# afcarl/BayesBridge

Hardware: AMD Instinct MI355X
Metric: Gibbs sweeps/sec at n=2000,p=50000,alpha=0.5 (higher is better)
Workload: dtype f64; 1 GPU; C3 Gaussian bridge n=2000 p=50000 alpha=0.5; n=2000, p=50000, mode=single, parallelism=one GPU, beta_step=woodbury (exact, p > n), gram=ozaki-II int8 (fp64-accurate)

## Files before the change

### bayesbridge_amd/__init__.py

```python
from __future__ import annotations

import ctypes
import os
from dataclasses import dataclass
from typing import Optional

import numpy as np

from . import _build

__all__ = ["bridge_reg_stb", "bridge_reg", "retstable_ld", "set_seed", "get_rng_state",
           "set_rng_state", "Engine", "EngineConfig", "library", "device_count",
           "sample_lambda", "retstable_batch", "gram", "chol_solve", "bridge_reg_stb_chains",
           "bridge_reg_tri_chains", "ChainBatch", "compute_units",
           "bridge_reg_stb_chains_summary", "bridge_reg_tri_chains_summary", "trace_summary",
           "bridge_reg_logit_chains", "bridge_reg_logit_chains_summary"]

_lib: Optional[ctypes.CDLL] = None
_dp = ctypes.POINTER(ctypes.c_double)
_ip = ctypes.POINTER(ctypes.c_int)


class bb_config(ctypes.Structure):
    _fields_ = [("n", ctypes.c_int), ("p", ctypes.c_int), ("p_local", ctypes.c_int),
                ("j0", ctypes.c_int), ("rank", ctypes.c_int), ("world", ctypes.c_int),
                ("sig2_shape", ctypes.c_double), ("sig2_scale", ctypes.c_double),
                ("nu_shape", ctypes.c_double), ("nu_rate", ctypes.c_double),
                ("alpha_a", ctypes.c_double), ("alpha_b", ctypes.c_double),
                ("true_sig2", ctypes.c_double), ("true_tau", ctypes.c_double),
                ("true_alpha", ctypes.c_double), ("ortho", ctypes.c_int),
                ("method", ctypes.c_int), ("trace_capacity", ctypes.c_int),
                ("seed", ctypes.c_uint64), ("stream", ctypes.c_uint64), ("device", ctypes.c_int),
                ("gram_mode", ctypes.c_int), ("betaburn", ctypes.c_int)]

GRAM_FP64, GRAM_OZAKI = 0, 1


EXPORTED_SYMBOLS = [
    "bridge_reg_stable", "retstable_LD", "bb_version", "bb_last_error", "bb_device_count",
    "bb_set_seed", "bb_get_rng_state", "bb_set_rng_state", "bb_use_r_rng", "bb_set_device",
    "bb_set_verbose", "bb_config_default", "bb_engine_create", "bb_engine_destroy",
    "bb_comm_id_size", "bb_comm_unique_id", "bb_engine_comm_init", "bb_engine_init_state",
    "bb_engine_run", "bb_engine_sync", "bb_engine_get_trace", "bb_engine_get_state",
    "bb_engine_set_state", "bb_engine_method", "bb_engine_enable_timing",
    "bb_engine_kernel_times", "bb_engine_reset_timing", "bb_engine_error_flags",
    "bb_retstable_batch", "bb_sample_lambda", "bb_gram", "bb_chol_solve",
    "bb_engine_phase_times", "bb_phase_count", "bb_phase_name", "bb_bench_lambda",
    "bb_group_create", "bb_group_destroy", "bb_group_init_state", "bb_group_run",
    "bb_bench_chol", "bb_gram_ozaki", "bb_engine_gram_mode", "bb_bench_ozaki",
    "bridge_EM", "bb_bridge_em", "bb_bridge_em_batch", "bridge_regression",
    "bb_engine_get_tri_trace", "bb_engine_get_tri_basis", "bb_engine_set_tri_state",
    "rtnorm_left", "rtnorm_both", "rtnorm", "rtexpon_rate_left", "rtexpon_rate_both",
    "rtexpon_rate", "mytest", "bb_trunc_batch", "rrtgamma_rate", "bb_rrtgamma_batch",
    "bridge_reg_stable_csc", "bb_engine_create_csc", "bb_engine_sparse_pairs", "bb_sparse_gram",
    "bb_bench_sparse_gram", "bb_engine_sparse_info", "bridge_reg_logit", "bb_engine_get_omega",
    "bb_pg_batch", "bb_group_create_rccl", "bb_group_sync", "bb_set_device_count",
    "bb_set_trace_budget", "bb_debug_interrupt_after", "bb_last_call_info",
    "bb_engine_set_timed_phase", "bb_engine_set_timing_stride", "bb_set_chol_version",
    "bb_set_tuning", "bridge_reg_stable_chains", "bb_chains_create", "bb_chains_destroy",
    "bb_chains_count", "bb_chains_resident_per_cu", "bb_chains_init_state", "bb_chains_run",
    "bb_chains_sync", "bb_chains_get_trace", "bb_chains_get_state", "bb_chains_set_state",
    "bb_chains_error_flags", "bridge_regression_chains", "bb_chains_get_tri_trace",
    "bb_chains_set_tri_state", "bb_chains_get_tri_basis", "bb_chains_threads",
    "bb_chains_set_threads", "bb_compute_units", "bridge_reg_stable_chains_summary",
    "bridge_regression_chains_summary", "bb_chains_summary_reset", "bb_chains_summary_add",
    "bb_chains_summary_get", "bb_trace_summary", "bridge_reg_logit_chains",
    "bridge_reg_logit_chains_summary", "bb_chains_get_omega", "bb_set_em_scratch_budget",
]


def library(build: bool = True) -> ctypes.CDLL:
    global _lib
    if _lib is not None:
        return _lib
    path = _build.SO_PATH
    if build:
        try:
            path = _build.build()
        except Exception:
            if not os.path.exists(_build.SO_PATH):
                raise
    if not os.path.exists(path):
        raise RuntimeError(f"BayesBridge.so not found at {path}; run bayesbridge_amd._build")
    L = ctypes.CDLL(path)
    c = ctypes
    L.bb_version.restype = c.c_char_p
    L.bb_last_error.restype = c.c_char_p
    L.bb_device_count.restype = c.c_int
    L.bb_set_seed.argtypes = [c.c_uint64]
    L.bb_get_rng_state.argtypes = [c.POINTER(c.c_uint64), c.POINTER(c.c_uint64)]
    L.bb_set_rng_state.argtypes = [c.c_uint64, c.c_uint64]
    L.bb_use_r_rng.argtypes = [c.c_int]
    L.bb_set_device.argtypes = [c.c_int]
    L.bb_set_verbose.argtypes = [c.c_int]
    L.bb_config_default.argtypes = [c.POINTER(bb_config)]
    L.bb_engine_create.argtypes = [c.POINTER(bb_config), _dp, _dp, c.POINTER(c.c_void_p)]
    L.bb_engine_destroy.argtypes = [c.c_void_p]
    L.bb_comm_id_size.restype = c.c_int
    L.bb_comm_unique_id.argtypes = [c.c_void_p]
    L.bb_engine_comm_init.argtypes = [c.c_void_p, c.c_void_p]
    L.bb_engine_init_state.argtypes = [c.c_void_p]
    L.bb_engine_run.argtypes = [c.c_void_p, c.c_uint64, c.c_int, c.c_int, c.c_int, c.c_int]
    L.bb_engine_sync.argtypes = [c.c_void_p]
    L.bb_engine_get_trace.argtypes = [c.c_void_p, c.c_int, c.c_int, _dp, _dp, _dp, _dp, _dp]
    L.bb_engine_get_state.argtypes = [c.c_void_p, _dp, _dp, _dp, _dp, _dp]
    L.bb_engine_set_state.argtypes = [c.c_void_p, _dp, c.c_double, c.c_double, c.c_double]
    L.bb_engine_method.argtypes = [c.c_void_p]
    L.bb_engine_gram_mode.argtypes = [c.c_void_p]
    L.bb_engine_enable_timing.argtypes = [c.c_void_p, c.c_int]
    L.bb_engine_reset_timing.argtypes = [c.c_void_p]
    L.bb_engine_set_timed_phase.argtypes = [c.c_void_p, c.c_int]
    L.bb_engine_set_timing_stride.argtypes = [c.c_void_p, c.c_int]
    L.bb_engine_kernel_times.argtypes = [c.c_void_p, _dp, _dp, _ip]
    L.bb_engine_error_flags.argtypes = [c.c_void_p, c.POINTER(c.c_uint32)]
    L.bb_retstable_batch.argtypes = [_dp, _dp, _dp, _dp, c.c_int, c.c_uint64, c.c_uint64,
                                     c.c_uint64, c.c_int]
    L.bb_sample_lambda.argtypes = [_dp, _dp, c.c_int, c.c_double, c.c_double, c.c_uint64,
                                   c.c_uint64, c.c_uint64, c.c_uint64, c.c_int]
    L.bb_gram.argtypes = [_dp, _dp, _dp, c.c_int, c.c_int]
    L.bb_gram_ozaki.argtypes = [_dp, _dp, _dp, c.c_int, c.c_int]
    L.bb_bench_ozaki.argtypes = [c.c_int, c.c_int, c.c_int, c.c_int, c.c_int, _dp]
    L.bb_chol_solve.argtypes = [_dp, _dp, _dp, c.c_int, c.c_int]
    L.bb_group_create.argtypes = [c.POINTER(c.c_void_p), c.c_int, c.POINTER(c.c_void_p)]
    L.bb_group_create_rccl.argtypes = [c.POINTER(c.c_void_p), c.c_int, c.POINTER(c.c_void_p)]
    L.bb_group_sync.argtypes = [c.c_void_p]
    L.bb_set_device_count.argtypes = [c.c_int]
    L.bb_set_chol_version.argtypes = [c.c_int]
    L.bb_set_tuning.argtypes = [c.c_int, c.c_int]
    L.bb_set_trace_budget.argtypes = [c.c_longlong]
    L.bb_set_em_scratch_budget.argtypes = [c.c_longlong]
    L.bb_debug_interrupt_after.argtypes = [c.c_int]
    L.bb_last_call_info.argtypes = [_ip, _ip, _ip]
    L.bb_debug_fail_member.argtypes = [c.c_int, c.c_int]
    u64p = c.POINTER(c.c_ulonglong)
    L.bb_engine_nid_stats.argtypes = [c.c_void_p, u64p, u64p, u64p, _dp, _ip]
    L.bb_engine_timed_brackets.argtypes = [c.c_void_p, _ip]
    L.bb_engine_nid_bound.argtypes = [c.c_void_p, _dp, _ip]
    L.bb_engine_launch_counts.argtypes = [c.c_void_p, u64p, u64p]
    L.bb_kernel_instance.argtypes = [c.c_char_p, c.c_char_p, c.c_int]
    L.bb_engine_nid_mixed.argtypes = [c.c_void_p, u64p, u64p, _dp, _ip, _ip]
    L.bb_engine_nid_beta32.argtypes = [c.c_void_p, u64p, _ip]
    L.bb_group_destroy.argtypes = [c.c_void_p]
    L.bb_group_init_state.argtypes = [c.c_void_p]
    L.bb_group_run.argtypes = [c.c_void_p, c.c_uint64, c.c_int, c.c_int, c.c_int, c.c_int]
    L.bb_bench_chol.argtypes = [c.c_int, c.c_int, _dp, _dp, c.c_void_p]
    L.bb_bench_lambda.argtypes = [_dp, c.c_int, c.c_double, c.c_double, c.c_int, c.c_int,
                                  c.c_int, _dp, _dp]
    L.bb_engine_phase_times.argtypes = [c.c_void_p, _dp, c.c_int, _ip]
    L.bb_phase_count.restype = c.c_int
    L.bb_phase_name.argtypes = [c.c_int]
    L.bb_phase_name.restype = c.c_char_p
    L.retstable_LD.argtypes = [_dp, _dp, _dp, _dp, _ip]
    L.bridge_reg_stable.argtypes = [_dp] * 7 + [_dp] * 9 + [_ip] * 4 + [_dp, _ip]
    L.bridge_reg_stable_chains.argtypes = [_dp] * 7 + [_dp] * 9 + [_ip] * 4 + [_dp, _ip, _ip]
    L.bb_chains_create.argtypes = [c.POINTER(bb_config), c.c_int, _dp, _dp,
                                   c.POINTER(c.c_void_p)]
    L.bb_chains_destroy.argtypes = [c.c_void_p]
    L.bb_chains_count.argtypes = [c.c_void_p]
    L.bb_chains_resident_per_cu.argtypes = [c.c_void_p]
    L.bb_chains_init_state.argtypes = [c.c_void_p]
    L.bb_chains_run.argtypes = [c.c_void_p, c.c_uint64, c.c_int, c.c_int, c.c_int, c.c_int]
    L.bb_chains_sync.argtypes = [c.c_void_p]
    L.bb_chains_get_trace.argtypes = [c.c_void_p, c.c_int, c.c_int, c.c_int, _dp, _dp, _dp, _dp,
                                      _dp]
    L.bb_chains_get_state.argtypes = [c.c_void_p, c.c_int, _dp, _dp, _dp, _dp, _dp]
    L.bb_chains_set_state.argtypes = [c.c_void_p, c.c_int, _dp, c.c_double, c.c_double,
                                      c.c_double]
    L.bb_chains_error_flags.argtypes = [c.c_void_p, c.c_int]
    L.bb_chains_error_flags.restype = c.c_uint
    L.bridge_reg_stable_csc.argtypes = ([_dp] * 6 + [_ip, _ip, _dp] + [_dp] * 9 + [_ip] * 4 +
                                        [_dp, _ip])
    L.bb_engine_create_csc.argtypes = [c.POINTER(bb_config), _ip, _ip, _dp, _dp,
                                       c.POINTER(c.c_void_p)]
    L.bb_engine_sparse_pairs.argtypes = [c.c_void_p]
    L.bb_engine_sparse_pairs.restype = c.c_longlong
    L.bridge_reg_logit.argtypes = [_dp] * 6 + [_dp] * 6 + [_ip] * 4 + [_dp]
    L.bb_engine_get_omega.argtypes = [c.c_void_p, _dp]
    L.bridge_reg_logit_chains.argtypes = [_dp] * 6 + [_dp] * 6 + [_ip] * 4 + [_dp, _ip]
    L.bridge_reg_logit_chains_summary.argtypes = ([_dp] * 5 + [_ip, _ip] + [_dp] * 2 + [_dp] * 6 +
                                                  [_ip] * 4 + [_dp, _ip])
    L.bb_chains_get_omega.argtypes = [c.c_void_p, c.c_int, _dp]
    L.bb_pg_batch.argtypes = [_dp, _dp, c.c_int, c.c_uint64, c.c_uint64, c.c_uint64]
    L.bb_engine_sparse_info.argtypes = [c.c_void_p, c.POINTER(c.c_longlong),
                                        c.POINTER(c.c_longlong), _ip, _ip]
    L.bb_sparse_gram.argtypes = [_dp, _dp, _ip, _ip, _dp, _dp, _dp, c.c_int, c.c_int]
    L.bb_bench_sparse_gram.argtypes = [_ip, _ip, _dp, _dp, c.c_int, c.c_int, c.c_int, _dp, _dp,
                                       c.POINTER(c.c_longlong)]
    L.bridge_regression.argtypes = [_dp] * 9 + [_dp] * 9 + [_ip] * 4 + [_dp] + [_ip] * 3
    for name, npar in (("rtnorm_left", 3), ("rtnorm_both", 4), ("rtnorm", 4),
                       ("rtexpon_rate_left", 2), ("rtexpon_rate_both", 3), ("rtexpon_rate", 3)):
        getattr(L, name).argtypes = [_dp] * (1 + npar) + [_ip]
    L.mytest.argtypes = [_ip, _dp]
    L.rrtgamma_rate.argtypes = [_dp] * 4 + [_ip]
    L.bb_rrtgamma_batch.argtypes = [c.c_int, _dp, _dp, _dp, _dp, c.c_uint64, c.c_uint64]
    L.bb_trunc_batch.argtypes = [c.c_int, c.c_int, _dp, _dp, _dp, _dp, _dp, c.c_uint64,
                                 c.c_uint64]
    L.bridge_regression_chains.argtypes = ([_dp] * 9 + [_dp] * 9 + [_ip] * 4 + [_dp] +
                                           [_ip] * 4)
    L.bb_chains_get_tri_trace.argtypes = [c.c_void_p, c.c_int, c.c_int, c.c_int, _dp, _dp]
    L.bridge_reg_stable_chains_summary.argtypes = ([_dp] * 5 + [_ip, _ip] + [_dp] * 2 +
                                                   [_dp] * 9 + [_ip] * 4 + [_dp, _ip, _ip])
    L.bridge_regression_chains_summary.argtypes = ([_dp] * 5 + [_ip, _ip] + [_dp] * 2 +
                                                   [_dp] * 9 + [_ip] * 4 + [_dp] + [_ip] * 4)
    L.bb_chains_summary_reset.argtypes = [c.c_void_p, c.c_int, c.c_int]
    L.bb_chains_summary_add.argtypes = [c.c_void_p, c.c_int, c.c_int, c.c_int]
    L.bb_chains_summary_get.argtypes = [c.c_void_p, _dp, _dp, _dp, _dp, _dp, _ip]
    L.bb_trace_summary.argtypes = [_dp, c.c_int, c.c_int, c.c_int, c.c_int, c.c_int, _dp, _dp,
                                   _dp, _dp, _dp]
    L.bb_chains_set_tri_state.argtypes = [c.c_void_p, c.c_int, _dp]
    L.bb_chains_get_tri_basis.argtypes = [c.c_void_p, _dp, _dp, _dp]
    L.bb_chains_threads.argtypes = [c.c_void_p]
    L.bb_compute_units.argtypes = [c.c_int]
    L.bb_chains_set_threads.argtypes = [c.c_void_p, c.c_int]
    L.bb_engine_get_tri_trace.argtypes = [c.c_void_p, c.c_int, c.c_int, _dp, _dp]
    L.bb_engine_get_tri_basis.argtypes = [c.c_void_p, _dp, _dp, _dp]
    L.bb_engine_set_tri_state.argtypes = [c.c_void_p, _dp]
    L.bridge_EM.argtypes = [_dp, _dp, _dp, _dp, _dp, _ip, _ip, _dp, _dp, _ip, _ip]
    L.bb_bridge_em.argtypes = [_dp, _dp, _dp, c.c_int, c.c_int, c.c_double, c.c_double,
                               c.c_double, c.c_double, c.c_int, c.c_int]
    L.bb_bridge_em_batch.argtypes = [_dp, _ip, _dp, _dp, c.c_int, c.c_int, _dp, _dp, c.c_int,
                                     c.c_double, c.c_double, c.c_int]
    _lib = L
    return L


def device_count() -> int:
    return int(library().bb_device_count())


def compute_units(device: int = 0) -> int:
    _require_gpu()
    n = int(library().bb_compute_units(int(device)))
    if n < 1:
        raise RuntimeError(f"bayesbridge_amd: cannot query device {device}")
    return n


def _require_gpu():
    if device_count() < 1:
        raise RuntimeError("bayesbridge_amd: no HIP device visible (the sampler has no CPU path)")


def kernel_instance(phase: str):
    buf = ctypes.create_string_buffer(512)
    if library().bb_kernel_instance(phase.encode(), buf, 512) != 0:
        return None
    return buf.value.decode()


def _err() -> str:
    return library().bb_last_error().decode()


def _check(rc: int, what: str):
    if rc != 0:
        raise RuntimeError(f"{what} failed ({rc}): {_err()}")


def _p(a: np.ndarray):
    return a.ctypes.data_as(_dp)


def set_seed(seed: int) -> None:
    library().bb_set_seed(int(seed) & 0xFFFFFFFFFFFFFFFF)


def get_rng_state():
    s, t = ctypes.c_uint64(), ctypes.c_uint64()
    library().bb_get_rng_state(ctypes.byref(s), ctypes.byref(t))
    return int(s.value), int(t.value)


def set_rng_state(seed: int, stream: int) -> None:
    library().bb_set_rng_state(int(seed), int(stream))


def set_verbose(v: int) -> None:
    library().bb_set_verbose(int(v))


def set_device_count(k: int) -> None:
    library().bb_set_device_count(int(k))


def set_chol_version(version: int) -> None:
    _check(library().bb_set_chol_version(int(version)), "bb_set_chol_version")


def set_tuning(key: int, value: int) -> int:
    return int(library().bb_set_tuning(int(key), int(value)))


def set_wide_chains(on: bool) -> bool:
    return bool(library().bb_set_tuning(25, 1 if on else 0))
# ... 829 lines not shown

    def __init__(self, cfg: EngineConfig, X_local, y):
        L = library()
        _require_gpu()
        self.cfg = cfg
        self._c = cfg.to_c()
        y = np.ascontiguousarray(y, dtype=np.float64)
        self.p_local = self._c.p_local
        h = ctypes.c_void_p()
        if _is_sparse(X_local):
            colptr, rowidx, val, shape = csc_arrays(X_local)
            assert shape == (cfg.n, self._c.p_local), shape
            _check(L.bb_engine_create_csc(ctypes.byref(self._c), colptr.ctypes.data_as(_ip),
                                          rowidx.ctypes.data_as(_ip), _p(val), _p(y),
                                          ctypes.byref(h)), "bb_engine_create_csc")
        else:
            X_local = np.asfortranarray(X_local, dtype=np.float64)
            assert X_local.shape == (cfg.n, self._c.p_local), X_local.shape
            _check(L.bb_engine_create(ctypes.byref(self._c), _p(X_local), _p(y),
                                      ctypes.byref(h)), "bb_engine_create")
        self._h = h

    def sparse_pairs(self) -> int:
        return int(library().bb_engine_sparse_pairs(self._h))

    def sparse_info(self):
        pr, nz, mr, cm = ctypes.c_longlong(), ctypes.c_longlong(), ctypes.c_int(), ctypes.c_int()
        _check(library().bb_engine_sparse_info(self._h, ctypes.byref(pr), ctypes.byref(nz),
                                               ctypes.byref(mr), ctypes.byref(cm)),
               "bb_engine_sparse_info")
        return dict(pairs=pr.value, nnz=nz.value, max_row=mr.value, col_mode=bool(cm.value))

    def comm_init(self, id_bytes: bytes):
        _check(library().bb_engine_comm_init(self._h, ctypes.c_char_p(id_bytes)),
               "bb_engine_comm_init")

    @staticmethod
    def comm_unique_id() -> bytes:
        L = library()
        buf = ctypes.create_string_buffer(L.bb_comm_id_size())
        _check(L.bb_comm_unique_id(buf), "bb_comm_unique_id")
        return buf.raw

    def init_state(self):
        _check(library().bb_engine_init_state(self._h), "bb_engine_init_state")

    def run(self, t0: int, count: int, first_slot: int = -1, slot_step: int = 1,
            mcmc_phase: int = 1):
        _check(library().bb_engine_run(self._h, int(t0), int(count), int(first_slot),
                                       int(slot_step), int(mcmc_phase)), "bb_engine_run")

    def sync(self):
        _check(library().bb_engine_sync(self._h), "bb_engine_sync")

    def method(self) -> int:
        return int(library().bb_engine_method(self._h))

    def gram_mode(self) -> int:
        return int(library().bb_engine_gram_mode(self._h))

    def trace(self, slot0: int, count: int):
        pl = self.p_local
        beta = np.zeros((pl, count), order="F")
        lam = np.zeros((pl, count), order="F")
        sig2, tau, alpha = np.zeros(count), np.zeros(count), np.zeros(count)
        _check(library().bb_engine_get_trace(self._h, slot0, count, _p(beta), _p(lam), _p(sig2),
                                             _p(tau), _p(alpha)), "bb_engine_get_trace")
        return dict(beta=beta, **{"lambda": lam}, sig2=sig2, tau=tau, alpha=alpha)

    def omega(self):
        om = np.zeros(self.cfg.n)
        _check(library().bb_engine_get_omega(self._h, _p(om)), "bb_engine_get_omega")
        return om

    def tri_trace(self, slot0: int, count: int):
        pl = self.p_local
        u = np.zeros((pl, count), order="F")
        shape = np.zeros((pl, count), order="F")
        _check(library().bb_engine_get_tri_trace(self._h, slot0, count, _p(u), _p(shape)),
               "bb_engine_get_tri_trace")
        return dict(u=u, shape=shape)

    def set_tri_state(self, u):
        u = np.ascontiguousarray(u, dtype=np.float64)
        _check(library().bb_engine_set_tri_state(self._h, _p(u)), "bb_engine_set_tri_state")

    def tri_basis(self):
        p = self.p_local
        tV = np.zeros((p, p), order="F")
        a, d = np.zeros(p), np.zeros(p)
        _check(library().bb_engine_get_tri_basis(self._h, _p(tV), _p(a), _p(d)),
               "bb_engine_get_tri_basis")
        return tV, a, d

    def state(self):
        pl = self.p_local
        beta, lam = np.zeros(pl), np.zeros(pl)
        tau, sig2, alpha = ctypes.c_double(), ctypes.c_double(), ctypes.c_double()
        _check(library().bb_engine_get_state(self._h, _p(beta), _p(lam), ctypes.byref(tau),
                                             ctypes.byref(sig2), ctypes.byref(alpha)),
               "bb_engine_get_state")
        return dict(beta=beta, **{"lambda": lam}, tau=tau.value, sig2=sig2.value,
                    alpha=alpha.value)

    def set_state(self, beta, tau, sig2, alpha):
        beta = np.ascontiguousarray(beta, dtype=np.float64)
        _check(library().bb_engine_set_state(self._h, _p(beta), tau, sig2, alpha),
               "bb_engine_set_state")

    def enable_timing(self, on: bool = True, phases: bool = True, timed_phase: str = "gram",
                      stride: int = 1):
        L = library()
        names = [L.bb_phase_name(i).decode() for i in range(L.bb_phase_count())]
        _check(L.bb_engine_set_timed_phase(self._h, names.index(timed_phase)),
               "bb_engine_set_timed_phase")
        _check(L.bb_engine_set_timing_stride(self._h, int(stride)),
               "bb_engine_set_timing_stride")
        L.bb_engine_enable_timing(self._h, (2 if phases else 1) if on else 0)

    def reset_timing(self):
        library().bb_engine_reset_timing(self._h)

    def kernel_times(self):
        g, s, n = ctypes.c_double(), ctypes.c_double(), ctypes.c_int()
        _check(library().bb_engine_kernel_times(self._h, ctypes.byref(g), ctypes.byref(s),
                                                ctypes.byref(n)), "bb_engine_kernel_times")
        return g.value, s.value, n.value

    def phase_times(self):
        L = library()
        k = L.bb_phase_count()
        ms = np.zeros(k)
        n = ctypes.c_int()
        _check(L.bb_engine_phase_times(self._h, _p(ms), k, ctypes.byref(n)),
               "bb_engine_phase_times")
        return {L.bb_phase_name(i).decode(): float(ms[i]) for i in range(k) if ms[i] > 0}

    def timed_brackets(self) -> int:
        k = ctypes.c_int()
        _check(library().bb_engine_timed_brackets(self._h, ctypes.byref(k)),
               "bb_engine_timed_brackets")
        return int(k.value)

    def nid_stats(self):
        a, b, c = ctypes.c_ulonglong(), ctypes.c_ulonglong(), ctypes.c_ulonglong()
        eps, mode = ctypes.c_double(), ctypes.c_int()
        _check(library().bb_engine_nid_stats(self._h, ctypes.byref(a), ctypes.byref(b),
                                             ctypes.byref(c), ctypes.byref(eps),
                                             ctypes.byref(mode)), "bb_engine_nid_stats")
        lam, kmax = ctypes.c_double(), ctypes.c_int()
        library().bb_engine_nid_bound(self._h, ctypes.byref(lam), ctypes.byref(kmax))
        return dict(cheb_sweeps=a.value, products=b.value, chol_sweeps=c.value, eps=eps.value,
                    mode=mode.value, lambda_x=lam.value, kmax=kmax.value,
                    beta32_sweeps=self._beta32()[0])

    def _beta32(self):
        a, f = ctypes.c_ulonglong(), ctypes.c_int()
        _check(library().bb_engine_nid_beta32(self._h, ctypes.byref(a), ctypes.byref(f)),
               "bb_engine_nid_beta32")
        return a.value, bool(f.value)

    def nid_mixed(self):
        a, b = ctypes.c_ulonglong(), ctypes.c_ulonglong()
        eta, k2, hx = ctypes.c_double(), ctypes.c_int(), ctypes.c_int()
        _check(library().bb_engine_nid_mixed(self._h, ctypes.byref(a), ctypes.byref(b),
                                             ctypes.byref(eta), ctypes.byref(k2),
                                             ctypes.byref(hx)), "bb_engine_nid_mixed")
        n32, last32 = self._beta32()
        return dict(mixed_sweeps=a.value, products32=b.value, eta=eta.value, k2=k2.value,
                    holds_x32=bool(hx.value), beta32_sweeps=n32, beta32=last32)

    def launch_counts(self):
        a, b = ctypes.c_ulonglong(), ctypes.c_ulonglong()
        library().bb_engine_launch_counts(self._h, ctypes.byref(a), ctypes.byref(b))
        return dict(lambda_xu=a.value, lambda_alone=b.value)

    def error_flags(self) -> int:
        f = ctypes.c_uint32()
        _check(library().bb_engine_error_flags(self._h, ctypes.byref(f)), "bb_engine_error_flags")
        return int(f.value)

    def close(self):
        if getattr(self, "_h", None):
            library().bb_engine_destroy(self._h)
            self._h = None

    def __del__(self):
        try:
            self.close()
        except Exception:
            pass


class ChainBatch:

    def __init__(self, cfg: EngineConfig, nchains: int, X, y):
        L = library()
        _require_gpu()
        self.cfg = cfg
        self._c = cfg.to_c()
        self.p = self._c.p
        X = np.asfortranarray(X, dtype=np.float64)
        y = np.ascontiguousarray(y, dtype=np.float64)
        assert X.shape == (cfg.n, cfg.p), X.shape
        h = ctypes.c_void_p()
        _check(L.bb_chains_create(ctypes.byref(self._c), int(nchains), _p(X), _p(y),
                                  ctypes.byref(h)), "bb_chains_create")
        self._h = h
        self.nchains = int(L.bb_chains_count(h))

    def resident_per_cu(self) -> int:
        return int(library().bb_chains_resident_per_cu(self._h))

    def init_state(self):
        _check(library().bb_chains_init_state(self._h), "bb_chains_init_state")

    def run(self, t0: int, count: int, first_slot: int = -1, slot_step: int = 1,
            mcmc_phase: int = 1):
        _check(library().bb_chains_run(self._h, int(t0), int(count), int(first_slot),
                                       int(slot_step), int(mcmc_phase)), "bb_chains_run")

    def sync(self):
        _check(library().bb_chains_sync(self._h), "bb_chains_sync")

    def trace(self, chain: int, slot0: int, count: int):
        p = self.p
        beta = np.zeros((p, count), order="F")
        lam = np.zeros((p, count), order="F")
        sig2, tau, alpha = np.zeros(count), np.zeros(count), np.zeros(count)
        _check(library().bb_chains_get_trace(self._h, int(chain), slot0, count, _p(beta),
                                             _p(lam), _p(sig2), _p(tau), _p(alpha)),
               "bb_chains_get_trace")
        return dict(beta=beta, **{"lambda": lam}, sig2=sig2, tau=tau, alpha=alpha)

    def state(self, chain: int):
        beta, lam = np.zeros(self.p), np.zeros(self.p)
        tau, sig2, alpha = ctypes.c_double(), ctypes.c_double(), ctypes.c_double()
        _check(library().bb_chains_get_state(self._h, int(chain), _p(beta), _p(lam),
                                             ctypes.byref(tau), ctypes.byref(sig2),
                                             ctypes.byref(alpha)), "bb_chains_get_state")
        return dict(beta=beta, **{"lambda": lam}, tau=tau.value, sig2=sig2.value,
                    alpha=alpha.value)

    def set_state(self, chain: int, beta, tau, sig2, alpha):
        beta = np.ascontiguousarray(beta, dtype=np.float64)
        _check(library().bb_chains_set_state(self._h, int(chain), _p(beta), tau, sig2, alpha),
               "bb_chains_set_state")

    def omega(self, chain: int):
        om = np.zeros(self._c.n)
        _check(library().bb_chains_get_omega(self._h, int(chain), _p(om)), "bb_chains_get_omega")
        return om

    def tri_trace(self, chain: int, slot0: int, count: int):
        u = np.zeros((self.p, count), order="F")
        shape = np.zeros((self.p, count), order="F")
        _check(library().bb_chains_get_tri_trace(self._h, int(chain), slot0, count, _p(u),
                                                 _p(shape)), "bb_chains_get_tri_trace")
        return dict(u=u, shape=shape)

    def set_tri_state(self, chain: int, u):
        u = np.ascontiguousarray(u, dtype=np.float64)
        _check(library().bb_chains_set_tri_state(self._h, int(chain), _p(u)),
               "bb_chains_set_tri_state")

    def tri_basis(self):
        p = self.p
        tV = np.zeros((p, p), order="F")
        a, d = np.zeros(p), np.zeros(p)
        _check(library().bb_chains_get_tri_basis(self._h, _p(tV), _p(a), _p(d)),
               "bb_chains_get_tri_basis")
        return tV, a, d

    def summary_reset(self, nsamp: int, maxlag=None):
        self._sum = (int(nsamp), _summary_maxlag(nsamp, maxlag))
        _check(library().bb_chains_summary_reset(self._h, *self._sum), "bb_chains_summary_reset")

    def summary_add(self, slot0: int, count: int, s0: int):
        _check(library().bb_chains_summary_add(self._h, int(slot0), int(count), int(s0)),
               "bb_chains_summary_add")

    def summary(self):
        nsamp, lag = getattr(self, "_sum", (0, 0))
        raw = _summary_buffers(self.nchains, self.p + 3, lag)
        _check(library().bb_chains_summary_get(
            self._h, _p(raw["mean"]), _p(raw["var"]), _p(raw["acov"]), _p(raw["hmean"]),
            _p(raw["hvar"]), raw["flags"].ctypes.data_as(_ip)), "bb_chains_summary_get")
        raw["flags"] = raw["flags"].astype(np.uint32)
        raw.update(nsamp=nsamp, maxlag=lag, p=self.p)
        return raw

    def threads(self) -> int:
        return int(library().bb_chains_threads(self._h))

    def set_threads(self, threads: int):
        _check(library().bb_chains_set_threads(self._h, int(threads)), "bb_chains_set_threads")

    def error_flags(self, chain: int) -> int:
        f = int(library().bb_chains_error_flags(self._h, int(chain)))
        if f == 0xFFFFFFFF and _err():
            raise RuntimeError(f"bb_chains_error_flags failed: {_err()}")
        return f

    def close(self):
        if getattr(self, "_h", None):
            library().bb_chains_destroy(self._h)
            self._h = None

    def __del__(self):
        try:
            self.close()
        except Exception:
            pass


class ShardGroup:

    def __init__(self, engines, rccl=False):
        L = library()
        self.engines = list(engines)
        arr = (ctypes.c_void_p * len(self.engines))(*[e._h.value for e in self.engines])
        h = ctypes.c_void_p()
        fn = L.bb_group_create_rccl if rccl else L.bb_group_create
# ... 24 lines not shown
```

### bayesbridge_amd/csrc/bb_engine.cpp

```cpp
#include <dlfcn.h>

#include <chrono>
#include <cxxabi.h>
#include <cmath>
#include <cstring>
#include <atomic>
#include <initializer_list>
#include <memory>
#include <mutex>
#include <thread>

#include "../../include/bayesbridge.h"
#include "bb_host.h"
#include "bb_ozaki.h"

using namespace bb;

namespace bb {

thread_local std::string g_last_error;
int g_device = 0;
int g_verbose = 1;

}

namespace {

std::mutex g_mu;
uint64_t g_seed = 0xB4E5B41D6EULL;
uint64_t g_stream = 0;
int g_use_r_rng = 1;
std::atomic<int> g_debug_fail_member{-1}, g_debug_fail_sweep{-1};

struct RRng {
    void (*get)(void) = nullptr;
    void (*put)(void) = nullptr;
    double (*unif)(void) = nullptr;
    bool tried = false;
    bool ok() {
        if (!tried) {
            tried = true;
            get = (void (*)(void))dlsym(RTLD_DEFAULT, "GetRNGstate");
            put = (void (*)(void))dlsym(RTLD_DEFAULT, "PutRNGstate");
            unif = (double (*)(void))dlsym(RTLD_DEFAULT, "unif_rand");
        }
        return get && put && unif;
    }
} g_rrng;

}

void bb::next_call_key(uint64_t *k0, uint64_t *k1, int count) {
    std::lock_guard<std::mutex> lk(g_mu);
    if (g_use_r_rng && g_rrng.ok()) {
        g_rrng.get();
        uint64_t a = (uint64_t)(g_rrng.unif() * 4294967296.0);
        uint64_t b = (uint64_t)(g_rrng.unif() * 4294967296.0);
        uint64_t c = (uint64_t)(g_rrng.unif() * 4294967296.0);
        g_rrng.put();
        *k0 = (a << 32) ^ b;
        *k1 = c;
        return;
    }
    *k0 = g_seed;
    *k1 = g_stream;
    g_stream += (uint64_t)count;
}

enum Phase {
    PH_PRE, PH_SCALARS, PH_LAMBDA, PH_PG, PH_OZPREP, PH_GRAM, PH_XU, PH_REDUCE, PH_FORM, PH_CHOL,
    PH_SOLVE, PH_BETA, PH_XB, PH_ALPHA, PH_NID, PH_EAPPLY, PH_END, PH_COUNT
};

int g_nid_kmax = 16;
int g_nid_sync = 1;
int g_shard_proto = 0;
int g_nid_mixed = 1;
int g_nid_poll = 1;
int g_nid_fold = 1;
int g_nid_b32 = 1;
int g_chains_packed = 0;
int g_chains_wide = 0;
int g_fused_alpha = 0;
int g_fused_tri_alpha = 0;
static const char *kPhaseNames[PH_COUNT] = {"pre", "scalars", "lambda", "pg", "ozprep", "gram",
                                            "xu", "reduce", "form", "chol", "solve", "beta",
                                            "xb", "alpha", "nid", "eapply", "end"};

enum Method { AUTO = 0, CHOL = 1, WOODBURY = 2, ORTHO = 3, TRI = 4, SPARSE = 5, LOGIT = 6 };

struct bb_engine {
    bb_config cfg{};
    int n = 0, p = 0, p_loc = 0, n_pad = 0, p_pad = 0;
    int chol_m = 0;
    Method method = AUTO;
    int group = 1;
    bool fused = false;
    bool wide = false;
    SparseDesign spd;
    Hyper hy{};
    hipStream_t stream = nullptr;
    std::vector<void *> owned;

    double *X = nullptr, *y = nullptr;
    double *beta = nullptr, *lam = nullptr, *D = nullptr, *u = nullptr;
    DevScalars *sc = nullptr;
    uint32_t *err = nullptr;
    double *xb_part = nullptr, *red1 = nullptr;
    double *red3 = nullptr;
    int nparts = 0, nbS = 0;
    bool xb_stale = false;
    double *slabs = nullptr, *xu_part = nullptr, *red2 = nullptr, *M = nullptr, *w = nullptr,
           *Wd = nullptr;
    unsigned int *flags = nullptr;
    int S = 1;
    size_t slab_stride = 0;
    int n_oz = 0, oz_b = 0, oz_S = 1;
    double *oz_xmax = nullptr, *oz_rscale = nullptr;
    double *oz_rowmax = nullptr;
    int *oz_escale = nullptr;
    int8_t *oz_R = nullptr, *oz_P = nullptr;
    double *Xt = nullptr, *omega = nullptr, *kappa = nullptr, *Gw = nullptr;
    double *G = nullptr, *cvec = nullptr, *A = nullptr, *Y2 = nullptr, *W2 = nullptr,
           *gdiag = nullptr;
    double *tVc = nullptr, *tVr = nullptr, *tri_a = nullptr, *tri_d = nullptr,
           *tri_G = nullptr;
    double *tr_u = nullptr, *tr_shape = nullptr;
    std::vector<double> h_tV, h_a, h_d;
    double *tr_beta = nullptr, *tr_lam = nullptr, *tr_sig2 = nullptr, *tr_tau = nullptr,
           *tr_alpha = nullptr;
    int cap = 1;
    double *cn = nullptr;
    NidState *nid = nullptr;
    double *ch_r = nullptr, *ch_d = nullptr, *ea_part = nullptr, *sp_s = nullptr,
           *nid_xu = nullptr;
    double *eps_host = nullptr;
    float *X32 = nullptr;
    double *ch_b = nullptr;
    int nid_k2 = 0;
    double *gb = nullptr, *ch_c = nullptr, *ch_xu = nullptr;
    bool nid_b32 = false;
    double nid_cost[3] = {0.0, 0.0, 0.0};
    int ea_parts = 1;
    int nid_kmax = 0;
    double lambda_x = 0.0;
    hipEvent_t nid_ev[8] = {};
    long nid_seq = 0;
    double *nid_red = nullptr, *nid_sum = nullptr, *nid_wg = nullptr;
    hipEvent_t nid_sev = nullptr;
    bool nid_only = false;
    bool group_member = false;
    int nid_last = -1;
    ncclComm_t comm = nullptr;
    bool own_comm = true;
    bool timing = false;
    int timing_level = 2;
    int timed_phase = PH_GRAM;
    int timing_stride = 1;
    std::vector<hipEvent_t> ev_pool;
    std::vector<std::vector<std::pair<int, int>>> sweep_marks;
    size_t ev_next = 0;

    void mark(int phase) {
        if (!timing) return;
        if (timing_level == 1) {
            if ((sweep_marks.size() - 1) % (size_t)timing_stride != 0) return;
            const bool open = !sweep_marks.back().empty() &&
                              sweep_marks.back().back().first == timed_phase;
            if (phase != timed_phase && !open) return;
        }
        int e0 = ev();
        HIPCHECK(hipEventRecord(ev_pool[e0], stream));
        sweep_marks.back().push_back({phase, e0});
    }

    ~bb_engine() {
        if (stream) (void)hipStreamSynchronize(stream);
        if (comm && own_comm) ncclCommDestroy(comm);
        for (auto e : ev_pool) (void)hipEventDestroy(e);
        for (auto e : nid_ev)
            if (e) (void)hipEventDestroy(e);
        if (nid_sev) (void)hipEventDestroy(nid_sev);
        if (eps_host) (void)hipHostFree(eps_host);
        for (void *q : owned) (void)hipFree(q);
        if (stream) (void)hipStreamDestroy(stream);
    }

    int ev() {
        if (ev_next == ev_pool.size()) {
            hipEvent_t e;
            HIPCHECK(hipEventCreate(&e));
            ev_pool.push_back(e);
        }
        return (int)ev_next++;
    }

    void allreduce(double *buf, size_t count) {
        if (cfg.world <= 1 && !comm) return;
        if (!comm) throw HipError("world > 1 but no communicator (call bb_engine_comm_init)");
        NCCLCHECK(ncclAllReduce(buf, buf, count, ncclFloat64, ncclSum, comm, stream));
    }

    double *slot_ptr(double *base, int slot, int stride) {
        if (slot < 0 || base == nullptr) return nullptr;
        return base + (size_t)(slot % cap) * stride;
    }

    bool woodbury() const { return method == WOODBURY || method == SPARSE; }
    bool dense() const { return method == WOODBURY; }
    bool sparse() const { return method == SPARSE; }
    bool ortho() const { return method == ORTHO; }
    bool tri() const { return method == TRI; }
    bool logit() const { return method == LOGIT; }
    bool pxp() const { return method == CHOL || method == LOGIT; }

    bool nid_enabled() const {
        return nid != nullptr && (cfg.world == 1 || comm != nullptr || group_member) &&
               std::min(g_nid_kmax, nid_kmax) > 0;
    }
    bool sharded() const {
        return cfg.world > 1 || (g_shard_proto && (comm != nullptr || group_member));
    }
    bool nid_sync() const { return (sharded() || g_nid_sync) && nid_enabled(); }
    bool mixed_ok() const {
        return X32 != nullptr && g_nid_mixed && !sharded() && !group_member && dense();
    }
    bool b32_ok() const { return gb != nullptr && g_nid_b32 && mixed_ok() && nid_sync(); }
    int allow_mask() const {
        return (mixed_ok() ? kAllowMixed : 0) |
               (b32_ok() ? kAllowBeta32 | (g_nid_b32 == 2 ? kBeta32AnyCost : 0) : 0);
    }
    double *bank() const { return b32_ok() ? gb : nullptr; }
    Beta32Vecs b32_vecs() const {
        return b32_ok() ? Beta32Vecs{ch_c, ch_b, ch_xu, xb_part} : Beta32Vecs{};
    }
    bool nid_vec() const { return sharded() || sparse(); }

    int nid_kmax_model() const {
        double t_pass, t_chol;
        const double steps = n_pad / 64.0;
        if (sparse()) {
            t_pass = 24.0 * (double)spd.nnz / 3.0e12 + 10e-6;
            t_chol = 10.0 * (double)spd.pairs / 4.0e12 + steps * 21e-6 + 60e-6;
        } else {
            t_pass = 8.0 * n_pad * (double)p_loc / 6.0e12 + 10e-6;
            const double gram = cfg.gram_mode == 1
                ? 16.0 * (double)n_pad * n_pad * p_pad / 2.6e15 + 24.0 * (double)n_pad * p_pad / 5.0e12
                : 2.0 * (double)n_pad * n_pad * p_pad / 33e12;
            t_chol = gram + steps * 19e-6 + 40e-6;
        }
        if (cfg.world > 1) {
            t_pass += 25e-6;
            t_chol += 8.0 * (double)red2_count() / 100e9 + 25e-6;
        }
        return (int)std::min(64.0, std::floor(t_chol / t_pass));
    }

    static constexpr int kNidRing = 8, kNidLag = 3;
    int nid_launch_count() {
        const int kmax = std::min(g_nid_kmax, nid_kmax);
        if (nid_seq < kNidLag) return kmax;
        const long q = nid_seq - kNidLag;
        wait_event(nid_ev[q % kNidRing]);
        const double h = ((volatile double *)eps_host)[q % kNidRing];
        if (!(h >= 0.0)) return kmax;
        return cheb_iterations(8.0 * h, kmax, kNidTol);
    }

    int nid_begin(int kl) {
        if (!nid_enabled()) return 0;
        mark(PH_NID);
        const long q = nid_seq++;
        launch_nid_sums(stream, D, cn, p_loc, sc, nid, kl, kl > 0, 1, nid_wg, nid_red,
                        eps_dev + q % kNidRing);
        hipEvent_t &ev = nid_ev[q % kNidRing];
        if (!ev) HIPCHECK(hipEventCreateWithFlags(&ev, hipEventDisableTiming));
        HIPCHECK(hipEventRecord(ev, stream));
        return kl;
    }
    double *eps_dev = nullptr;

    void nid_solve(uint64_t t, int kl) {
        mark(PH_NID);
        if (sparse())
            launch_cheb_init(stream, nid_xu, 1, n, n_pad, y, sc, cfg.seed, cfg.stream, t, nid, w,
                             ch_r, ch_d);
        else
            launch_cheb_init(stream, nid_xu, xu_fused ? xu_fused : ea_parts, n, n_pad, y, sc,
                             cfg.seed, cfg.stream, t, nid, w, ch_r, ch_d);
        for (int j = 1; j < kl; ++j) {
            mark(PH_EAPPLY);
            if (sparse())
                launch_sp_eapply(stream, spd.colptr, spd.rowidx, spd.cval, spd.rowptr, spd.colidx,
                                 spd.rval, p_loc, n_pad, D, ch_d, nid, j, sp_s, ea_part);
            else
                launch_eapply(stream, X, n_pad, n_pad, p_loc, D, ch_d, nid, j, ea_part);
            mark(PH_NID);
            launch_cheb_step(stream, ea_part, sparse() ? 1 : ea_parts, n_pad, sc, nid, j, w,
                             ch_r, ch_d);
        }
    }

    static constexpr int kNidRed = kNidTS + 2;
    void nidx_partials(int folded = 0, int nstream = 0) {
        mark(PH_NID);
        if (folded == 2) return;
        if (folded == 1 && sharded())
            launch_nid_reduce(stream, nid_wg, nstream, sc, nid, nid_red);
        else if (folded == 1)
            launch_nid_reduce(stream, nid_wg, nstream, sc, nid, nid_red,
                              std::min(g_nid_kmax, nid_kmax), eps_dev + kNidRing,
                              allow_mask(), ++nid_dseq);
        else if (sharded())
            launch_nid_sums(stream, D, cn, p_loc, sc, nid, 0, 0, 0, nid_wg, nid_red, nullptr);
        else
            launch_nid_sums_decide(stream, D, cn, p_loc, sc, nid, std::min(g_nid_kmax, nid_kmax),
                                   nid_wg, nid_red, eps_dev + kNidRing, allow_mask(),
                                   ++nid_dseq);
    }
    void nidx_decide_launch() {
        if (sharded())
            launch_nid_decide_from(stream, nid_red, sc, std::min(g_nid_kmax, nid_kmax), nid,
                                   eps_dev + kNidRing, ++nid_dseq);
        if (g_nid_poll) return;
        if (!nid_sev) HIPCHECK(hipEventCreateWithFlags(&nid_sev, hipEventDisableTiming));
        HIPCHECK(hipEventRecord(nid_sev, stream));
    }
    int nidx_decide_read() {
        int mode, k2;
        if (g_nid_poll) {
            const unsigned long long tag = wait_tag(nid_dseq);
            mode = (int)((tag >> 8) & 0xff);
            k2 = (int)(tag & 0xff);
        } else {
            wait_event(nid_sev);
            mode = (int)((volatile double *)eps_host)[kNidRing + 1];
            k2 = (int)((volatile double *)eps_host)[kNidRing + 2];
        }
        nid_b32 = b32_ok() && (k2 & 128) != 0;
        k2 &= 127;
        nid_k2 = mixed_ok() ? k2 : 0;
        nid_only = mode > 0;
        nid_last = mode;
        return mode;
    }
    unsigned long long wait_tag(unsigned long long seq) {
        const unsigned long long *tp = (const unsigned long long *)(eps_host + kNidRing + 3);
        const unsigned long long want = seq & 0xffffffffffffull;
        for (long spin = 0;; ++spin) {
            const unsigned long long v = __atomic_load_n(tp, __ATOMIC_ACQUIRE);
            if ((v >> 16) == want) return v;
            if ((spin & 1023) != 1023) {
                __builtin_ia32_pause();
                continue;
            }
            if (stop && stop->load(std::memory_order_relaxed))
                throw HipError("stopped: another member of the shard group failed");
            const hipError_t q = hipStreamQuery(stream);
            if (q == hipSuccess) {
                const unsigned long long w = __atomic_load_n(tp, __ATOMIC_ACQUIRE);
                if ((w >> 16) == want) return w;
                throw HipError("near-identity decision tag not written by the drained stream");
            }
            if (q != hipErrorNotReady) HIPCHECK(q);
            if (spin > 65536) std::this_thread::yield();
        }
    }
    unsigned long long nid_dseq = 0;
    void wait_event(hipEvent_t ev) {
        if (!stop) {
            HIPCHECK(hipEventSynchronize(ev));
            return;
        }
        for (long spin = 0;; ++spin) {
            const hipError_t q = hipEventQuery(ev);
            if (q == hipSuccess) return;
            if (q != hipErrorNotReady) HIPCHECK(q);
            if (stop->load(std::memory_order_relaxed))
                throw HipError("stopped: another member of the shard group failed");
            if (spin > 64) std::this_thread::yield();
        }
    }
    void nidx_xu() {
        mark(PH_NID);
        if (sparse()) {
            launch_sp_nid_xu(stream, spd.rowptr, spd.colidx, spd.rval, n_pad, u, nid, nid_sum);
        } else {
            if (!xu_fused) launch_nid_xu(stream, X, n_pad, u, p_loc, n_pad, nid, nid_xu);
            if (nid_vec())
                launch_part_sum(stream, nid_xu, xu_fused ? xu_fused : ea_parts, n_pad, nid_sum);
        }
    }
    void nidx_init(uint64_t t) {
        if (nid_vec())
            launch_cheb_init(stream, nid_sum, 1, n, n_pad, y, sc, cfg.seed, cfg.stream, t, nid,
                             w, ch_r, ch_d);
        else
            launch_cheb_init(stream, nid_xu, xu_fused ? xu_fused : ea_parts, n, n_pad, y, sc,
                             cfg.seed, cfg.stream, t, nid, w, ch_r, ch_d,
                             mixed_ok() ? ch_b : nullptr, b32_ok() ? ch_xu : nullptr);
    }
    void nidx_mixed_tail(int k2) {
        const Beta32Vecs bv = b32_vecs();
        mark(PH_EAPPLY);
        launch_eapply(stream, X, n_pad, n_pad, p_loc, D, w, nid, 0, ea_part, X32, 2, bank());
        mark(PH_NID);
        launch_cheb_restart(stream, ea_part, ea_parts, n_pad, sc, nid, ch_b, w, ch_r, ch_d, &bv);
        for (int j = 1; j < k2; ++j) {
            mark(PH_EAPPLY);
            launch_eapply(stream, X, n_pad, n_pad, p_loc, D, ch_d, nid, j, ea_part, X32, 3);
            mark(PH_NID);
            launch_cheb_step(stream, ea_part, ea_parts, n_pad, sc, nid, j, w, ch_r, ch_d, 2,
                             &bv);
        }
    }
    void nidx_eapply(int j) {
        mark(PH_EAPPLY);
        if (sparse()) {
            launch_sp_eapply(stream, spd.colptr, spd.rowidx, spd.cval, spd.rowptr, spd.colidx,
                             spd.rval, p_loc, n_pad, D, ch_d, nid, j, sp_s, nid_sum);
        } else {
            launch_eapply(stream, X, n_pad, n_pad, p_loc, D, ch_d, nid, j, ea_part,
                          mixed_ok() ? X32 : nullptr, 0, bank());
            if (nid_vec()) launch_part_sum(stream, ea_part, ea_parts, n_pad, nid_sum);
        }
    }
    void nidx_step(int j) {
        mark(PH_NID);
        if (nid_vec())
            launch_cheb_step(stream, nid_sum, 1, n_pad, sc, nid, j, w, ch_r, ch_d);
        else {
            const Beta32Vecs bv = b32_vecs();
            launch_cheb_step(stream, ea_part, ea_parts, n_pad, sc, nid, j, w, ch_r, ch_d, 1, &bv);
        }
    }
    void xbeta() {
        xb_stale = false;
        if (sparse()) {
            launch_sp_rows(stream, spd.rowptr, spd.colidx, spd.rval, n_pad, beta, nullptr,
                           xb_part, nullptr);
            nparts = 1;
        } else {
            launch_xv(stream, X, n_pad, beta, p_loc, n_pad, xb_part);
            nparts = xv_chunks(p_loc, n_pad);
        }
    }

    void pre() {
        if (xb_stale) xbeta();
        launch_pre(stream, xb_part, nparts, n_pad, beta, p_loc, sc, red1, nbS);
    }
    void scalars(uint64_t t, int slot, int tau_only) {
        launch_scalars(stream, red1, nbS, y, n, p, sc, hy, cfg.seed, cfg.stream, t,
                       slot_ptr(tr_tau, slot, 1), slot_ptr(tr_sig2, slot, 1),
                       slot_ptr(tr_alpha, slot, 1), tau_only, err);
    }

    void phase_a(uint64_t t) {
        (void)t;
        if (timing) sweep_marks.emplace_back();
        mark(PH_PRE);
        pre();
    }

    void wb_gram(const int *gate) {
        if (sparse()) {
            mark(PH_GRAM);
            spd.gram(stream, D, u, red2, red2 + tri_count(n_pad), gate);
            return;
        }
        if (cfg.gram_mode == 1) {
            mark(PH_OZPREP);
            launch_oz_scale(stream, D, p_pad, oz_xmax, n_oz, oz_b, oz_rowmax, oz_rscale,
                            oz_escale, gate);
            launch_oz_residues(stream, X, n_pad, n_pad, n_oz, p_pad, D, oz_rscale, oz_R, u,
                               xu_part, gate);
            mark(PH_GRAM);
            launch_oz_gemm(stream, oz_R, n_oz, p_pad, oz_S, oz_P, 0, kOzLeadDefault, -1, gate);
        } else {
            mark(PH_GRAM);
            launch_gram(stream, X, n_pad, D, n_pad, p_pad, S, slabs, n_pad, slab_stride, gate);
            mark(PH_XU);
            launch_xv(stream, X, n_pad, u, p_pad, n_pad, xu_part, gate);
        }
        mark(PH_REDUCE);
        if (cfg.gram_mode == 1)
            launch_oz_crt(stream, oz_P, oz_S, n_oz, n_pad, oz_escale, xu_part,
                          oz_xu_parts(p_pad, n_oz), red2, gate);
        else
            launch_slab_sum(stream, slabs, S, slab_stride, n_pad, xu_part, xv_chunks(p_pad, n_pad),
                            red2, 1, gate);
    }

    void phase_b(uint64_t t, int slot) {
        mark(PH_SCALARS);
        scalars(t, slot, 0);
        double *trl = slot_ptr(tr_lam, slot, p_loc);
        mark(PH_LAMBDA);
        if (woodbury()) {
            const bool sync = nid_sync();
            const int kl = (!sync && nid_enabled()) ? nid_launch_count() : 0;
            xu_fused = 0;
            int folded = 0;
            if (dense() && (sync ? nid_last != 0 : kl > 0)) {
                NidFold fold;
                if (sync && g_nid_fold) {
                    fold.cn = cn;
                    fold.wg_part = nid_wg;
                    fold.cnt = lam_sync + lambda_xs_sync_words(p_pad);
                    fold.decide = (!sharded() && g_nid_fold == 2) ? 1 : 0;
                    fold.k_launched = std::min(g_nid_kmax, nid_kmax);
                    fold.allow_mixed = allow_mask();
                    fold.nid = nid;
                    fold.red = nid_red;
                    fold.host2 = eps_dev + kNidRing;
                    fold.tag_seq = nid_dseq + 1;
                }
                xu_fused = launch_lambda_xu(stream, beta, p_loc, p_pad, (uint64_t)cfg.j0, sc,
                                            cfg.seed, cfg.stream, t, lam, D, u, trl, err, X,
                                            n_pad, n_pad, nid_xu, lam_sync, ++lam_ep, &fold,
                                            &folded);
                if (folded == 2) ++nid_dseq;
            }
            if (!xu_fused)
                launch_lambda(stream, beta, p_loc, p_pad, (uint64_t)cfg.j0, sc, cfg.seed,
                              cfg.stream, t, LAMBDA_WOODBURY, group, lam, D, u, trl, err);
            ++(xu_fused ? n_lambda_xu : n_lambda_alone);
            nid_only = false;
            nid_b32 = false;
            if (sync) {
                nid_kl = 0;
                nidx_partials(folded, xu_fused);
                return;
            }
            nid_kl = nid_begin(kl);
            wb_gram(nid_kl ? &nid->mode : nullptr);
            if (nid_kl && !xu_fused) {
                mark(PH_NID);
                if (sparse())
                    launch_sp_nid_xu(stream, spd.rowptr, spd.colidx, spd.rval, n_pad, u, nid,
                                     nid_xu);
                else
                    launch_nid_xu(stream, X, n_pad, u, p_loc, n_pad, nid, nid_xu);
            }
        } else if (logit()) {
            if (!launch_lambda_pg(stream, beta, p_loc, p_pad, 0, sc, cfg.seed, cfg.stream, t,
                                  group, lam, trl, red1 + nbS, n, n_pad, omega, err))
                throw HipError("logistic sweep: p beyond the fused lambda / Polya-Gamma launch");
            if (cfg.gram_mode == 1) {
                mark(PH_OZPREP);
                launch_oz_scale(stream, omega, n_pad, oz_xmax, n_oz, oz_b, oz_rowmax, oz_rscale,
                                oz_escale);
                launch_oz_residues(stream, Xt, p_pad, p_pad, n_oz, n_pad, omega, oz_rscale, oz_R,
                                   nullptr, nullptr);
                mark(PH_GRAM);
                launch_oz_gemm(stream, oz_R, n_oz, n_pad, oz_S, oz_P);
                mark(PH_REDUCE);
                launch_oz_crt(stream, oz_P, oz_S, n_oz, p_pad, oz_escale, nullptr, 0, Gw);
            } else {
                mark(PH_GRAM);
                launch_gram(stream, Xt, p_pad, omega, p_pad, n_pad, S, slabs, p_pad, slab_stride);
                mark(PH_REDUCE);
                launch_slab_sum(stream, slabs, S, slab_stride, p_pad, nullptr, 0, Gw, 0);
            }
        } else if (tri()) {
            mark(PH_BETA);
            launch_tri_update(stream, beta, u, lam, D, p, tVc, tVr, tri_a, tri_d, tri_G, cvec,
// ... 273 lines not shown
                if (c == 0.0 || fabs(c) <= 1e-15 * sqrt(a * b)) continue;
                ++rotated;
                const double zeta = (b - a) / (2.0 * c);
                const double t = (zeta >= 0 ? 1.0 : -1.0) / (fabs(zeta) + sqrt(1.0 + zeta * zeta));
                const double cs = 1.0 / sqrt(1.0 + t * t), sn = cs * t;
                nrm2[i] = a - t * c;
                nrm2[j] = b + t * c;
                for (int k = 0; k < p; ++k) {
                    const double x = wi[k], y = wj[k];
                    wi[k] = cs * x - sn * y;
                    wj[k] = sn * x + cs * y;
                    const double u = vi[k], w = vj[k];
                    vi[k] = cs * u - sn * w;
                    vj[k] = sn * u + cs * w;
                }
            }
        }
        if (rotated == 0) break;
    }
    d.resize(p);
    for (int j = 0; j < p; ++j) {
        double s2 = 0.0;
        for (int k = 0; k < p; ++k) s2 += W[(size_t)j * p + k] * W[(size_t)j * p + k];
        d[j] = sqrt(s2);
    }
}

void tri_setup(bb_engine *e, const double *Xh) {
    const int p = e->p, pp = e->p_pad;
    std::vector<double> Gp((size_t)pp * pp), c(pp);
    HIPCHECK(hipStreamSynchronize(e->stream));
    HIPCHECK(hipMemcpy(Gp.data(), e->G, Gp.size() * sizeof(double), hipMemcpyDeviceToHost));
    HIPCHECK(hipMemcpy(c.data(), e->cvec, (size_t)pp * sizeof(double), hipMemcpyDeviceToHost));
    std::vector<double> G((size_t)p * p);
    for (int j = 0; j < p; ++j)
        for (int i = 0; i < p; ++i) {
            const int r = i < j ? i : j, q = i < j ? j : i;
            G[(size_t)j * p + i] = Gp[(size_t)q * pp + r];
        }
    std::vector<double> V, sv;
    svd_right(Xh, e->n, p, V, sv);
    std::vector<int> ord(p);
    for (int i = 0; i < p; ++i) ord[i] = i;
    std::stable_sort(ord.begin(), ord.end(), [&](int x, int y) { return sv[x] > sv[y]; });
    e->h_tV.assign((size_t)p * p, 0.0);
    e->h_a.assign(p, 0.0);
    e->h_d.assign(p, 0.0);
    std::vector<double> tVr((size_t)p * p);
    for (int i = 0; i < p; ++i) {
        const double *v = &V[(size_t)ord[i] * p];
        int jm = 0;
        for (int j = 1; j < p; ++j)
            if (fabs(v[j]) > fabs(v[jm])) jm = j;
        const double sg = v[jm] < 0 ? -1.0 : 1.0;
        double a = 0.0;
        for (int j = 0; j < p; ++j) {
            const double x = sg * v[j];
            e->h_tV[i + (size_t)j * p] = x;
            tVr[(size_t)i * p + j] = x;
            a += x * c[j];
        }
        e->h_a[i] = a;
        e->h_d[i] = sv[ord[i]];
    }
    auto &o = e->owned;
    e->tVc = dalloc<double>((size_t)p * p, o);
    e->tVr = dalloc<double>((size_t)p * p, o);
    e->tri_a = dalloc<double>(p, o);
    e->tri_d = dalloc<double>(p, o);
    HIPCHECK(hipMemcpy(e->tVc, e->h_tV.data(), (size_t)p * p * sizeof(double),
                       hipMemcpyHostToDevice));
    HIPCHECK(hipMemcpy(e->tVr, tVr.data(), (size_t)p * p * sizeof(double), hipMemcpyHostToDevice));
    HIPCHECK(hipMemcpy(e->tri_a, e->h_a.data(), (size_t)p * sizeof(double), hipMemcpyHostToDevice));
    HIPCHECK(hipMemcpy(e->tri_d, e->h_d.data(), (size_t)p * sizeof(double), hipMemcpyHostToDevice));
    e->tri_G = dalloc<double>((size_t)p * p, o);
    HIPCHECK(hipMemcpy(e->tri_G, G.data(), (size_t)p * p * sizeof(double), hipMemcpyHostToDevice));
    e->tr_u = dalloc<double>((size_t)p * e->cap, o);
    e->tr_shape = dalloc<double>((size_t)p * e->cap, o);
}

struct SparseIn {
    const int *colptr, *rowidx;
    const double *val;
};

void nid_certify_lambda(bb_engine *e) {
    const int n_pad = e->n_pad, p_pad = e->p_pad;
    hipStream_t s = e->stream;
    double *ones = nullptr;
    NidState *gate = nullptr;
    HIPCHECK(hipMalloc(&ones, (size_t)p_pad * sizeof(double)));
    HIPCHECK(hipMalloc(&gate, sizeof(NidState)));
    std::vector<double> h1(p_pad, 0.0);
    for (int j = 0; j < e->p_loc; ++j) h1[j] = 1.0;
    HIPCHECK(hipMemcpyAsync(ones, h1.data(), h1.size() * sizeof(double), hipMemcpyHostToDevice, s));
    NidState g{};
    g.mode = 64;
    HIPCHECK(hipMemcpyAsync(gate, &g, sizeof(g), hipMemcpyHostToDevice, s));
    std::vector<double> v(n_pad, 0.0), w(n_pad);
    double nv = 0.0;
    for (int i = 0; i < e->n; ++i) {
        v[i] = std::cos(0.7 * i + 0.3) + 0.5 * std::sin(1.3 * i * i + 0.1);
        nv += v[i] * v[i];
    }
    for (auto &x : v) x /= std::sqrt(nv);
    double rho = 0.0;
    for (int it = 0; it < 40; ++it) {
        HIPCHECK(hipMemcpyAsync(e->ch_d, v.data(), n_pad * sizeof(double), hipMemcpyHostToDevice, s));
        if (e->sparse())
            launch_sp_eapply(s, e->spd.colptr, e->spd.rowidx, e->spd.cval, e->spd.rowptr,
                             e->spd.colidx, e->spd.rval, e->p_loc, n_pad, ones, e->ch_d, gate, 0,
                             e->sp_s, e->ea_part);
        else
            launch_eapply(s, e->X, n_pad, n_pad, e->p_loc, ones, e->ch_d, gate, 0, e->ea_part);
        launch_part_sum(s, e->ea_part, e->sparse() ? 1 : e->ea_parts, n_pad, e->ch_r);
        HIPCHECK(hipMemcpyAsync(w.data(), e->ch_r, n_pad * sizeof(double), hipMemcpyDeviceToHost, s));
        HIPCHECK(hipStreamSynchronize(s));
        double vw = 0.0, ww = 0.0;
        for (int i = 0; i < n_pad; ++i) {
            vw += v[i] * w[i];
            ww += w[i] * w[i];
        }
        rho = vw;
        if (!(ww > 0.0)) break;
        for (int i = 0; i < n_pad; ++i) v[i] = w[i] / std::sqrt(ww);
    }
    double lam = 0.0;
    if (rho > 0.0 && std::isfinite(rho)) {
        if (e->sparse()) {
            e->spd.gram(s, ones, ones, e->red2, e->red2 + tri_count(n_pad));
        } else if (e->cfg.gram_mode == 1) {
            launch_oz_scale(s, ones, p_pad, e->oz_xmax, e->n_oz, e->oz_b, e->oz_rowmax,
                            e->oz_rscale, e->oz_escale);
            launch_oz_residues(s, e->X, n_pad, n_pad, e->n_oz, p_pad, ones, e->oz_rscale, e->oz_R);
            launch_oz_gemm(s, e->oz_R, e->n_oz, p_pad, e->oz_S, e->oz_P);
            launch_oz_crt(s, e->oz_P, e->oz_S, e->n_oz, n_pad, e->oz_escale, nullptr, 0, e->red2);
        } else {
            launch_gram(s, e->X, n_pad, ones, n_pad, p_pad, e->S, e->slabs, n_pad, e->slab_stride);
            launch_slab_sum(s, e->slabs, e->S, e->slab_stride, n_pad, nullptr, 0, e->red2, 1);
        }
        double U = 1.02 * rho;
        for (int attempt = 0; attempt < 7 && lam == 0.0; ++attempt, U *= 1.25) {
            e->clear_err();
            launch_shift_gram(s, e->red2, n_pad, U, e->M, n_pad);
            chol_factor(s, e->M, n_pad, n_pad, 1, e->err, e->Wd, e->flags);
            if ((e->read_err() & (8u | 16u)) == 0) lam = U * (1.0 + 1e-9);
        }
        e->clear_err();
    }
    HIPCHECK(hipMemsetAsync(e->nid, 0, sizeof(NidState), s));
    HIPCHECK(hipMemcpyAsync(&e->nid->lambda_x, &lam, sizeof(double), hipMemcpyHostToDevice, s));
    HIPCHECK(hipMemcpyAsync(&e->nid->c64, e->nid_cost, sizeof(e->nid_cost), hipMemcpyHostToDevice,
                            s));
    HIPCHECK(hipStreamSynchronize(s));
    e->lambda_x = lam;
    (void)hipFree(ones);
    (void)hipFree(gate);
}

void engine_setup(bb_engine *e, const double *Xh, const double *yh, const SparseIn *spin) {
    const bb_config &c = e->cfg;
    e->n = c.n;
    e->p = c.p;
    e->p_loc = c.p_local;
    e->n_pad = round_up(c.n, kGramTile);
    e->p_pad = round_up(c.p_local, 256);
    e->chol_m = round_up(c.p_local, kNB);
    e->cap = c.trace_capacity < 1 ? 1 : c.trace_capacity;
    e->hy = Hyper{c.sig2_shape, c.sig2_scale, c.nu_shape, c.nu_rate, c.alpha_a, c.alpha_b,
                  c.true_tau > 0, c.true_sig2 > 0, c.true_alpha > 0};
    if (spin) {
        if (c.ortho || c.method == CHOL || c.method == ORTHO || c.method == TRI ||
            c.method == LOGIT)
            throw HipError("a CSC design runs the Woodbury (p > n) draw only");
        e->method = SPARSE;
    } else if (c.method == LOGIT) {
        e->method = LOGIT;
        e->hy.know_sig2 = 1;
        e->n_pad = round_up(c.n, 512);
        if (c.world > 1) throw HipError("the logistic path runs on one device (world == 1)");
        if (c.ortho) throw HipError("the logistic path has no orthogonal-design variant");
        if (c.p > 16384) throw HipError("logistic path limited to p <= 16384");
    } else if (c.method == TRI) e->method = TRI;
    else if (c.ortho) e->method = ORTHO;
    else if (c.method == CHOL || (c.method == AUTO && c.p <= c.n)) e->method = CHOL;
    else e->method = WOODBURY;
    if (c.world > 1 && !e->woodbury() && !(e->ortho() && c.p > c.n))
        throw HipError("column sharding (world > 1) is implemented for the p > n paths only "
                       "(Woodbury, sparse Woodbury, orthogonal design)");
    if (e->tri() && (c.p > c.n || c.p > kTriMaxP))
        throw HipError("triangle sampler needs p <= n and p <= 2048");
    if (e->method == CHOL && c.p > 16384)
        throw HipError("p x p Cholesky path limited to p <= 16384");
    if (e->woodbury() && e->n_pad > 8192)
        throw HipError("Woodbury path limited to n <= 8192 in this build");

    HIPCHECK(hipSetDevice(c.device));
    HIPCHECK(hipStreamCreateWithFlags(&e->stream, hipStreamNonBlocking));
    auto &o = e->owned;
    const int n_pad = e->n_pad, p_pad = e->p_pad;
    if (spin) {
        e->spd.build(e->stream, c.n, n_pad, c.p_local, spin->colptr, spin->rowidx, spin->val, o);
    } else {
        e->X = dalloc<double>((size_t)n_pad * p_pad, o);
        HIPCHECK(hipMemcpy2D(e->X, (size_t)n_pad * sizeof(double), Xh,
                             (size_t)c.n * sizeof(double), (size_t)c.n * sizeof(double),
                             (size_t)c.p_local, hipMemcpyHostToDevice));
    }
    e->y = dalloc<double>(n_pad, o);
    HIPCHECK(hipMemcpy(e->y, yh, (size_t)c.n * sizeof(double), hipMemcpyHostToDevice));
    e->beta = dalloc<double>(p_pad, o);
    e->lam = dalloc<double>(p_pad, o);
    e->D = dalloc<double>(p_pad, o);
    e->u = dalloc<double>(p_pad, o);
    e->sc = dalloc<DevScalars>(1, o);
    e->err = dalloc<uint32_t>(4, o);
    e->nparts = xv_chunks(p_pad, n_pad);
    e->xb_part = dalloc<double>(
        (size_t)std::max(e->sparse() ? 1 : xv_chunks_max(p_pad), beta_xb_parts(c.p_local)) *
            n_pad,
        o);
    e->nbS = pre_blocks_s(c.p_local);
    e->red1 = dalloc<double>((size_t)e->nbS + n_pad, o);
    e->red3 = dalloc<double>(2, o);
    e->group = stable_group_for(c.p_local);
    e->tr_beta = dalloc<double>((size_t)c.p_local * e->cap, o);
    e->tr_lam = dalloc<double>((size_t)c.p_local * e->cap, o);
    e->tr_sig2 = dalloc<double>(e->cap, o);
    e->tr_tau = dalloc<double>(e->cap, o);
    e->tr_alpha = dalloc<double>(e->cap, o);

    if (e->dense()) {
        if (c.gram_mode == 1) {
            e->n_oz = oz_rows(n_pad);
            const int nkc = p_pad / kOzKC;
            e->oz_b = oz_bits_for(p_pad);
            e->oz_S = oz_splits_for(e->n_oz, nkc);
            e->oz_xmax = dalloc<double>((size_t)nkc * e->n_oz, o);
            e->oz_rowmax = dalloc<double>((size_t)oz_bound_groups(p_pad) * e->n_oz, o);
            e->oz_rscale = dalloc<double>(e->n_oz, o);
            e->oz_escale = dalloc<int>(e->n_oz, o);
            e->oz_R = dalloc<int8_t>(oz_residue_bytes(e->n_oz, p_pad), o);
            e->oz_P = dalloc<int8_t>(oz_partial_bytes(e->n_oz, e->oz_S), o);
            launch_oz_xmax(e->stream, e->X, n_pad, n_pad, e->n_oz, p_pad, e->oz_xmax);
        } else {
            e->S = gram_splits_for(n_pad, p_pad);
            e->slab_stride = (size_t)n_pad * n_pad;
            e->slabs = dalloc<double>(e->slab_stride * e->S, o);
        }
        e->xu_part = dalloc<double>((size_t)xv_chunks_max(p_pad) * n_pad, o);
    }
    if (e->woodbury()) {
        e->red2 = dalloc<double>(tri_count(n_pad) + n_pad, o);
        e->M = dalloc<double>((size_t)n_pad * (n_pad + kNB), o);
        e->w = dalloc<double>(n_pad, o);
        if (e->sparse() || eapply_supported(n_pad)) {
            e->cn = dalloc<double>(p_pad, o);
            if (e->sparse()) {
                std::vector<double> h(c.p_local, 0.0);
                for (int j = 0; j < c.p_local; ++j)
                    for (int q = spin->colptr[j]; q < spin->colptr[j + 1]; ++q)
                        h[j] += spin->val[q] * spin->val[q];
                HIPCHECK(hipMemcpy(e->cn, h.data(), h.size() * sizeof(double),
                                   hipMemcpyHostToDevice));
                e->sp_s = dalloc<double>(p_pad, o);
                e->ea_parts = 1;
                e->ea_part = dalloc<double>(n_pad, o);
                e->nid_xu = dalloc<double>(n_pad, o);
            } else {
                launch_colnorm2(e->stream, e->X, n_pad, n_pad, c.p_local, e->cn);
                e->ea_parts = eapply_parts(c.p_local, n_pad);
                e->ea_part = dalloc<double>((size_t)e->ea_parts * n_pad, o);
                const int xp = std::max(e->ea_parts, lambda_xu_parts(c.p_local, p_pad, n_pad));
                e->nid_xu = dalloc<double>((size_t)xp * n_pad, o);
                const int sw = lambda_xs_sync_words(p_pad) + 1;
                e->lam_sync = dalloc<unsigned int>(sw, o);
                HIPCHECK(hipMemsetAsync(e->lam_sync, 0, sizeof(unsigned int) * sw, e->stream));
            }
            e->nid = dalloc<NidState>(1, o);
            {
                const double bytes = (double)n_pad * (double)c.p_local;
                e->nid_cost[0] = 8.0 * bytes / 6.2e12 + 4e-6;
                e->nid_cost[1] = 4.0 * bytes / 6.2e12 + 4e-6;
                e->nid_cost[2] = 6e-6;
            }
            e->ch_r = dalloc<double>(n_pad, o);
            e->ch_d = dalloc<double>(n_pad, o);
            e->nid_red = dalloc<double>(bb_engine::kNidRed, o);
            e->nid_wg = dalloc<double>(
                (size_t)std::max(nid_sum_groups(c.p_local), 1024) * (kNidTS + 1), o);
            e->nid_sum = dalloc<double>(n_pad, o);
            const int nh = bb_engine::kNidRing + 4;
            HIPCHECK(hipHostMalloc((void **)&e->eps_host, nh * sizeof(double),
                                   hipHostMallocMapped | hipHostMallocCoherent));
            for (int q = 0; q < nh; ++q) e->eps_host[q] = -1.0;
            *(unsigned long long *)(e->eps_host + bb_engine::kNidRing + 3) = 0ull;
            HIPCHECK(hipHostGetDevicePointer((void **)&e->eps_dev, e->eps_host, 0));
            e->nid_kmax = e->nid_kmax_model();
            if (e->dense() && c.world == 1 && g_nid_mixed && e->nid_kmax > 0) {
                void *x32 = nullptr;
                if (hipMalloc(&x32, (size_t)n_pad * p_pad * sizeof(float)) != hipSuccess) {
                    (void)hipGetLastError();
                    x32 = nullptr;
                }
                if (x32) {
                    e->ch_b = dalloc<double>(n_pad, o);
                    int *bad = dalloc<int>(1, o);
                    HIPCHECK(hipMemsetAsync(bad, 0, sizeof(int), e->stream));
                    launch_cast_f32(e->stream, e->X, n_pad, n_pad, c.p_local, (float *)x32, bad);
                    int hb = 0;
                    HIPCHECK(hipMemcpyAsync(&hb, bad, sizeof(int), hipMemcpyDeviceToHost, e->stream));
                    HIPCHECK(hipStreamSynchronize(e->stream));
                    if (hb) {
                        (void)hipFree(x32);
                    } else {
                        o.push_back(x32);
                        e->X32 = (float *)x32;
                        if (beta_xb_supported(n_pad)) {
                            e->gb = dalloc<double>(p_pad, o);
                            e->ch_c = dalloc<double>(n_pad, o);
                            e->ch_xu = dalloc<double>(n_pad, o);
                            HIPCHECK(hipMemsetAsync(e->gb, 0, sizeof(double) * p_pad, e->stream));
                            HIPCHECK(hipMemsetAsync(e->ch_c, 0, sizeof(double) * n_pad, e->stream));
                            HIPCHECK(hipMemsetAsync(e->ch_xu, 0, sizeof(double) * n_pad, e->stream));
                        }
                    }
                }
            }
        }
    }
    const bool small = c.p <= c.n && c.world == 1 && !e->sparse() && !e->logit();
    const int m_sys = (e->woodbury() && !small) ? n_pad : (n_pad > p_pad ? n_pad : p_pad);
    e->Wd = dalloc<double>(chol_wd_words(m_sys), o);
    e->flags = dalloc<unsigned int>(chol_flag_words(m_sys, 1), o);
    if (e->logit()) {
        e->Xt = dalloc<double>((size_t)p_pad * n_pad, o);
        launch_transpose(e->stream, e->X, n_pad, n_pad, p_pad, e->Xt, p_pad);
        if (c.gram_mode == 1) {
            e->n_oz = oz_rows(p_pad);
            const int nkc = n_pad / kOzKC;
            e->oz_b = oz_bits_for(n_pad);
            e->oz_S = oz_splits_for(e->n_oz, nkc);
            e->oz_xmax = dalloc<double>((size_t)nkc * e->n_oz, o);
            e->oz_rowmax = dalloc<double>((size_t)oz_bound_groups(n_pad) * e->n_oz, o);
            e->oz_rscale = dalloc<double>(e->n_oz, o);
            e->oz_escale = dalloc<int>(e->n_oz, o);
            e->oz_R = dalloc<int8_t>(oz_residue_bytes(e->n_oz, n_pad), o);
            e->oz_P = dalloc<int8_t>(oz_partial_bytes(e->n_oz, e->oz_S), o);
            launch_oz_xmax(e->stream, e->Xt, p_pad, p_pad, e->n_oz, n_pad, e->oz_xmax);
        } else {
            e->S = gram_splits_for(p_pad, n_pad);
            e->slab_stride = (size_t)p_pad * p_pad;
            e->slabs = dalloc<double>(e->slab_stride * e->S, o);
        }
        e->Gw = dalloc<double>(std::max((size_t)p_pad * p_pad, tri_count(p_pad)) + p_pad, o);
        e->omega = dalloc<double>(n_pad, o);
        e->kappa = dalloc<double>(n_pad, o);
        launch_kappa(e->stream, e->y, c.n, n_pad, e->kappa);
        e->cvec = dalloc<double>(p_pad, o);
        launch_coldot(e->stream, e->X, n_pad, n_pad, e->kappa, c.p_local, e->cvec);
        e->A = dalloc<double>((size_t)p_pad * (p_pad + kNB), o);
        e->Y2 = dalloc<double>((size_t)2 * p_pad, o);
        e->W2 = dalloc<double>((size_t)2 * p_pad, o);
    } else if (!e->woodbury() || small) {
        e->cvec = dalloc<double>(p_pad, o);
        launch_coldot(e->stream, e->X, n_pad, n_pad, e->y, c.p_local, e->cvec);
        e->gdiag = dalloc<double>(p_pad, o);
        if (small) {
            double *Xt = nullptr;
            HIPCHECK(hipMalloc(&Xt, (size_t)p_pad * n_pad * sizeof(double)));
            launch_transpose(e->stream, e->X, n_pad, n_pad, p_pad, Xt, p_pad);
            double *ones = nullptr;
            HIPCHECK(hipMalloc(&ones, (size_t)n_pad * sizeof(double)));
            std::vector<double> h1(n_pad, 1.0);
            HIPCHECK(hipMemcpyAsync(ones, h1.data(), n_pad * sizeof(double),
                                    hipMemcpyHostToDevice, e->stream));
            const int Sg = gram_splits_for(p_pad, n_pad);
            double *sl = nullptr;
            HIPCHECK(hipMalloc(&sl, (size_t)Sg * p_pad * p_pad * sizeof(double)));
            launch_gram(e->stream, Xt, p_pad, ones, p_pad, n_pad, Sg, sl, p_pad,
                        (size_t)p_pad * p_pad);
            double *red = nullptr;
            HIPCHECK(hipMalloc(&red, ((size_t)p_pad * p_pad + p_pad) * sizeof(double)));
            launch_slab_sum(e->stream, sl, Sg, (size_t)p_pad * p_pad, p_pad, nullptr, 0, red, 0);
            e->G = dalloc<double>((size_t)p_pad * p_pad, o);
            HIPCHECK(hipMemcpyAsync(e->G, red, (size_t)p_pad * p_pad * sizeof(double),
                                    hipMemcpyDeviceToDevice, e->stream));
            HIPCHECK(hipStreamSynchronize(e->stream));
            (void)hipFree(Xt);
            (void)hipFree(ones);
            (void)hipFree(sl);
            (void)hipFree(red);
            launch_gdiag(e->stream, e->G, p_pad, c.p_local, e->gdiag);
            e->A = dalloc<double>((size_t)p_pad * (p_pad + kNB), o);
            e->Y2 = dalloc<double>((size_t)2 * p_pad, o);
            e->W2 = dalloc<double>((size_t)2 * p_pad, o);
        } else {
            launch_colnorm2(e->stream, e->X, n_pad, n_pad, c.p_local, e->gdiag);
        }
    }
    if (e->tri()) tri_setup(e, Xh);
    e->fused = (e->method == CHOL || e->ortho()) && c.p <= kSmallChainMaxP && c.world == 1 &&
               (e->hy.know_alpha || g_fused_alpha) && e->cvec && e->gdiag &&
               (e->ortho() || e->G);
    e->wide = g_chains_wide && (e->method == CHOL || e->ortho()) && c.p > kSmallChainMaxP &&
              c.p <= kWideChainMaxP && (c.p <= c.n || e->ortho()) && c.world == 1 &&
              e->hy.know_alpha && e->cvec && e->gdiag && (e->ortho() || e->G);
    if (e->wide) e->fused = true;
    if (e->tri())
        e->fused = c.p <= kTriChainMaxP && c.world == 1 &&
                   (e->hy.know_alpha || (g_fused_tri_alpha && c.p <= c.n)) &&
                   (!c.ortho || (e->tri_G && e->cvec));
    if (e->nid) nid_certify_lambda(e);
    HIPCHECK(hipStreamSynchronize(e->stream));
}

void engine_init_state_local(bb_engine *e) {
    const bb_config &c = e->cfg;
    e->nid_seq = 0;
    e->nid_last = -1;
    bool ls_ok = false;
    if (e->G != nullptr) {
        e->clear_err();
        const int m = e->chol_m ? e->chol_m : e->p_pad;
        launch_form_a(e->stream, e->G, e->p_pad, nullptr, e->sc, e->cvec, e->p, m, e->A,
                      e->p_pad, m);
        chol_factor(e->stream, e->A, e->p_pad, m, 1, e->err, e->Wd, e->flags);
        HIPCHECK(hipMemcpyAsync(e->Y2, e->A + (size_t)m * e->p_pad, m * sizeof(double),
                                hipMemcpyDeviceToDevice, e->stream));
        chol_bsolve(e->stream, e->A, e->p_pad, m, e->Wd, e->Y2, e->W2, 1, e->flags, e->err);
        uint32_t f = e->read_err();
        ls_ok = (f & 8u) == 0;
        if (ls_ok) {
            HIPCHECK(hipMemcpyAsync(e->beta, e->W2, (size_t)e->p * sizeof(double),
                                    hipMemcpyDeviceToDevice, e->stream));
        }
        e->clear_err();
    }
    if (!ls_ok) {
        HIPCHECK(hipMemsetAsync(e->beta, 0, (size_t)e->p_pad * sizeof(double), e->stream));
        if (g_verbose && c.rank == 0 && !e->logit()) {
            printf("Warning: cannot calculate least squares estimate; X'X is singular.\n");
            printf("Warning: setting least squares estimate to 0.0.\n");
        }
    }
    DevScalars s{};
    s.alpha = c.true_alpha > 0 ? c.true_alpha : 0.5;
    s.sig2 = e->logit() ? 1.0 : (c.true_sig2 > 0 ? c.true_sig2 : 0.0);
    s.tau = c.true_tau > 0 ? c.true_tau : 0.0;
    HIPCHECK(hipMemcpyAsync(e->sc, &s, sizeof(s), hipMemcpyHostToDevice, e->stream));
    if (e->tri()) {
        std::vector<double> h(e->p_pad, 0.5);
        HIPCHECK(hipMemcpyAsync(e->u, h.data(), h.size() * sizeof(double), hipMemcpyHostToDevice,
                                e->stream));
        std::vector<double> h1(e->p_pad, 1.0);
        HIPCHECK(hipMemcpyAsync(e->lam, h1.data(), h1.size() * sizeof(double),
                                hipMemcpyHostToDevice, e->stream));
        HIPCHECK(hipMemcpyAsync(e->tr_u, h.data(), (size_t)e->p_loc * sizeof(double),
                                hipMemcpyHostToDevice, e->stream));
        HIPCHECK(hipMemcpyAsync(e->tr_lam, h1.data(), (size_t)e->p_loc * sizeof(double),
                                hipMemcpyHostToDevice, e->stream));
        HIPCHECK(hipStreamSynchronize(e->stream));
    }
    HIPCHECK(hipMemcpyAsync(e->tr_beta, e->beta, (size_t)e->p_loc * sizeof(double),
                            hipMemcpyDeviceToDevice, e->stream));
    e->xbeta();
    launch_record_scalars(e->stream, e->sc, e->tr_tau, e->tr_sig2, e->tr_alpha);
}

void engine_preburn_draw(bb_engine *e) {
// ... 455 lines not shown
    return guarded([&] {
        if (!e->logit()) throw HipError("not a logistic engine");
        HIPCHECK(hipStreamSynchronize(e->stream));
        HIPCHECK(hipMemcpy(omega, e->omega, (size_t)e->n * sizeof(double), hipMemcpyDeviceToHost));
    });
}

int bb_engine_get_tri_trace(bb_engine *e, int slot0, int count, double *u, double *shape) {
    return guarded([&] {
        if (!e->tri()) throw HipError("not a triangle-method engine");
        HIPCHECK(hipStreamSynchronize(e->stream));
        const size_t pl = (size_t)e->p_loc;
        ring_fetch(slot0, count, e->cap, {{u, e->tr_u, pl}, {shape, e->tr_shape, pl}});
    });
}

int bb_engine_set_tri_state(bb_engine *e, const double *u) {
    return guarded([&] {
        if (!e->tri()) throw HipError("not a triangle-method engine");
        HIPCHECK(hipStreamSynchronize(e->stream));
        HIPCHECK(hipMemcpy(e->u, u, (size_t)e->p_loc * sizeof(double), hipMemcpyHostToDevice));
    });
}

int bb_engine_get_tri_basis(bb_engine *e, double *tV, double *a, double *d) {
    if (!e->tri()) {
        set_error("not a triangle-method engine");
        return -1;
    }
    if (tV) memcpy(tV, e->h_tV.data(), e->h_tV.size() * sizeof(double));
    if (a) memcpy(a, e->h_a.data(), e->h_a.size() * sizeof(double));
    if (d) memcpy(d, e->h_d.data(), e->h_d.size() * sizeof(double));
    return 0;
}
int bb_engine_gram_mode(const bb_engine *e) { return e->cfg.gram_mode; }

int bb_engine_enable_timing(bb_engine *e, int enable) {
    e->timing = enable != 0;
    e->timing_level = enable == 1 ? 1 : 2;
    return 0;
}

int bb_engine_set_timed_phase(bb_engine *e, int phase) {
    if (phase < 0 || phase >= PH_END) {
        set_error("bb_engine_set_timed_phase: phase %d out of range", phase);
        return -1;
    }
    e->timed_phase = phase;
    return 0;
}

int bb_engine_set_timing_stride(bb_engine *e, int stride) {
    if (stride < 1) {
        set_error("bb_engine_set_timing_stride: stride %d < 1", stride);
        return -1;
    }
    e->timing_stride = stride;
    return 0;
}

int bb_engine_reset_timing(bb_engine *e) {
    (void)hipStreamSynchronize(e->stream);
    e->sweep_marks.clear();
    e->ev_next = 0;
    return 0;
}

int bb_engine_phase_times(bb_engine *e, double *ms, int cap, int *samples) {
    return guarded([&] {
        HIPCHECK(hipStreamSynchronize(e->stream));
        std::vector<double> acc(PH_COUNT, 0.0);
        for (auto &marks : e->sweep_marks)
            for (size_t i = 0; i + 1 < marks.size(); ++i) {
                float v = 0;
                HIPCHECK(hipEventElapsedTime(&v, e->ev_pool[marks[i].second],
                                             e->ev_pool[marks[i + 1].second]));
                acc[marks[i].first] += v;
            }
        const double ns = e->sweep_marks.empty() ? 1.0 : (double)e->sweep_marks.size();
        for (int i = 0; i < cap && i < PH_COUNT; ++i) ms[i] = acc[i] / ns;
        if (samples) *samples = (int)e->sweep_marks.size();
    });
}

const char *bb_phase_name(int i) { return (i >= 0 && i < PH_COUNT) ? kPhaseNames[i] : ""; }
int bb_phase_count(void) { return PH_COUNT; }

int bb_engine_kernel_times(bb_engine *e, double *gram_ms_avg, double *sweep_ms_avg,
                           int *samples) {
    return guarded([&] {
        HIPCHECK(hipStreamSynchronize(e->stream));
        double g = 0, s = 0;
        int ng = 0, ns = 0;
        for (auto &marks : e->sweep_marks) {
            for (size_t i = 0; i + 1 < marks.size(); ++i)
                if (marks[i].first == e->timed_phase) {
                    float v = 0;
                    HIPCHECK(hipEventElapsedTime(&v, e->ev_pool[marks[i].second],
                                                 e->ev_pool[marks[i + 1].second]));
                    g += v;
                    ++ng;
                }
            if (marks.size() >= 2) {
                float v = 0;
                HIPCHECK(hipEventElapsedTime(&v, e->ev_pool[marks.front().second],
                                             e->ev_pool[marks.back().second]));
                s += v;
                ++ns;
            }
        }
        if (gram_ms_avg) *gram_ms_avg = ng ? g / ng : 0.0;
        if (sweep_ms_avg) *sweep_ms_avg = ns ? s / ns : 0.0;
        if (samples) *samples = ns;
    });
}

int bb_engine_timed_brackets(bb_engine *e, int *count) {
    int ng = 0;
    for (auto &marks : e->sweep_marks)
        for (size_t i = 0; i + 1 < marks.size(); ++i)
            if (marks[i].first == e->timed_phase) ++ng;
    *count = ng;
    return 0;
}

int bb_engine_nid_mixed(bb_engine *e, unsigned long long *mixed_sweeps,
                        unsigned long long *products32, double *eta, int *k2, int *holds_x32) {
    return guarded([&] {
        NidState h{};
        if (e->nid) {
            HIPCHECK(hipMemcpyAsync(&h, e->nid, sizeof(h), hipMemcpyDeviceToHost, e->stream));
            HIPCHECK(hipStreamSynchronize(e->stream));
        }
        if (mixed_sweeps) *mixed_sweeps = h.n_mixed;
        if (products32) *products32 = h.n_products32;
        if (eta) *eta = h.eta;
        if (k2) *k2 = h.k2;
        if (holds_x32) *holds_x32 = e->X32 != nullptr;
    });
}

int bb_engine_nid_beta32(bb_engine *e, unsigned long long *beta32_sweeps, int *b32) {
    return guarded([&] {
        NidState h{};
        if (e->nid) {
            HIPCHECK(hipMemcpyAsync(&h, e->nid, sizeof(h), hipMemcpyDeviceToHost, e->stream));
            HIPCHECK(hipStreamSynchronize(e->stream));
        }
        if (beta32_sweeps) *beta32_sweeps = h.n_beta32;
        if (b32) *b32 = h.b32;
    });
}

int bb_engine_nid_bound(bb_engine *e, double *lambda_x, int *kmax) {
    if (lambda_x) *lambda_x = e->lambda_x;
    if (kmax) *kmax = e->nid ? std::min(g_nid_kmax, e->nid_kmax) : -1;
    return 0;
}

int bb_engine_nid_stats(bb_engine *e, unsigned long long *cheb_sweeps,
                        unsigned long long *products, unsigned long long *chol_sweeps,
                        double *eps, int *mode) {
    return guarded([&] {
        NidState h{};
        if (e->nid) {
            HIPCHECK(hipMemcpyAsync(&h, e->nid, sizeof(h), hipMemcpyDeviceToHost, e->stream));
            HIPCHECK(hipStreamSynchronize(e->stream));
        }
        if (cheb_sweeps) *cheb_sweeps = h.n_cheb;
        if (products) *products = h.n_products;
        if (chol_sweeps) *chol_sweeps = h.n_chol;
        if (eps) *eps = e->nid ? h.eps : -1.0;
        if (mode) *mode = e->nid ? h.mode : -1;
    });
}

int bb_kernel_instance(const char *phase, char *buf, int len) {
    static const char *kFam[KF_COUNT] = {"lambda", "gram", "reduce", "chol", "solve", "beta",
                                         "eapply"};
    if (!phase || !buf || len <= 0) return -1;
    buf[0] = 0;
    int f = -1;
    for (int i = 0; i < KF_COUNT; ++i)
        if (!strcmp(phase, kFam[i])) f = i;
    const void *k = launched_instance(f);
    if (!k) return -1;
    const char *mangled = hipKernelNameRefByPtr(k, nullptr);
    if (!mangled) return -1;
    int st = 0;
    char *dem = abi::__cxa_demangle(mangled, nullptr, nullptr, &st);
    std::string name = (st == 0 && dem) ? dem : mangled;
    free(dem);
    if (name.rfind("void ", 0) == 0) name = name.substr(5);
    int depth = 0;
    for (size_t i = 0; i < name.size(); ++i) {
        if (name[i] == '<') ++depth;
        if (name[i] == '>') --depth;
        if (name[i] == '(' && depth == 0) {
            name.resize(i);
            break;
        }
    }
    snprintf(buf, (size_t)len, "%s", name.c_str());
    return 0;
}

int bb_engine_launch_counts(bb_engine *e, unsigned long long *lambda_xu,
                            unsigned long long *lambda_alone) {
    if (lambda_xu) *lambda_xu = e->n_lambda_xu;
    if (lambda_alone) *lambda_alone = e->n_lambda_alone;
    return 0;
}

int bb_engine_error_flags(bb_engine *e, uint32_t *flags) {
    return guarded([&] { *flags = e->read_err(); });
}

int bb_chains_create(const bb_config *cfg, int nchains, const double *X, const double *y,
                     bb_chains **out) {
    *out = nullptr;
    if (nchains < 1) {
        set_error("bb_chains_create: nchains must be at least 1 (got %d)", nchains);
        return -1;
    }
    if (const char *why = chains_refusal(*cfg)) {
        set_error("bb_chains_create: %s", why);
        return -1;
    }
    bb_chains *b = new bb_chains();
    try {
        bb_config c = *cfg;
        b->K = nchains;
        b->p = c.p;
        b->cap = c.trace_capacity < 1 ? 1 : c.trace_capacity;
        b->base_stream = c.stream;
        c.p_local = c.p;
        c.trace_capacity = 1;
        if (bb_engine_create(&c, X, y, &b->proto) != 0) throw HipError(g_last_error);
        if (b->proto->logit() != (c.method == LOGIT) ||
            (!b->proto->logit() && (!b->proto->fused || b->proto->tri() != (c.method == TRI))))
            throw HipError("this design does not run as a fused small chain");
        int cus = 0;
        HIPCHECK(hipDeviceGetAttribute(&cus, hipDeviceAttributeMultiprocessorCount, c.device));
        b->wide = b->proto->wide;
        b->packed = !b->tri() && !b->wide && g_chains_packed && nchains >= 2 * cus &&
                    b->proto->hy.know_alpha;
        if (b->tri())
            b->threads = tri_chains_threads(c.n, c.p, nchains, cus, !b->proto->hy.know_alpha);
        auto &o = b->owned;
        const size_t K = (size_t)nchains, p = (size_t)c.p, cap = (size_t)b->cap;
        b->beta = dalloc<double>(K * p, o);
        b->lam = dalloc<double>(K * p, o);
        b->sc = dalloc<DevScalars>(K, o);
        b->sc0 = dalloc<DevScalars>(1, o);
        b->err = dalloc<uint32_t>(K, o);
        b->tr_beta = dalloc<double>(K * cap * p, o);
        b->tr_lam = dalloc<double>(K * cap * p, o);
        b->tr_sig2 = dalloc<double>(K * cap, o);
        b->tr_tau = dalloc<double>(K * cap, o);
        b->tr_alpha = dalloc<double>(K * cap, o);
        if (b->tri()) {
            b->u = dalloc<double>(K * p, o);
            b->shape = dalloc<double>(K * p, o);
            b->tr_u = dalloc<double>(K * cap * p, o);
            b->tr_shape = dalloc<double>(K * cap * p, o);
        }
        if (b->logit()) {
            b->omega = dalloc<double>(K * (size_t)c.n, o);
            HIPCHECK(hipMemset(b->omega, 0, K * (size_t)c.n * sizeof(double)));
        }
    } catch (std::exception &ex) {
        const std::string msg = ex.what();
        delete b;
        set_error("bb_chains_create: %s", msg.c_str());
        return -1;
    }
    *out = b;
    return 0;
}

void bb_chains_destroy(bb_chains *b) { delete b; }
int bb_chains_count(const bb_chains *b) { return b->K; }

int bb_chains_resident_per_cu(const bb_chains *b) {
    if (hipSetDevice(b->proto->cfg.device) != hipSuccess) return -1;
    if (b->tri())
        return tri_chains_resident_per_cu(b->proto->n, b->p, b->threads,
                                          !b->proto->hy.know_alpha);
    if (b->logit())
        return logit_chains_resident_per_cu(b->proto->n, b->p, !b->proto->hy.know_alpha);
    if (b->wide) return wide_chains_resident_per_cu(b->p);
    return small_chains_resident_per_cu(b->proto->n, b->p, b->packed, !b->proto->hy.know_alpha);
}

int bb_chains_threads(const bb_chains *b) {
    if (b->wide) return wide_chains_threads(b->p);
    return b->tri() ? b->threads : b->packed ? 256 : 512;
}

int bb_chains_set_threads(bb_chains *b, int threads) {
    if (!b->tri() || hipSetDevice(b->proto->cfg.device) != hipSuccess ||
        tri_chains_resident_per_cu(b->proto->n, b->p, threads, !b->proto->hy.know_alpha) < 0) {
        set_error("bb_chains_set_threads: no triangle chain-batch instance of %d threads", threads);
        return -1;
    }
    b->threads = threads;
// ... 868 lines not shown
        print_abort("%s", ex.what());
        *runtime = 0.0;
        return OUT_ERROR;
    }
    std::vector<double> Xd((size_t)n * p, 0.0);
    for (int j = 0; j < p; ++j)
        for (int q = Xcolptr[j]; q < Xcolptr[j + 1]; ++q) Xd[(size_t)j * n + Xrowidx[q]] = Xval[q];
    return dense_call(stable_kind(b), c, yp, Xd.data(), b, out, runtime);
}

Outcome logit_call(bb_config c, const double *yp, const double *Xp, int b, Traces out,
                   double *runtime) {
    c.method = LOGIT;
    for (int i = 0; i < c.n; ++i)
        if (!(yp[i] == 0.0 || yp[i] == 1.0)) {
            print_abort("logistic bridge needs y in {0, 1} (y[%d] = %g)", i, yp[i]);
            *runtime = 0.0;
            return OUT_ERROR;
        }
    std::vector<double> sig2(c.trace_capacity);
    out.sig2 = sig2.data();
    return dense_call(
        stable_kind(b, "Bridge Regression (logistic, Polya-Gamma mix. of normals):"), c, yp, Xp,
        b, out, runtime);
}

CallKind logit_kind(int b) {
    return stable_kind(b, "Bridge Regression (logistic, Polya-Gamma mix. of normals):");
}

bool logit_y_ok(const char *entry, const double *yp, int n) {
    for (int i = 0; i < n; ++i)
        if (!(yp[i] == 0.0 || yp[i] == 1.0)) {
            set_error("%s: logistic bridge needs y in {0, 1} (y[%d] = %g)", entry, i, yp[i]);
            printf("Error: %s\n", g_last_error.c_str());
            fflush(stdout);
            return false;
        }
    return true;
}

bb_config logit_chains_config(const double *nu_shape, const double *nu_rate,
                              const double *alpha_a, const double *alpha_b,
                              const double *true_tau, const double *true_alpha, int p, int n,
                              int m, int nchains) {
    const double zero = 0.0, one = 1.0;
    const int no = 0;
    bb_config c = stable_call_config(&zero, &zero, nu_shape, nu_rate, alpha_a, alpha_b, &one,
                                     true_tau, true_alpha, p, n, m, &no, nchains);
    c.method = LOGIT;
    return c;
}

bool nchains_ok(const char *entry, int nchains) {
    if (nchains >= 1) return true;
    set_error("%s: nchains must be at least 1 (got %d)", entry, nchains);
    printf("Error: %s\n", g_last_error.c_str());
    fflush(stdout);
    return false;
}

bool summary_args_ok(const char *entry, int nsamp, int maxlag) {
    const char *why = TraceSummary::refusal(nsamp, maxlag);
    if (!why) return true;
    set_error("%s: %s (got maxlag %d, %d samples)", entry, why, maxlag, nsamp);
    printf("Error: %s\n", g_last_error.c_str());
    fflush(stdout);
    return false;
}

bb_config tri_call_config(const double *sig2_shape, const double *sig2_scale,
                          const double *nu_shape, const double *nu_rate, const double *alpha_a,
                          const double *alpha_b, const double *true_sig2, const double *true_tau,
                          const double *true_alpha, int p, int n, int m, const int *ortho,
                          const int *betaburn, int nchains = 1) {
    const int no = 0;
    bb_config c = stable_call_config(sig2_shape, sig2_scale, nu_shape, nu_rate, alpha_a, alpha_b,
                                     true_sig2, true_tau, true_alpha, p, n, m, &no, nchains);
    c.method = TRI;
    c.ortho = *ortho != 0;
    c.betaburn = *betaburn > 0 ? *betaburn : 0;
    return c;
}

}

extern "C" {

void bb_set_device_count(int count) { g_max_devices = count < 0 ? 0 : count; }

void bb_set_device_count_C(const int *count) { bb_set_device_count(*count); }
void bb_get_device_count_C(int *count) { *count = g_max_devices; }
void bb_plan_devices_C(const int *n, const int *p, const int *ortho, const int *nvisible,
                       int *devices) {
    bb_config c;
    bb_config_default(&c);
    c.n = *n;
    c.p = *p;
    c.ortho = *ortho != 0;
    *devices = chain_devices(c, *nvisible >= 0 ? *nvisible : -1);
}
void bb_set_device_C(const int *device, int *status) {
    const int rc = bb_set_device(*device);
    if (status) *status = rc;
}
void bb_set_verbose_C(const int *verbose) { bb_set_verbose(*verbose); }
void bb_use_r_rng_C(const int *enable) { bb_use_r_rng(*enable); }
static bool r_count_ok(const char *what, double v) {
    if (std::isfinite(v) && v >= 0.0 && v <= 9007199254740992.0 && v == std::floor(v)) return true;
    set_error("%s: %g is not an integer in [0, 2^53]; ignored", what, v);
    fprintf(stderr, "BayesBridge: %s: %g is not an integer in [0, 2^53]; ignored\n", what, v);
    return false;
}
void bb_set_seed_C(const double *seed) {
    if (r_count_ok("bb_set_seed_C seed", *seed)) bb_set_seed((uint64_t)*seed);
}
void bb_set_rng_state_C(const double *seed, const double *stream) {
    if (r_count_ok("bb_set_rng_state_C seed", *seed) &&
        r_count_ok("bb_set_rng_state_C stream", *stream))
        bb_set_rng_state((uint64_t)*seed, (uint64_t)*stream);
}
void bb_get_rng_state_C(double *seed, double *stream) {
    uint64_t s = 0, t = 0;
    bb_get_rng_state(&s, &t);
    *seed = (double)s;
    *stream = (double)t;
}
void bb_set_trace_budget_C(const double *bytes) {
    if (r_count_ok("bb_set_trace_budget_C bytes", *bytes)) bb_set_trace_budget((long long)*bytes);
}
void bb_last_call_info_C(int *devices, int *trace_capacity, int *interrupted) {
    (void)bb_last_call_info(devices, trace_capacity, interrupted);
}
void bb_debug_fail_member(int member, int sweep) {
    g_debug_fail_sweep = sweep;
    g_debug_fail_member = member;
}

int bb_set_chol_version(int version) {
    if (version == 0) return g_chol_version;
    if (version < 1 || version > 4) return -1;
    g_chol_version = version;
    return 0;
}
int bb_set_tuning(int key, int value) {
    static const struct {
        int key, *var, max;
    } kKeys[] = {{1, &g_oz_res_nt, 2},  {2, &g_bxb_nt, 1},     {3, &g_sp_nt, 3},
                 {6, &g_nid_kmax, 64},  {7, &g_lam_xu, 3},     {8, &g_nid_sync, 2},
                 {9, &g_shard_proto, 1}, {10, &g_nid_mixed, 1}, {11, &g_nid_poll, 1},
                 {12, &g_rs_xcd, 1},    {13, &g_lam_wave, 1},  {15, &g_lam_lend, 1},
                 {17, &g_nid_fold, 2},  {20, &g_bsolve_ll, 1}, {21, &g_chains_packed, 1},
                 {24, &g_nid_b32, 2},   {25, &g_chains_wide, 1}, {26, &g_fused_alpha, 1},
                 {27, &g_fused_tri_alpha, 1}};
    for (const auto &k : kKeys)
        if (k.key == key) {
            const int old = *k.var;
            if (value >= 0) *k.var = std::min(value, k.max);
            return old;
        }
    if (key == 4) {
        const int old = g_lam_occ;
        if (value >= 0) g_lam_occ = value & 15;
        return old;
    }
    if (key == 5) {
        const int old = g_lam_lanes;
        if (value == 0 || value == 4 || value == 8 || value == 16 || value == 32 || value == 64)
            g_lam_lanes = value;
        return old;
    }
    if (key == 16) {
        const int old = g_nid_force_k;
        if (value >= 0) nid_set_force_k(std::min(value, 64));
        return old;
    }
    return -1;
}
void bb_set_trace_budget(long long bytes) {
    g_trace_budget = bytes > 0 ? (size_t)bytes : (size_t(1) << 30);
}
void bb_debug_interrupt_after(int polls) { g_debug_interrupt = polls; }
int bb_last_call_info(int *devices, int *trace_capacity, int *interrupted) {
    if (devices) *devices = g_last_devices;
    if (trace_capacity) *trace_capacity = g_last_capacity;
    if (interrupted) *interrupted = g_last_interrupted;
    return 0;
}

void bridge_reg_stable(double *betap, double *lambdap, double *sig2p, double *taup,
                       double *alphap, const double *yp, const double *Xp,
                       const double *sig2_shape, const double *sig2_scale,
                       const double *nu_shape, const double *nu_rate, const double *alpha_a,
                       const double *alpha_b, const double *true_sig2, const double *true_tau,
                       const double *true_alpha, const int *P, const int *N, const int *M,
                       const int *burn, double *runtime, const int *ortho) {
    const bb_config c = stable_call_config(sig2_shape, sig2_scale, nu_shape, nu_rate, alpha_a,
                                           alpha_b, true_sig2, true_tau, true_alpha, *P, *N, *M,
                                           ortho);
    if (dense_call(stable_kind(*burn), c, yp, Xp, *burn, {betap, lambdap, sig2p, taup, alphap},
                   runtime) == OUT_INTERRUPTED)
        reraise_interrupt();
}

void bridge_reg_stable_chains(double *betap, double *lambdap, double *sig2p, double *taup,
                              double *alphap, const double *yp, const double *Xp,
                              const double *sig2_shape, const double *sig2_scale,
                              const double *nu_shape, const double *nu_rate,
                              const double *alpha_a, const double *alpha_b,
                              const double *true_sig2, const double *true_tau,
                              const double *true_alpha, const int *P, const int *N,
                              const int *M, const int *burn, double *runtime,
                              const int *ortho, const int *nchains) {
    if (!nchains_ok("bridge_reg_stable_chains", *nchains)) return;
    const bb_config c = stable_call_config(sig2_shape, sig2_scale, nu_shape, nu_rate, alpha_a,
                                           alpha_b, true_sig2, true_tau, true_alpha, *P, *N, *M,
                                           ortho, *nchains);
    if (chains_call(stable_kind(*burn), c, *nchains, yp, Xp, *burn,
                    {betap, lambdap, sig2p, taup, alphap}, runtime) == OUT_INTERRUPTED)
        reraise_interrupt();
}

void bridge_reg_stable_chains_summary(double *meanp, double *varp, double *acovp, double *hmeanp,
                                      double *hvarp, int *flagsp, const int *maxlag,
                                      const double *yp, const double *Xp,
                                      const double *sig2_shape, const double *sig2_scale,
                                      const double *nu_shape, const double *nu_rate,
                                      const double *alpha_a, const double *alpha_b,
                                      const double *true_sig2, const double *true_tau,
                                      const double *true_alpha, const int *P, const int *N,
                                      const int *M, const int *burn, double *runtime,
                                      const int *ortho, const int *nchains) {
    const char *entry = "bridge_reg_stable_chains_summary";
    if (!nchains_ok(entry, *nchains) || !summary_args_ok(entry, *M, *maxlag)) return;
    const bb_config c = stable_call_config(sig2_shape, sig2_scale, nu_shape, nu_rate, alpha_a,
                                           alpha_b, true_sig2, true_tau, true_alpha, *P, *N, *M,
                                           ortho, *nchains);
    if (chains_summary_call(entry, stable_kind(*burn), c, *nchains, yp, Xp, *burn,
                            {meanp, varp, acovp, hmeanp, hvarp, flagsp, *maxlag},
                            runtime) == OUT_INTERRUPTED)
        reraise_interrupt();
}

void bridge_reg_stable_csc(double *betap, double *lambdap, double *sig2p, double *taup,
                           double *alphap, const double *yp, const int *Xcolptr,
                           const int *Xrowidx, const double *Xval, const double *sig2_shape,
                           const double *sig2_scale, const double *nu_shape,
                           const double *nu_rate, const double *alpha_a, const double *alpha_b,
                           const double *true_sig2, const double *true_tau,
                           const double *true_alpha, const int *P, const int *N, const int *M,
                           const int *burn, double *runtime, const int *ortho) {
    const bb_config c = stable_call_config(sig2_shape, sig2_scale, nu_shape, nu_rate, alpha_a,
                                           alpha_b, true_sig2, true_tau, true_alpha, *P, *N, *M,
                                           ortho);
    if (stable_csc(c, yp, Xcolptr, Xrowidx, Xval, *burn, {betap, lambdap, sig2p, taup, alphap},
                   runtime) == OUT_INTERRUPTED)
        reraise_interrupt();
}

void bridge_reg_logit(double *betap, double *lambdap, double *taup, double *alphap,
                      const double *yp, const double *Xp, const double *nu_shape,
                      const double *nu_rate, const double *alpha_a, const double *alpha_b,
                      const double *true_tau, const double *true_alpha, const int *P,
                      const int *N, const int *M, const int *burn, double *runtime) {
    const double zero = 0.0, one = 1.0;
    const int no = 0;
    const bb_config c = stable_call_config(&zero, &zero, nu_shape, nu_rate, alpha_a, alpha_b,
                                           &one, true_tau, true_alpha, *P, *N, *M, &no);
    if (logit_call(c, yp, Xp, *burn, {betap, lambdap, nullptr, taup, alphap}, runtime) ==
        OUT_INTERRUPTED)
        reraise_interrupt();
}

void bridge_reg_logit_chains(double *betap, double *lambdap, double *taup, double *alphap,
                             const double *yp, const double *Xp, const double *nu_shape,
                             const double *nu_rate, const double *alpha_a,
                             const double *alpha_b, const double *true_tau,
                             const double *true_alpha, const int *P, const int *N, const int *M,
                             const int *burn, double *runtime, const int *nchains) {
    const char *entry = "bridge_reg_logit_chains";
    if (!nchains_ok(entry, *nchains) || !logit_y_ok(entry, yp, *N)) return;
    const bb_config c = logit_chains_config(nu_shape, nu_rate, alpha_a, alpha_b, true_tau,
                                            true_alpha, *P, *N, *M, *nchains);
    std::vector<double> sig2((size_t)c.trace_capacity * (size_t)*nchains);
    if (chains_call(logit_kind(*burn), c, *nchains, yp, Xp, *burn,
                    {betap, lambdap, sig2.data(), taup, alphap}, runtime) == OUT_INTERRUPTED)
        reraise_interrupt();
}

void bridge_reg_logit_chains_summary(double *meanp, double *varp, double *acovp, double *hmeanp,
                                     double *hvarp, int *flagsp, const int *maxlag,
                                     const double *yp, const double *Xp, const double *nu_shape,
                                     const double *nu_rate, const double *alpha_a,
                                     const double *alpha_b, const double *true_tau,
                                     const double *true_alpha, const int *P, const int *N,
                                     const int *M, const int *burn, double *runtime,
                                     const int *nchains) {
    const char *entry = "bridge_reg_logit_chains_summary";
    if (!nchains_ok(entry, *nchains) || !summary_args_ok(entry, *M, *maxlag) ||
        !logit_y_ok(entry, yp, *N))
        return;
    const bb_config c = logit_chains_config(nu_shape, nu_rate, alpha_a, alpha_b, true_tau,
                                            true_alpha, *P, *N, *M, *nchains);
    if (chains_summary_call(entry, logit_kind(*burn), c, *nchains, yp, Xp, *burn,
                            {meanp, varp, acovp, hmeanp, hvarp, flagsp, *maxlag},
                            runtime) == OUT_INTERRUPTED)
        reraise_interrupt();
// ... 64 lines not shown
```

### bayesbridge_amd/csrc/bb_kernels.h

```cpp
#pragma once
#include <hip/hip_runtime.h>
#include <stddef.h>
#include <stdint.h>

#include <cmath>

namespace bb {

struct Key;

struct DevScalars {
    double tau, sig2, alpha;
    double s_abs_pow;
    double rss;
    double pad[3];
};

struct Hyper {
    double sig2_shape, sig2_scale, nu_shape, nu_rate, alpha_a, alpha_b;
    int know_tau, know_sig2, know_alpha;
};

constexpr int kGramTile = 128;
constexpr int kGramBK = 16;
constexpr int kNB = 64;
constexpr int kXvCols = 256;
constexpr int kXvMinCols = 32;
constexpr int kXvRows = 512;
constexpr int kTriMaxP = 2048;

__host__ __device__ inline size_t tri_index(int r, int c) { return (size_t)c * (c + 1) / 2 + r; }
__host__ __device__ inline size_t tri_count(int n) { return (size_t)n * (n + 1) / 2; }

enum LambdaMode { LAMBDA_ONLY = 0, LAMBDA_WOODBURY = 1 };

struct NidState {
    double eps, theta, delta, sigma1;
    int mode, k2;
    unsigned long long n_cheb, n_products, n_chol;
    double lambda_x;
    double eta;
    unsigned long long n_mixed, n_products32;
    double c64, c32, cstep;
    int b32;
    unsigned long long n_beta32;
};
constexpr double kNidTol = 1.3877787807814457e-17;
constexpr double kBeta32Tol = 1.4901161193847656e-08;

struct ChebConst {
    double theta, delta, sigma1;
};
__host__ __device__ inline ChebConst cheb_const(double eps) {
    ChebConst c;
    c.theta = 1.0 + 0.5 * eps;
    c.delta = 0.5 * eps;
    c.sigma1 = c.delta > 0.0 ? c.theta / c.delta : 0.0;
    return c;
}
__host__ __device__ inline int cheb_iterations(double eps, int kmax, double tol) {
    if (!(eps >= 0.0) || !(eps < 1e300)) return 0;
    if (eps == 0.0) return kmax >= 1 ? 1 : 0;
    const ChebConst c = cheb_const(eps);
    const double lim = sqrt(1.0 + eps) / tol;
    double tm1 = 1.0, tk = c.sigma1;
    for (int k = 1; k <= kmax; ++k) {
        if (tk >= lim) return k;
        const double tn = 2.0 * c.sigma1 * tk - tm1;
        tm1 = tk;
        tk = tn;
    }
    return 0;
}

__host__ __device__ inline double cheb_bound_at(double eps, int k) {
    const ChebConst c = cheb_const(eps);
    double tm1 = 1.0, tk = c.sigma1;
    for (int i = 1; i < k; ++i) {
        const double tn = 2.0 * c.sigma1 * tk - tm1;
        tm1 = tk;
        tk = tn;
    }
    return sqrt(1.0 + eps) / tk;
}

__device__ __forceinline__ bool gated(const int *gate) { return gate && *gate != 0; }

enum KernelFamily { KF_LAMBDA, KF_GRAM, KF_REDUCE, KF_CHOL, KF_SOLVE, KF_BETA, KF_EAPPLY, KF_COUNT };
void note_launch(KernelFamily f, const void *kernel);
const void *launched_instance(int f);

int eapply_parts(int p_loc, int n_pad);
bool eapply_supported(int n_pad);
constexpr int kNidTS = 32;
constexpr int kAllowMixed = 1, kAllowBeta32 = 2, kBeta32AnyCost = 4;
int nid_sum_groups(int p_loc);
void launch_nid_sums(hipStream_t s, const double *D, const double *cn, int p_loc,
                     const DevScalars *sc, NidState *nid, int k_launched, int allow, int decide,
                     double *wg_part, double *red, double *eps_host);
void launch_nid_sums_decide(hipStream_t s, const double *D, const double *cn, int p_loc,
                            const DevScalars *sc, NidState *nid, int k_launched,
                            double *wg_part, double *red, double *host2, int allow_mixed = 0,
                            unsigned long long tag_seq = 0);
void launch_nid_reduce(hipStream_t s, const double *wg_part, int G, const DevScalars *sc,
                       NidState *nid, double *red, int k_launched = 0, double *host2 = nullptr,
                       int allow_mixed = 0, unsigned long long tag_seq = 0);
struct NidFold {
    const double *cn = nullptr;
    double *wg_part = nullptr;
    unsigned int *cnt = nullptr;
    int decide = 0, k_launched = 0, allow_mixed = 0;
    NidState *nid = nullptr;
    double *red = nullptr, *host2 = nullptr;
    unsigned long long tag_seq = 0;
};
void launch_nid_decide_from(hipStream_t s, const double *red, const DevScalars *sc,
                            int k_launched, NidState *nid, double *host2,
                            unsigned long long tag_seq = 0);
void launch_nid_xu(hipStream_t s, const double *X, int ldx, const double *u, int ncols,
                   int n_pad, const NidState *nid, double *part);
void launch_cheb_init(hipStream_t s, const double *xu_part, int nparts, int n, int n_pad,
                      const double *y, const DevScalars *sc, uint64_t k0, uint64_t k1,
                      uint64_t t, const NidState *nid, double *x, double *r, double *d,
                      double *b = nullptr, double *xu = nullptr);
struct Beta32Vecs {
    double *c = nullptr;
    const double *b = nullptr, *xu = nullptr;
    double *xb = nullptr;
};
void launch_cheb_step(hipStream_t s, const double *part, int nparts, int n_pad,
                      const DevScalars *sc, const NidState *nid, int j, double *x, double *r,
                      double *d, int phase = 1, const Beta32Vecs *bv = nullptr);
void launch_cheb_restart(hipStream_t s, const double *part, int nparts, int n_pad,
                         const DevScalars *sc, const NidState *nid, const double *b, double *x,
                         double *r, double *d, const Beta32Vecs *bv = nullptr);
void launch_eapply(hipStream_t s, const double *X, int ldx, int n_pad, int p_loc,
                   const double *D, const double *v, const NidState *nid, int j, double *part,
                   const float *X32 = nullptr, int kind = 0, double *gb = nullptr);
void launch_cast_f32(hipStream_t s, const double *X, int ldx, int n_pad, int ncols, float *X32,
                     int *bad);
constexpr double kU32 = 5.9604644775390625e-08;
void launch_sp_eapply(hipStream_t s, const int *colptr, const int *rowidx, const double *cval,
                      const int *rowptr, const int *colidx, const double *rval, int p_loc,
                      int n_pad, const double *D, const double *v, const NidState *nid, int j,
                      double *scratch_p, double *out);
void launch_part_sum(hipStream_t s, const double *part, int nparts, int n_pad, double *out);
void launch_shift_gram(hipStream_t s, const double *red2, int n_pad, double U, double *M,
                       int ldm);
void launch_sp_nid_xu(hipStream_t s, const int *rowptr, const int *colidx, const double *rval,
                      int n_pad, const double *u, const NidState *nid, double *out);

int stable_group_for(long count);
bool stable_noinline_for(long count);

void launch_retstable_batch(hipStream_t s, double *x, const double *alpha, const double *V0,
                            const double *h, int num, uint64_t k0, uint64_t k1, uint64_t t,
                            int group, uint32_t *err);

bool launch_lambda_pg(hipStream_t s, const double *beta, int p_loc, int p_pad, uint64_t j0,
                      const DevScalars *sc, uint64_t k0, uint64_t k1, uint64_t t, int group,
                      double *lam, double *lam_trace, const double *psi, int n, int n_pad,
                      double *omega, uint32_t *err);
void launch_lambda(hipStream_t s, const double *beta, int p_loc, int p_pad, uint64_t j0,
                   const DevScalars *sc, uint64_t k0, uint64_t k1, uint64_t t, int mode,
                   int group, double *lam, double *D, double *u, double *lam_trace,
                   uint32_t *err);

int lambda_xu_parts(int p_loc, int p_pad, int n_pad);
int launch_lambda_xu(hipStream_t s, const double *beta, int p_loc, int p_pad, uint64_t j0,
                     const DevScalars *sc, uint64_t k0, uint64_t k1, uint64_t t, double *lam,
                     double *D, double *u, double *lam_trace, uint32_t *err, const double *X,
                     int ldx, int n_pad, double *xu_part, unsigned int *sync = nullptr,
                     unsigned int ep = 0, const NidFold *fold = nullptr, int *folded = nullptr);
int launch_lambda_xs(hipStream_t s, const double *beta, int p_loc, int p_pad, uint64_t j0,
                     const DevScalars *sc, uint64_t k0, uint64_t k1, uint64_t t, double *lam,
                     double *D, double *u, double *lam_trace, uint32_t *err, const double *X,
                     int ldx, int n_pad, int nchunk, double *xu_part, unsigned int *sync,
                     unsigned int ep, int ndraw, int nstream, const NidFold *fold);
int lambda_xs_resident(int nr);
int lambda_xs_sync_words(int p_pad);
extern int g_lam_xu;
extern int g_lam_wave;
extern int g_lam_lend;

void launch_lambda_variant(hipStream_t s, const double *beta, int p, const DevScalars *sc,
                           uint64_t k0, uint64_t k1, uint64_t t, int group, int noinline,
                           double *lam, uint32_t *err);

int gram_splits_for(int n_pad, int K);
void launch_gram(hipStream_t s, const double *Y, int ldy, const double *w, int n_pad, int K,
                 int S, double *slabs, int ldo, size_t slab_stride, const int *gate = nullptr);

int xv_chunks(int ncols, int n_pad);
int xv_chunks_max(int ncols);
void launch_xv(hipStream_t s, const double *X, int ldx, const double *v, int ncols, int n_pad,
               double *part, const int *gate = nullptr);

int pre_blocks_s(int p_loc);
void launch_pre(hipStream_t s, const double *part, int nparts, int n_pad, const double *beta,
                int p_loc, const DevScalars *sc, double *red1, int nbS);

void launch_scalars(hipStream_t s, const double *red1, int nbS, const double *y, int n,
                    int p, DevScalars *sc, Hyper hy, uint64_t k0, uint64_t k1, uint64_t t,
                    double *tau_tr, double *sig2_tr, double *alpha_tr, int tau_only,
                    uint32_t *err);

void launch_slab_sum(hipStream_t s, const double *slabs, int S, size_t slab_stride, int n_pad,
                     const double *xu_part, int nxu, double *red2, int packed, const int *gate = nullptr);

void launch_form_m(hipStream_t s, const double *red2, int n, int n_pad, const double *y,
                   const DevScalars *sc, uint64_t k0, uint64_t k1, uint64_t t, double *M,
                   int ldm, int rhs_col, const int *gate = nullptr);

void launch_em_form(hipStream_t s, const double *G, int ldg, const double *dlam, const int *mask,
                    const double *b, int p, int p_pad, double *A, int lda, int rhs_col);
void launch_em_cg(hipStream_t s, const double *A, int lda, int n, const double *b, double *x,
                  double tol, int max_it, double *work, int *out_it);
void launch_em_batch(hipStream_t s, const double *G, int ldg, const double *b, int p,
                     const double *ratios, const double *lambda_max, int count, double alpha,
                     double tol, int max_iter, double *beta_out, int *solves_out);
void launch_em_batch_tiled(hipStream_t s, const double *G, int ldg, const double *b, int p,
                           int p_pad, const double *ratios, const double *lambda_max, int r0,
                           int count, double alpha, double tol, int max_iter, double *scratch,
                           double *vecs, int *masks, double *beta_out, int *solves_out);
int em_tile();
void launch_form_a(hipStream_t s, const double *G, int ldg, const double *lam,
                   const DevScalars *sc, const double *c, int p, int p_pad, double *A, int lda,
                   int rhs_col, int packed = 0);

size_t chol_flag_words(int m_pad, int nrhs_blocks);
extern int g_bsolve_ll;
size_t chol_wd_words(int m_pad);
extern int g_bxb_nt;
extern int g_rs_xcd;
extern int g_nid_force_k;
void nid_set_force_k(int k);
extern int g_lam_occ;
extern int g_lam_lanes;
extern int g_chol_version;
void chol_factor(hipStream_t s, double *A, int lda, int m_pad, int nrhs_blocks, uint32_t *err,
                 double *Wd, unsigned int *flags, unsigned long long *trace = nullptr, const int *gate = nullptr);


void chol_bsolve(hipStream_t s, const double *A, int lda, int m_pad, const double *Wd,
                 double *Y, double *W, int nrhs, unsigned int *flags = nullptr,
                 uint32_t *err = nullptr, const int *gate = nullptr);

void launch_beta_woodbury(hipStream_t s, const double *X, int ldx, int n_pad, const double *w,
                          const double *u, const double *D, const DevScalars *sc, int p_loc,
                          double *beta, double *beta_trace);

int beta_xb_parts(int p_loc);
bool beta_xb_supported(int n_pad);
void launch_beta_woodbury_xb(hipStream_t s, const double *X, int ldx, int n_pad, const double *w,
                             const double *u, const double *D, const DevScalars *sc, int p_loc,
                             double *beta, double *beta_trace, double *part);
void launch_beta_woodbury32(hipStream_t s, const float *X32, int ldx, int n_pad, const double *wd,
                            const double *wc, const double *gb, const double *u, const double *D,
                            const DevScalars *sc, const NidState *nid, int p_loc, double *beta,
                            double *beta_trace);

void launch_chol_rhs(hipStream_t s, const double *A, int lda, int rhs_col, int p, int p_pad,
                     uint64_t k0, uint64_t k1, uint64_t t, double *Y2);

void launch_beta_chol(hipStream_t s, const double *W2, int p_pad, const DevScalars *sc, int p,
                      double *beta, double *beta_trace);

void launch_beta_ortho(hipStream_t s, const double *gdiag, const double *c, const double *lam,
                       const DevScalars *sc, int p, uint64_t j0, uint64_t k0, uint64_t k1,
                       uint64_t t, double *beta, double *beta_trace);

void launch_alpha_mh(hipStream_t s, const double *beta, int p, DevScalars *sc, double pr_a,
                     double pr_b, uint64_t k0, uint64_t k1, uint64_t t, double *alpha_tr);
void launch_alpha_sums(hipStream_t s, const double *beta, int p_loc, const DevScalars *sc,
                       uint64_t k0, uint64_t k1, uint64_t t, double *sums);
void launch_alpha_decide(hipStream_t s, const double *sums, int p, DevScalars *sc, double pr_a,
                         double pr_b, uint64_t k0, uint64_t k1, uint64_t t, double *alpha_tr);

void launch_tri_update(hipStream_t s, double *beta, double *u, double *omega, double *shape,
                       int p, const double *tVc, const double *tVr, const double *a,
                       const double *d, const double *Gf, const double *c, int ortho,
                       const DevScalars *sc, int betaburn, uint64_t k0, uint64_t k1, uint64_t t,
                       double *tr_beta, double *tr_u, double *tr_omega, double *tr_shape,
                       uint32_t *err);

void launch_trunc_batch(hipStream_t s, int mode, int num, double *x, const double *p0,
                        const double *p1, const double *p2, const double *p3, uint64_t k0,
                        uint64_t k1, uint32_t *err);
// ... 95 lines not shown
```

### bayesbridge_amd/csrc/bb_nid.hip

```cpp
#include <hip/hip_runtime.h>

#include <algorithm>
#include <cmath>
#include <mutex>

#include "bb_kernels.h"
#include "bb_sampler.h"
#include "bb_wave.h"

namespace bb {

namespace {

__device__ inline double cheb_rho(double sigma1, int j) {
    double rho = 1.0 / sigma1;
    for (int i = 1; i <= j; ++i) rho = 1.0 / (2.0 * sigma1 - rho);
    return rho;
}

}

constexpr int kNidSumWG = 256;

__device__ __forceinline__ double shard_threshold(double tau2, int k) {
    return ldexp(tau2, 40 - 2 * k);
}

__device__ void nid_plan_mixed(double eps, double tr, int kcap, double cost_fp64,
                               const NidState *nid, int &K1, int &K2, double &eta, double &e2,
                               double &err1_out, double bsave) {
    const int lane = threadIdx.x & 63;
    K1 = K2 = 0;
    err1_out = HUGE_VAL;
    eta = (2.0 * kU32 * sqrt(tr * eps) + kU32 * kU32 * tr) * (1.0 + 1e-6);
    e2 = eps + eta;
    if (!(e2 < 1e300) || kcap < 1) return;
    const ChebConst c = cheb_const(e2);
    const int kmax = kcap < 64 ? kcap : 64;
    const double ac = acosh(c.sigma1);
    const double tk = (lane + 1 <= kmax) ? sqrt(1.0 + e2) / cosh((lane + 1) * ac) * (1.0 + 1e-12)
                                         : HUGE_VAL;
    const double step32 = nid->c32 + nid->cstep, step64 = nid->c64 + nid->cstep;
    const double cap = (kcap - 1) * step64;
    const int k1 = lane + 1;
    const double err1 = eta + tk * (1.0 + eta);
    const double need = kNidTol / err1;
    int lo = 1, hi = kmax + 1;
#pragma unroll
    for (int it = 0; it < 7; ++it) {
        const int mid = (lo + hi) >> 1;
        const double t2 = __shfl(tk, (mid < kmax ? mid : kmax) - 1, 64);
        if (lo < hi) {
            if (eta + t2 * (1.0 + eta) <= need)
                hi = mid;
            else
                lo = mid + 1;
        }
    }
    const int k2 = lo <= kmax ? lo : 0;
    double cost = (k1 <= kmax && err1 < 1.0 && k2)
                      ? (k1 - 1) * step32 + step64 + (k2 - 1) * step32
                      : HUGE_VAL;
    if (!(cost < cap * (1.0 - 1e-9))) cost = HUGE_VAL;
    if (err1 * (1.0 + 1e-6) <= kBeta32Tol) cost -= bsave;
    if (!(cost < cost_fp64 * (1.0 - 1e-9))) cost = HUGE_VAL;
    double bc = cost;
    int bk1 = k1, bk2 = k2;
#pragma unroll
    for (int o = 32; o > 0; o >>= 1) {
        const double oc = __shfl_xor(bc, o, 64);
        const int ok1 = __shfl_xor(bk1, o, 64), ok2 = __shfl_xor(bk2, o, 64);
        if (oc < bc || (oc == bc && ok1 < bk1)) {
            bc = oc;
            bk1 = ok1;
            bk2 = ok2;
        }
    }
    const double be = __shfl(err1, (bk1 - 1) & 63, 64);
    if (bc < HUGE_VAL) {
        K1 = bk1;
        K2 = bk2;
        err1_out = be;
    }
}

__device__ int g_dev_nid_force_k = 0;
int g_nid_force_k = 0;
void nid_set_force_k(int k) {
    g_nid_force_k = k;
    (void)hipMemcpyToSymbol(HIP_SYMBOL(g_dev_nid_force_k), &k, sizeof(int));
}

__device__ __forceinline__ double round_up_12(double x) {
    if (!(x > 0.0 && x < HUGE_VAL)) return x;
    constexpr unsigned long long m = (1ull << 40) - 1;
    unsigned long long b = (unsigned long long)__double_as_longlong(x);
    if (b & m) b = (b | m) + 1;
    return __longlong_as_double((long long)b);
}

__device__ void nid_finish(const double *red, const DevScalars *sc, int k_launched, int allow,
                           NidState *nid, double *eps_host, double *mode_host,
                           int allow_mixed = 0, double *k2_host = nullptr,
                           unsigned long long tag_seq = 0) {
    const double tau2 = sc->tau * sc->tau;
    const double lam = red[kNidTS + 1];
    double best = red[kNidTS];
    if (lam > 0.0 && lam < HUGE_VAL)
        for (int k = 0; k < kNidTS; ++k)
            best = fmin(best, red[k] + shard_threshold(tau2, k) * lam);
    const double eps = round_up_12(best / sc->sig2 * (1.0 + 1e-6));
    int K = cheb_iterations(eps, k_launched, kNidTol);
    if (g_dev_nid_force_k > 0) K = g_dev_nid_force_k < k_launched ? g_dev_nid_force_k : k_launched;
    int mode = (allow && K > 0) ? K : 0, k2 = 0;
    double ecb = eps, eta = 0.0, err1 = HUGE_VAL;
    const bool b32_pays = (allow_mixed & kAllowBeta32) && g_dev_nid_force_k == 0 &&
                          ((allow_mixed & kBeta32AnyCost) || nid->c64 - nid->c32 > nid->cstep);
    const double bsave = b32_pays ? nid->c64 - nid->c32 : 0.0;
    if (allow && (allow_mixed & kAllowMixed) && g_dev_nid_force_k == 0 && (K == 0 || K > 2)) {
        const double tr = round_up_12(red[kNidTS] / sc->sig2 * (1.0 + 1e-6));
        int k1m, k2m;
        double e2;
        nid_plan_mixed(eps, tr, k_launched,
                       K > 0 ? (K - 1) * (nid->c64 + nid->cstep) - bsave : HUGE_VAL, nid, k1m,
                       k2m, eta, e2, err1, bsave);
        if (k2m > 0) {
            mode = k1m;
            k2 = k2m;
            ecb = e2;
        } else {
            eta = 0.0;
        }
    }
    if ((threadIdx.x & 63) != 0) return;
    int b32 = 0;
    if (b32_pays && mode > 0) {
        double bound = HUGE_VAL;
        if (k2 > 0)
            bound = err1;
        else if (mode >= 2 && eps > 0.0)
            bound = cheb_bound_at(eps, mode) + cheb_bound_at(eps, mode - 1);
        b32 = bound * (1.0 + 1e-6) <= kBeta32Tol;
    }
    nid->eps = eps;
    nid->mode = mode;
    nid->k2 = k2;
    nid->b32 = b32;
    nid->n_beta32 += (unsigned long long)b32;
    nid->eta = eta;
    const ChebConst c = cheb_const(ecb);
    nid->theta = c.theta;
    nid->delta = c.delta;
    nid->sigma1 = c.sigma1;
    if (mode && k2) {
        nid->n_cheb += 1;
        nid->n_mixed += 1;
        nid->n_products += 1ull;
        nid->n_products32 += (unsigned long long)(mode - 1 + k2 - 1);
    } else if (mode) {
        nid->n_cheb += 1;
        nid->n_products += (unsigned long long)(mode - 1);
    } else {
        nid->n_chol += 1;
    }
    if (eps_host) *eps_host = eps;
    if (mode_host) *mode_host = (double)mode;
    if (k2_host) *k2_host = (double)(k2 + 128 * b32);
    if (tag_seq && mode_host)
        __hip_atomic_store((unsigned long long *)(mode_host + 2),
                           (tag_seq << 16) | ((unsigned long long)mode << 8) |
                               (unsigned)(k2 | (b32 << 7)),
                           __ATOMIC_RELAXED, __HIP_MEMORY_SCOPE_SYSTEM);
}

__global__ __launch_bounds__(kNidSumWG) void k_nid_sums(const double *__restrict__ D,
                                                        const double *__restrict__ cn, int p_loc,
                                                        const DevScalars *sc,
                                                        double *__restrict__ wg_part) {
    __shared__ double part[kNidSumWG / 64][kNidTS + 1];
    __shared__ double thr[kNidTS];
    const int lane = threadIdx.x & 63, wid = threadIdx.x >> 6;
    const double tau2 = sc->tau * sc->tau;
    if (threadIdx.x < kNidTS) thr[threadIdx.x] = shard_threshold(tau2, threadIdx.x);
    __syncthreads();
    double acc[kNidTS + 1];
#pragma unroll
    for (int k = 0; k <= kNidTS; ++k) acc[k] = 0.0;
    for (int j = blockIdx.x * kNidSumWG + threadIdx.x; j < p_loc; j += gridDim.x * kNidSumWG) {
        const double dj = D[j], v = dj * cn[j];
        acc[kNidTS] += v;
#pragma unroll
        for (int k = 0; k < kNidTS; ++k)
            if (dj > thr[k]) acc[k] += v;
    }
#pragma unroll
    for (int k = 0; k <= kNidTS; ++k) acc[k] = wave_sum_all(acc[k]);
    if (lane == 0)
#pragma unroll
        for (int k = 0; k <= kNidTS; ++k) part[wid][k] = acc[k];
    __syncthreads();
    if (threadIdx.x <= kNidTS) {
        double s = 0.0;
        for (int w = 0; w < kNidSumWG / 64; ++w) s += part[w][threadIdx.x];
        wg_part[(size_t)blockIdx.x * (kNidTS + 1) + threadIdx.x] = s;
    }
}

constexpr int kNidRedQ = 8;
template <bool WT>
__device__ __forceinline__ void nid_reduce_body(const double *__restrict__ wg_part, int G,
                                                const DevScalars *sc, int k_launched, int allow,
                                                int decide, NidState *nid,
                                                double *__restrict__ red, double *eps_host,
                                                int allow_mixed, unsigned long long tag_seq) {
    __shared__ double pq[kNidRedQ][kNidTS + 1];
    __shared__ double r[kNidTS + 2];
    auto ld = [&](size_t i) {
        return WT ? __hip_atomic_load(&wg_part[i], __ATOMIC_RELAXED, __HIP_MEMORY_SCOPE_AGENT)
                  : wg_part[i];
    };
    const int t = threadIdx.x;
    for (int tt = t; tt < kNidRedQ * (kNidTS + 1); tt += blockDim.x) {
        const int k = tt % (kNidTS + 1), q = tt / (kNidTS + 1);
        double a[4] = {0.0, 0.0, 0.0, 0.0};
        int b = q;
        for (; b + 3 * kNidRedQ < G; b += 4 * kNidRedQ)
#pragma unroll
            for (int u = 0; u < 4; ++u) a[u] += ld((size_t)(b + u * kNidRedQ) * (kNidTS + 1) + k);
        for (; b < G; b += kNidRedQ) a[0] += ld((size_t)b * (kNidTS + 1) + k);
        pq[q][k] = (a[0] + a[1]) + (a[2] + a[3]);
    }
    __syncthreads();
    if (t <= kNidTS) {
        double s = 0.0;
#pragma unroll
        for (int q = 0; q < kNidRedQ; ++q) s += pq[q][t];
        r[t] = s;
        red[t] = s;
    }
    if (t == kNidTS + 1) {
        const double lam = nid->lambda_x;
        const double v = lam > 0.0 ? lam : HUGE_VAL;
        r[t] = v;
        red[t] = v;
    }
    __syncthreads();
    if (decide && t < 64)
        nid_finish(r, sc, k_launched, allow, nid, eps_host, decide == 2 ? eps_host + 1 : nullptr,
                   decide == 2 ? allow_mixed : 0, decide == 2 ? eps_host + 2 : nullptr,
                   decide == 2 ? tag_seq : 0ull);
}
__global__ __launch_bounds__(64 * 5) void k_nid_reduce(const double *__restrict__ wg_part, int G,
                                                       const DevScalars *sc, int k_launched,
                                                       int allow, int decide, NidState *nid,
                                                       double *__restrict__ red,
                                                       double *eps_host, int allow_mixed,
                                                       unsigned long long tag_seq) {
    nid_reduce_body<false>(wg_part, G, sc, k_launched, allow, decide, nid, red, eps_host,
                           allow_mixed, tag_seq);
}

__global__ __launch_bounds__(64) void k_nid_decide_from(const double *__restrict__ red,
                                                        const DevScalars *sc, int k_launched,
                                                        NidState *nid, double *host2,
                                                        unsigned long long tag_seq) {
    nid_finish(red, sc, k_launched, 1, nid, host2, host2 + 1, 0, host2 + 2, tag_seq);
}

constexpr int kRedWaves = 16;
__device__ __forceinline__ double part_rowsum(const double *__restrict__ part, int nparts,
                                              int n_pad, int row, double (*red)[64]) {
    const int lane = threadIdx.x & 63, wid = threadIdx.x >> 6;
    double a[8];
#pragma unroll
    for (int u = 0; u < 8; ++u) a[u] = 0.0;
    if (row < n_pad) {
        int q = wid;
        for (; q + 7 * kRedWaves < nparts; q += 8 * kRedWaves)
#pragma unroll
            for (int u = 0; u < 8; ++u) a[u] += part[(size_t)(q + u * kRedWaves) * n_pad + row];
        for (; q < nparts; q += kRedWaves) a[0] += part[(size_t)q * n_pad + row];
    }
    red[wid][lane] = ((a[0] + a[1]) + (a[2] + a[3])) + ((a[4] + a[5]) + (a[6] + a[7]));
    __syncthreads();
    double s = 0.0;
    if (wid == 0)
#pragma unroll
        for (int w = 0; w < kRedWaves; ++w) s += red[w][lane];
    return s;
}

constexpr int kRsThreads = 1024;
template <int RW>
__device__ __forceinline__ double part_rowsum_rw(const double *__restrict__ part, int nparts,
                                                 int n_pad, int row0) {
    constexpr int S = kRsThreads / RW, G2 = S < 8 ? S : 8;
    __shared__ double red[S][RW];
    __shared__ double red2[G2][RW];
    const int r = threadIdx.x % RW, sl = threadIdx.x / RW;
    const int row = row0 + r;
    double a[8] = {0.0, 0.0, 0.0, 0.0, 0.0, 0.0, 0.0, 0.0};
    if (row < n_pad) {
        int q = sl;
        for (; q + 7 * S < nparts; q += 8 * S)
#pragma unroll
            for (int u = 0; u < 8; ++u) a[u] += part[(size_t)(q + u * S) * n_pad + row];
        for (; q < nparts; q += S) a[0] += part[(size_t)q * n_pad + row];
    }
    red[sl][r] = ((a[0] + a[1]) + (a[2] + a[3])) + ((a[4] + a[5]) + (a[6] + a[7]));
    __syncthreads();
    if ((int)threadIdx.x < G2 * RW) {
        const int g = threadIdx.x / RW;
        double v = 0.0;
#pragma unroll
        for (int k = 0; k < S / G2; ++k) v += red[g * (S / G2) + k][r];
        red2[g][r] = v;
    }
    __syncthreads();
    double v = 0.0;
    if ((int)threadIdx.x < RW)
#pragma unroll
        for (int g = 0; g < G2; ++g) v += red2[g][r];
    return v;
}

__device__ __forceinline__ int rs_block(int xcd) {
    const int G = (int)gridDim.x, b = (int)blockIdx.x;
    if (!xcd || (G & 7)) return b;
    return (b & 7) * (G >> 3) + (b >> 3);
}

int g_rs_xcd = 1;
static int rowsum_rw(int nparts) { return nparts >= 128 ? 8 : 64; }

template <int RW>
__global__ __launch_bounds__(kRsThreads) void k_cheb_init(
    const double *__restrict__ xu_part, int nparts, int n, int n_pad,
    const double *__restrict__ y, const DevScalars *sc, Key key, uint64_t t, const NidState *nid,
    double *x, double *r, double *d, double *b, double *xu_out, int xcd) {
    if (nid->mode == 0) return;
    const int i = rs_block(xcd) * RW + (int)threadIdx.x;
    const double xu = part_rowsum_rw<RW>(xu_part, nparts, n_pad, rs_block(xcd) * RW);
    if ((int)threadIdx.x >= RW || i >= n_pad) return;
    double rhs = 0.0;
    if (i < n) {
        const double sig = sqrt(sc->sig2);
        const double delta = normal_at(key, t, KIND_DELTA, (uint64_t)i);
        rhs = y[i] / sig - (xu / sig + delta);
    }
    const double d0 = rhs / nid->theta;
    r[i] = rhs;
    d[i] = d0;
    x[i] = d0;
    if (b) b[i] = rhs;
    if (xu_out) xu_out[i] = xu;
}

__device__ __forceinline__ void beta32_xb(const Beta32Vecs &bv, const DevScalars *sc, int i,
                                          double w) {
    bv.xb[i] = bv.xu[i] + sqrt(sc->sig2) * (bv.b[i] - w);
}

template <int RW>
__global__ __launch_bounds__(kRsThreads) void k_cheb_step(
    const double *__restrict__ part, int nparts, int n_pad, const DevScalars *sc,
    const NidState *nid, int j, double *x, double *r, double *d, int phase, int xcd,
    Beta32Vecs bv) {
    if ((phase == 1 ? nid->mode : nid->k2) <= j) return;
    const int i = rs_block(xcd) * RW + (int)threadIdx.x;
    const double e = part_rowsum_rw<RW>(part, nparts, n_pad, rs_block(xcd) * RW);
    if ((int)threadIdx.x >= RW || i >= n_pad) return;
    const double dv = d[i];
    const double qv = dv + e / sc->sig2;
    const double rv = r[i] - qv;
    const double s1 = nid->sigma1;
    const double rho0 = cheb_rho(s1, j - 1), rho1 = 1.0 / (2.0 * s1 - rho0);
    const double dn = rho1 * rho0 * dv + (2.0 * rho1 / nid->delta) * rv;
    r[i] = rv;
    d[i] = dn;
    const double xn = x[i] + dn;
    x[i] = xn;
    if (bv.c) {
        if (phase == 2) bv.c[i] += dn;
        const bool last = phase == 2 ? j == nid->k2 - 1 : (nid->k2 == 0 && j == nid->mode - 1);
        if (last && nid->b32) beta32_xb(bv, sc, i, xn);
    }
}

template <int RW>
__global__ __launch_bounds__(kRsThreads) void k_cheb_restart(
    const double *__restrict__ part, int nparts, int n_pad, const DevScalars *sc,
    const NidState *nid, const double *__restrict__ b, double *x, double *r, double *d, int xcd,
    Beta32Vecs bv) {
    if (nid->k2 == 0 || nid->mode == 0) return;
    const int i = rs_block(xcd) * RW + (int)threadIdx.x;
    const double e = part_rowsum_rw<RW>(part, nparts, n_pad, rs_block(xcd) * RW);
    if ((int)threadIdx.x >= RW || i >= n_pad) return;
    const double xv = x[i];
    const double rv = b[i] - (xv + e / sc->sig2);
    const double dv = rv / nid->theta;
    r[i] = rv;
    d[i] = dv;
    x[i] = xv + dv;
    if (bv.c) {
        bv.c[i] = dv;
        if (nid->k2 == 1 && nid->b32) beta32_xb(bv, sc, i, xv + dv);
    }
}

__global__ __launch_bounds__(64 * kRedWaves) void k_part_sum(const double *__restrict__ part,
                                                             int nparts, int n_pad,
                                                             double *__restrict__ out) {
    __shared__ double red[kRedWaves][64];
    const int i = blockIdx.x * 64 + (threadIdx.x & 63);
    const double v = part_rowsum(part, nparts, n_pad, i, red);
    if (threadIdx.x < 64 && i < n_pad) out[i] = v;
}

__global__ __launch_bounds__(256) void k_shift_gram(const double *__restrict__ red2, int n_pad,
                                                    double U, double *__restrict__ M, int ldm) {
    const size_t idx = (size_t)blockIdx.x * 256 + threadIdx.x;
    if (idx >= tri_count(n_pad)) return;
    int c = (int)((sqrt(8.0 * (double)idx + 1.0) - 1.0) * 0.5);
    while ((size_t)c * (c + 1) / 2 > idx) --c;
    while ((size_t)(c + 1) * (c + 2) / 2 <= idx) ++c;
    const int r = (int)(idx - (size_t)c * (c + 1) / 2);
    M[(size_t)r + (size_t)c * ldm] = (r == c ? U : 0.0) - red2[idx];
}

constexpr int kEaCols = 8;
constexpr int kEaThreads = 256;

template <int NR, bool XU, typename T, bool BANK = false>
__device__ __forceinline__ void eapply_body(const T *__restrict__ X, int ldx, int n_pad,
                                            int p_loc, const double *__restrict__ D,
                                            const double *__restrict__ v,
                                            double *__restrict__ part, double *gb = nullptr,
                                            bool gacc = false) {
    __shared__ double ws[4][kEaCols];
    const int tid = threadIdx.x, lane = tid & 63, wid = tid >> 6;
    double vr[NR], acc[NR];
#pragma unroll
    for (int m = 0; m < NR; ++m) {
        const int row = tid + kEaThreads * m;
        vr[m] = (!XU && row < n_pad) ? v[row] : 0.0;
        acc[m] = 0.0;
    }
    const int nchunk = (p_loc + kEaCols - 1) / kEaCols;
    for (int ch = blockIdx.x; ch < nchunk; ch += gridDim.x) {
        const int c0 = ch * kEaCols;
        T raw[kEaCols][NR];
        if (c0 + kEaCols <= p_loc && NR * kEaThreads <= n_pad) {
#pragma unroll
            for (int c = 0; c < kEaCols; ++c)
#pragma unroll
                for (int m = 0; m < NR; ++m)
                    raw[c][m] = __builtin_nontemporal_load(X + (size_t)(c0 + c) * ldx +
                                                           tid + kEaThreads * m);
        } else {
#pragma unroll
            for (int c = 0; c < kEaCols; ++c) {
                const bool ok = c0 + c < p_loc;
                const T *col = X + (size_t)(c0 + c) * ldx;
#pragma unroll
                for (int m = 0; m < NR; ++m) {
                    const int row = tid + kEaThreads * m;
                    raw[c][m] = (ok && row < n_pad) ? __builtin_nontemporal_load(col + row) : T(0);
                }
            }
        }
        double gold = 0.0;
        if constexpr (BANK)
            if (gb && gacc && tid < kEaCols && c0 + tid < p_loc) gold = gb[c0 + tid];
        double xv[kEaCols][NR];
#pragma unroll
        for (int c = 0; c < kEaCols; ++c)
#pragma unroll
            for (int m = 0; m < NR; ++m) xv[c][m] = (double)raw[c][m];
        if constexpr (XU) {
#pragma unroll
            for (int c = 0; c < kEaCols; ++c) {
                const double f = (c0 + c < p_loc) ? D[c0 + c] : 0.0;
#pragma unroll
                for (int m = 0; m < NR; ++m) acc[m] = __builtin_fma(xv[c][m], f, acc[m]);
            }
            continue;
        }
        double s[kEaCols];
#pragma unroll
        for (int c = 0; c < kEaCols; ++c) {
            double a = 0.0;
#pragma unroll
            for (int m = 0; m < NR; ++m) a = __builtin_fma(xv[c][m], vr[m], a);
            s[c] = wave_sum_all(a);
        }
        __syncthreads();
        if (lane == 0)
#pragma unroll
            for (int c = 0; c < kEaCols; ++c) ws[wid][c] = s[c];
        __syncthreads();
        double mine = 0.0;
#pragma unroll
        for (int c = 0; c < kEaCols; ++c) {
            const double dc = (c0 + c < p_loc) ? D[c0 + c] : 0.0;
            const double sc = ((ws[0][c] + ws[1][c]) + ws[2][c]) + ws[3][c];
            if constexpr (BANK)
                if (c == tid) mine = sc;
            const double f = dc * sc;
#pragma unroll
            for (int m = 0; m < NR; ++m) acc[m] = __builtin_fma(xv[c][m], f, acc[m]);
        }
        if constexpr (BANK)
            if (gb && tid < kEaCols && c0 + tid < p_loc) gb[c0 + tid] = gold + mine;
    }
#pragma unroll
    for (int m = 0; m < NR; ++m) {
        const int row = tid + kEaThreads * m;
        if (row < n_pad) part[(size_t)blockIdx.x * n_pad + row] = acc[m];
    }
}

template <int NR, int KIND>
__global__ __launch_bounds__(kEaThreads) void k_eapply(const double *__restrict__ X,
                                                       const float *__restrict__ X32, int ldx,
                                                       int n_pad, int p_loc,
                                                       const double *__restrict__ D,
                                                       const double *__restrict__ v,
                                                       const NidState *nid, int j,
                                                       double *__restrict__ part,
                                                       double *__restrict__ gb) {
    if constexpr (KIND == 1) {
        if (nid->mode == 0) return;
        eapply_body<NR, true, double>(X, ldx, n_pad, p_loc, D, v, part);
    } else if constexpr (KIND == 0) {
        if (nid->mode <= j) return;
        if (X32 && nid->k2 > 0)
            eapply_body<NR, false, float>(X32, ldx, n_pad, p_loc, D, v, part);
        else
            eapply_body<NR, false, double, true>(X, ldx, n_pad, p_loc, D, v, part,
                                                 (gb && nid->b32) ? gb : nullptr, j > 1);
    } else if constexpr (KIND == 2) {
        if (nid->k2 == 0 || nid->mode == 0) return;
        eapply_body<NR, false, double, true>(X, ldx, n_pad, p_loc, D, v, part,
                                             (gb && nid->b32) ? gb : nullptr, false);
    } else {
        if (nid->k2 <= j) return;
        eapply_body<NR, false, float>(X32, ldx, n_pad, p_loc, D, v, part);
    }
}

__global__ __launch_bounds__(256) void k_cast_f32(const double *__restrict__ X, int ldx,
                                                  int n_pad, int ncols, float *__restrict__ X32,
                                                  int *bad) {
    const size_t tot = (size_t)n_pad * ncols;
    bool b = false;
    for (size_t e = (size_t)blockIdx.x * 256 + threadIdx.x; e < tot; e += (size_t)gridDim.x * 256) {
        const size_t c = e / n_pad, r = e % n_pad;
        const double x = X[c * ldx + r];
        const double ax = fabs(x);
        b |= !(ax <= 0x1p126) || (ax != 0.0 && ax < 0x1p-125);
        X32[c * ldx + r] = (float)x;
    }
    if (__any(b) && (threadIdx.x & 63) == 0) atomicOr(bad, 1);
}

constexpr int kSpEaLanes = 16;

__global__ __launch_bounds__(256) void k_sp_eapply_cols(const int *__restrict__ colptr,
                                                        const int *__restrict__ rowidx,
                                                        const double *__restrict__ cval,
                                                        int p_loc, const double *__restrict__ D,
                                                        const double *__restrict__ v,
                                                        const NidState *nid, int j,
                                                        double *__restrict__ s) {
    if (nid->mode <= j) return;
    const long gid = (long)blockIdx.x * 256 + threadIdx.x;
    const int c = (int)(gid / kSpEaLanes);
    const int q = (int)(gid % kSpEaLanes);
    double a = 0.0;
    if (c < p_loc)
        for (int k = colptr[c] + q; k < colptr[c + 1]; k += kSpEaLanes) a += cval[k] * v[rowidx[k]];
#pragma unroll
    for (int o = kSpEaLanes / 2; o > 0; o >>= 1) a += __shfl_xor(a, o, 64);
    if (q == 0 && c < p_loc) s[c] = D[c] * a;
}

__global__ __launch_bounds__(256) void k_sp_eapply_rows(const int *__restrict__ rowptr,
                                                        const int *__restrict__ colidx,
                                                        const double *__restrict__ rval,
                                                        int n_pad, const double *__restrict__ s,
                                                        const NidState *nid, int j, int pol,
                                                        double *__restrict__ out) {
    if (pol == 0 ? nid->mode <= j : nid->mode == 0) return;
    const int lane = threadIdx.x & 63;
    const int row = blockIdx.x * 4 + (threadIdx.x >> 6);
    if (row >= n_pad) return;
    double a = 0.0;
    for (int k = rowptr[row] + lane; k < rowptr[row + 1]; k += 64) a += rval[k] * s[colidx[k]];
    a = wave_sum_all(a);
    if (lane == 0) out[row] = a;
}

static int nid_cus() {
    static int n = [] {
        int dev = 0, v = 0;
        (void)hipGetDevice(&dev);
        if (hipDeviceGetAttribute(&v, hipDeviceAttributeMultiprocessorCount, dev) != hipSuccess ||
            v <= 0)
            v = 256;
        return v;
    }();
    return n;
}

int eapply_parts(int p_loc, int n_pad) {
    (void)n_pad;
    const int nchunk = (p_loc + kEaCols - 1) / kEaCols;
    return std::max(1, std::min(nchunk, 2 * nid_cus()));
}

bool eapply_supported(int n_pad) { return n_pad <= 16 * kEaThreads; }


int nid_sum_groups(int p_loc) { return std::max(1, std::min(256, (p_loc + 255) / 256)); }

void launch_nid_sums(hipStream_t s, const double *D, const double *cn, int p_loc,
                     const DevScalars *sc, NidState *nid, int k_launched, int allow, int decide,
                     double *wg_part, double *red, double *eps_host) {
    const int G = nid_sum_groups(p_loc);
    k_nid_sums<<<G, kNidSumWG, 0, s>>>(D, cn, p_loc, sc, wg_part);
    k_nid_reduce<<<1, 64 * 5, 0, s>>>(wg_part, G, sc, k_launched, allow, decide, nid, red,
                                  eps_host, 0, 0ull);
}

void launch_nid_sums_decide(hipStream_t s, const double *D, const double *cn, int p_loc,
                            const DevScalars *sc, NidState *nid, int k_launched,
                            double *wg_part, double *red, double *host2, int allow_mixed,
                            unsigned long long tag_seq) {
    const int G = nid_sum_groups(p_loc);
    k_nid_sums<<<G, kNidSumWG, 0, s>>>(D, cn, p_loc, sc, wg_part);
    k_nid_reduce<<<1, 64 * 5, 0, s>>>(wg_part, G, sc, k_launched, 1, 2, nid, red, host2,
                                      allow_mixed, tag_seq);
}

void launch_nid_reduce(hipStream_t s, const double *wg_part, int G, const DevScalars *sc,
                       NidState *nid, double *red, int k_launched, double *host2,
                       int allow_mixed, unsigned long long tag_seq) {
    if (host2)
        k_nid_reduce<<<1, 64 * 5, 0, s>>>(wg_part, G, sc, k_launched, 1, 2, nid, red, host2,
                                          allow_mixed, tag_seq);
    else
        k_nid_reduce<<<1, 64 * 5, 0, s>>>(wg_part, G, sc, 0, 0, 0, nid, red, nullptr, 0, 0ull);
}

void launch_nid_decide_from(hipStream_t s, const double *red, const DevScalars *sc,
                            int k_launched, NidState *nid, double *host2,
                            unsigned long long tag_seq) {
    k_nid_decide_from<<<1, 64, 0, s>>>(red, sc, k_launched, nid, host2, tag_seq);
}

template <int KIND>
static void launch_pass(hipStream_t s, const double *X, const float *X32, int ldx, int n_pad,
                        int p_loc, const double *D, const double *v, const NidState *nid, int j,
                        double *part, double *gb = nullptr) {
    const int g = eapply_parts(p_loc, n_pad);
    const int nr = (n_pad + kEaThreads - 1) / kEaThreads;
    auto *kern = nr <= 1 ? k_eapply<1, KIND> : nr <= 2 ? k_eapply<2, KIND>
               : nr <= 4 ? k_eapply<4, KIND> : nr <= 8 ? k_eapply<8, KIND> : k_eapply<16, KIND>;
    if (KIND == 0) note_launch(KF_EAPPLY, (const void *)kern);
    kern<<<g, kEaThreads, 0, s>>>(X, X32, ldx, n_pad, p_loc, D, v, nid, j, part, gb);
}

void launch_nid_xu(hipStream_t s, const double *X, int ldx, const double *u, int ncols,
                   int n_pad, const NidState *nid, double *part) {
    launch_pass<1>(s, X, nullptr, ldx, n_pad, ncols, u, nullptr, nid, 0, part);
}

void launch_cheb_init(hipStream_t s, const double *xu_part, int nparts, int n, int n_pad,
                      const double *y, const DevScalars *sc, uint64_t k0, uint64_t k1,
                      uint64_t t, const NidState *nid, double *x, double *r, double *d,
                      double *b, double *xu) {
    if (rowsum_rw(nparts) == 8)
        k_cheb_init<8><<<(n_pad + 7) / 8, kRsThreads, 0, s>>>(xu_part, nparts, n, n_pad, y, sc,
                                                              Key{k0, k1}, t, nid, x, r, d, b,
                                                              xu, g_rs_xcd);
    else
        k_cheb_init<64><<<(n_pad + 63) / 64, kRsThreads, 0, s>>>(xu_part, nparts, n, n_pad, y,
                                                                 sc, Key{k0, k1}, t, nid, x, r, d,
                                                                 b, xu, g_rs_xcd);
}

void launch_cheb_step(hipStream_t s, const double *part, int nparts, int n_pad,
                      const DevScalars *sc, const NidState *nid, int j, double *x, double *r,
                      double *d, int phase, const Beta32Vecs *bv) {
    const Beta32Vecs v = bv ? *bv : Beta32Vecs{};
    if (rowsum_rw(nparts) == 8)
        k_cheb_step<8><<<(n_pad + 7) / 8, kRsThreads, 0, s>>>(part, nparts, n_pad, sc, nid, j, x,
                                                              r, d, phase, g_rs_xcd, v);
    else
        k_cheb_step<64><<<(n_pad + 63) / 64, kRsThreads, 0, s>>>(part, nparts, n_pad, sc, nid, j,
                                                                 x, r, d, phase, g_rs_xcd, v);
}

void launch_cheb_restart(hipStream_t s, const double *part, int nparts, int n_pad,
                         const DevScalars *sc, const NidState *nid, const double *b, double *x,
                         double *r, double *d, const Beta32Vecs *bv) {
    const Beta32Vecs v = bv ? *bv : Beta32Vecs{};
    if (rowsum_rw(nparts) == 8)
        k_cheb_restart<8><<<(n_pad + 7) / 8, kRsThreads, 0, s>>>(part, nparts, n_pad, sc, nid, b,
                                                                 x, r, d, g_rs_xcd, v);
    else
        k_cheb_restart<64><<<(n_pad + 63) / 64, kRsThreads, 0, s>>>(part, nparts, n_pad, sc, nid,
                                                                    b, x, r, d, g_rs_xcd, v);
}

void launch_eapply(hipStream_t s, const double *X, int ldx, int n_pad, int p_loc,
                   const double *D, const double *v, const NidState *nid, int j, double *part,
                   const float *X32, int kind, double *gb) {
    switch (kind) {
        case 2: launch_pass<2>(s, X, X32, ldx, n_pad, p_loc, D, v, nid, j, part, gb); break;
        case 3: launch_pass<3>(s, X, X32, ldx, n_pad, p_loc, D, v, nid, j, part); break;
        default: launch_pass<0>(s, X, X32, ldx, n_pad, p_loc, D, v, nid, j, part, gb); break;
    }
}

void launch_cast_f32(hipStream_t s, const double *X, int ldx, int n_pad, int ncols, float *X32,
                     int *bad) {
    const size_t tot = (size_t)n_pad * ncols;
    const unsigned g = (unsigned)std::min<size_t>((tot + 255) / 256, 4096);
    k_cast_f32<<<g, 256, 0, s>>>(X, ldx, n_pad, ncols, X32, bad);
}

void launch_sp_eapply(hipStream_t s, const int *colptr, const int *rowidx, const double *cval,
                      const int *rowptr, const int *colidx, const double *rval, int p_loc,
                      int n_pad, const double *D, const double *v, const NidState *nid, int j,
                      double *scratch_p, double *out) {
    const long threads = (long)p_loc * kSpEaLanes;
    k_sp_eapply_cols<<<(unsigned)((threads + 255) / 256), 256, 0, s>>>(colptr, rowidx, cval,
                                                                       p_loc, D, v, nid, j,
                                                                       scratch_p);
    k_sp_eapply_rows<<<(n_pad + 3) / 4, 256, 0, s>>>(rowptr, colidx, rval, n_pad, scratch_p,
                                                     nid, j, 0, out);
}

void launch_part_sum(hipStream_t s, const double *part, int nparts, int n_pad, double *out) {
    k_part_sum<<<(n_pad + 63) / 64, 64 * kRedWaves, 0, s>>>(part, nparts, n_pad, out);
}

void launch_shift_gram(hipStream_t s, const double *red2, int n_pad, double U, double *M,
                       int ldm) {
    const size_t tot = tri_count(n_pad);
    k_shift_gram<<<(unsigned)((tot + 255) / 256), 256, 0, s>>>(red2, n_pad, U, M, ldm);
}

void launch_sp_nid_xu(hipStream_t s, const int *rowptr, const int *colidx, const double *rval,
                      int n_pad, const double *u, const NidState *nid, double *out) {
    k_sp_eapply_rows<<<(n_pad + 3) / 4, 256, 0, s>>>(rowptr, colidx, rval, n_pad, u, nid, 0, 1,
                                                     out);
}

__device__ __noinline__ void nid_fold_decide(const double *wg_part, int S, const DevScalars *sc,
                                             int k_launched, int allow_mixed, NidState *nid,
                                             double *red, double *host2,
                                             unsigned long long tag_seq) {
    nid_reduce_body<true>(wg_part, S, sc, k_launched, 1, 2, nid, red, host2, allow_mixed,
                          tag_seq);
}

template <int NR>
__device__ __forceinline__ void lambda_xs_body(const double *beta, int p_loc, int p_pad,
                                               uint64_t j0, const DevScalars *sc, Key key,
                                               uint64_t t, double *lam, double *D, double *u,
                                               double *lam_trace, uint32_t *err,
                                               const double *__restrict__ X, int ldx, int n_pad,
                                               int nchunk, double *__restrict__ xu_part,
                                               unsigned int *sync, unsigned int ep, int ndraw,
                                               NidFold fold) {
    constexpr int C = 32;
    const int tid = threadIdx.x;
    unsigned int *ctr = sync + nchunk;
    if ((int)blockIdx.x < ndraw) {
        __shared__ int claim;
        const double tau = sc->tau;
        for (;;) {
            if (tid == 0)
                claim = (int)__hip_atomic_fetch_add(ctr, 1u, __ATOMIC_RELAXED,
                                                    __HIP_MEMORY_SCOPE_AGENT);
            __syncthreads();
            const int ch = claim;
            __syncthreads();
            if (ch >= nchunk) {
                if (tid == 0 && ch == nchunk + ndraw - 1)
                    __hip_atomic_store(ctr, 0u, __ATOMIC_RELAXED, __HIP_MEMORY_SCOPE_AGENT);
                return;
            }
            const int i = ch * C + tid / 8;
            const bool active = i < p_loc;
            const double b = active ? beta[i] : 0.0;
            const double x = stable_wave_draw(active, b * b / (tau * tau), 0.5 * sc->alpha, 1.0,
                                              key, t, j0 + (uint64_t)i, err);
            if ((tid % 8) == 0) {
                double uv = 0.0;
                if (active) {
                    const double l = 2 * x;
                    lam[i] = l;
                    if (lam_trace) lam_trace[i] = l;
                    const double d = (tau * tau) / l;
                    __hip_atomic_store(&D[i], d, __ATOMIC_RELAXED, __HIP_MEMORY_SCOPE_AGENT);
                    uv = sqrt(d) * normal_at(key, t, KIND_BETA_Z, j0 + (uint64_t)i);
                } else if (i < p_pad) {
                    lam[i] = 1.0;
                    __hip_atomic_store(&D[i], 0.0, __ATOMIC_RELAXED, __HIP_MEMORY_SCOPE_AGENT);
                }
                if (i < p_pad)
                    __hip_atomic_store(&u[i], uv, __ATOMIC_RELAXED, __HIP_MEMORY_SCOPE_AGENT);
            }
            asm volatile("s_waitcnt vmcnt(0)" ::: "memory");
            __syncthreads();
            if (tid == 0) __hip_atomic_store(&sync[ch], ep, __ATOMIC_RELAXED, __HIP_MEMORY_SCOPE_AGENT);
        }
    }
    const int sidx = (int)blockIdx.x - ndraw, S = (int)gridDim.x - ndraw;
    __shared__ double us[8];
    const bool sums = fold.wg_part != nullptr;
    const double nthr = sums ? shard_threshold(sc->tau * sc->tau, tid & 31) : 0.0;
    double nacc = 0.0, ntr = 0.0;
    double a[NR];
#pragma unroll
    for (int m = 0; m < NR; ++m) a[m] = 0.0;
    const int nunit = nchunk * 4;
    int have = -1;
    for (int q = sidx; q < nunit; q += S) {
        const int ch = q >> 2, c0 = ch * C + (q & 3) * 8;
        if (ch != have) {
            if (tid == 0) {
                const uint64_t t0 = __builtin_amdgcn_s_memrealtime();
                while (__hip_atomic_load(&sync[ch], __ATOMIC_RELAXED, __HIP_MEMORY_SCOPE_AGENT) !=
                       ep) {
                    __builtin_amdgcn_s_sleep(2);
                    if (__builtin_amdgcn_s_memrealtime() - t0 > 200000000ull) {
                        atomicOr(err, 16u);
                        break;
                    }
                }
            }
            have = ch;
        }
        __syncthreads();
        double ndv = 0.0, ncv = 0.0;
        if (sums && c0 + (tid >> 5) < p_loc) {
            ndv = __hip_atomic_load(&D[c0 + (tid >> 5)], __ATOMIC_RELAXED, __HIP_MEMORY_SCOPE_AGENT);
            ncv = fold.cn[c0 + (tid >> 5)];
        }
        if (tid < 8)
            us[tid] = c0 + tid < p_pad ? __hip_atomic_load(&u[c0 + tid], __ATOMIC_RELAXED,
                                                           __HIP_MEMORY_SCOPE_AGENT)
                                       : 0.0;
        __syncthreads();
        if (sums) {
            const double v = ndv * ncv;
            if (ndv > nthr) nacc += v;
            ntr += v;
        }
        constexpr int CB = NR >= 16 ? 2 : 4;
#pragma unroll
        for (int cb = 0; cb < 8; cb += CB) {
// ... 98 lines not shown
```

### include/bayesbridge.h

```cpp
#ifndef BAYESBRIDGE_AMD_H
#define BAYESBRIDGE_AMD_H

#include <stdint.h>
#include <stddef.h>

#ifdef __cplusplus
extern "C" {
#endif


void bridge_reg_stable(double *betap, double *lambdap, double *sig2p, double *taup,
                       double *alphap, const double *yp, const double *Xp,
                       const double *sig2_shape, const double *sig2_scale,
                       const double *nu_shape, const double *nu_rate, const double *alpha_a,
                       const double *alpha_b, const double *true_sig2, const double *true_tau,
                       const double *true_alpha, const int *P, const int *N, const int *M,
                       const int *burn, double *runtime, const int *ortho);

void retstable_LD(double *x, double *alpha, double *V0, double *h, int *num);

void bridge_EM(double *betap, const double *yp, const double *Xp, const double *ratio,
               const double *alpha, const int *P, const int *N, const double *lambda_max,
               const double *tol, int *max_iter, const int *use_cg);

// ... 105 lines not shown
                  int mcmc_phase);
int bb_chains_sync(bb_chains *b);
int bb_chains_get_trace(bb_chains *b, int chain, int slot0, int count, double *beta,
                        double *lambda, double *sig2, double *tau, double *alpha);
int bb_chains_get_state(bb_chains *b, int chain, double *beta, double *lambda, double *tau,
                        double *sig2, double *alpha);
int bb_chains_set_state(bb_chains *b, int chain, const double *beta, double tau, double sig2,
                        double alpha);
unsigned bb_chains_error_flags(bb_chains *b, int chain);
int bb_chains_get_tri_trace(bb_chains *b, int chain, int slot0, int count, double *u,
                            double *shape);
int bb_chains_set_tri_state(bb_chains *b, int chain, const double *u);
int bb_chains_get_tri_basis(bb_chains *b, double *tV, double *a, double *d);
int bb_chains_get_omega(bb_chains *b, int chain, double *omega);
int bb_chains_threads(const bb_chains *b);
int bb_chains_set_threads(bb_chains *b, int threads);

void bridge_reg_stable_chains(double *betap, double *lambdap, double *sig2p, double *taup,
                              double *alphap, const double *yp, const double *Xp,
                              const double *sig2_shape, const double *sig2_scale,
                              const double *nu_shape, const double *nu_rate,
                              const double *alpha_a, const double *alpha_b,
                              const double *true_sig2, const double *true_tau,
                              const double *true_alpha, const int *P, const int *N,
                              const int *M, const int *burn, double *runtime,
                              const int *ortho, const int *nchains);

void bridge_regression_chains(double *betap, double *up, double *omegap, double *shapep,
                              double *sig2p, double *taup, double *alphap, const double *yp,
                              const double *Xp, const double *sig2_shape,
                              const double *sig2_scale, const double *nu_shape,
                              const double *nu_rate, const double *alpha_a,
                              const double *alpha_b, const double *true_sig2,
                              const double *true_tau, const double *true_alpha, const int *P,
                              const int *N, const int *M, const int *burn, double *runtime,
                              const int *ortho, const int *betaburn, const int *use_hmc,
                              const int *nchains);

void bridge_reg_logit_chains(double *betap, double *lambdap, double *taup, double *alphap,
                             const double *yp, const double *Xp, const double *nu_shape,
                             const double *nu_rate, const double *alpha_a,
                             const double *alpha_b, const double *true_tau,
                             const double *true_alpha, const int *P, const int *N, const int *M,
                             const int *burn, double *runtime, const int *nchains);

int bb_chains_summary_reset(bb_chains *b, int nsamp, int maxlag);
int bb_chains_summary_add(bb_chains *b, int slot0, int count, int s0);
int bb_chains_summary_get(bb_chains *b, double *mean, double *var, double *acov, double *hmean,
                          double *hvar, int *flags);

void bridge_reg_stable_chains_summary(double *meanp, double *varp, double *acovp, double *hmeanp,
                                      double *hvarp, int *flagsp, const int *maxlag,
                                      const double *yp, const double *Xp,
                                      const double *sig2_shape, const double *sig2_scale,
                                      const double *nu_shape, const double *nu_rate,
                                      const double *alpha_a, const double *alpha_b,
                                      const double *true_sig2, const double *true_tau,
                                      const double *true_alpha, const int *P, const int *N,
                                      const int *M, const int *burn, double *runtime,
                                      const int *ortho, const int *nchains);
void bridge_reg_logit_chains_summary(double *meanp, double *varp, double *acovp, double *hmeanp,
                                     double *hvarp, int *flagsp, const int *maxlag,
                                     const double *yp, const double *Xp, const double *nu_shape,
                                     const double *nu_rate, const double *alpha_a,
                                     const double *alpha_b, const double *true_tau,
                                     const double *true_alpha, const int *P, const int *N,
                                     const int *M, const int *burn, double *runtime,
                                     const int *nchains);
void bridge_regression_chains_summary(double *meanp, double *varp, double *acovp, double *hmeanp,
                                      double *hvarp, int *flagsp, const int *maxlag,
                                      const double *yp, const double *Xp,
                                      const double *sig2_shape, const double *sig2_scale,
                                      const double *nu_shape, const double *nu_rate,
                                      const double *alpha_a, const double *alpha_b,
                                      const double *true_sig2, const double *true_tau,
                                      const double *true_alpha, const int *P, const int *N,
                                      const int *M, const int *burn, double *runtime,
                                      const int *ortho, const int *betaburn, const int *use_hmc,
                                      const int *nchains);

typedef struct bb_group bb_group;
int bb_trunc_batch(int mode, int num, double *x, const double *p0, const double *p1,
                   const double *p2, const double *p3, uint64_t seed, uint64_t stream);

int bb_pg_batch(double *omega, const double *psi, int n, uint64_t seed, uint64_t stream,
                uint64_t t);

int bb_rrtgamma_batch(int num, double *x, const double *shape, const double *rate,
                      const double *right_t, uint64_t seed, uint64_t stream);

int bb_engine_get_tri_trace(bb_engine *e, int slot0, int count, double *u, double *shape);
int bb_engine_get_tri_basis(bb_engine *e, double *tV, double *a, double *d);
int bb_engine_set_tri_state(bb_engine *e, const double *u);

int bb_group_create(bb_engine **engines, int count, bb_group **out);
int bb_group_create_rccl(bb_engine **engines, int count, bb_group **out);
void bb_group_destroy(bb_group *g);
int bb_group_init_state(bb_group *g);
int bb_group_run(bb_group *g, uint64_t t0, int count, int first_slot, int slot_step,
                 int mcmc_phase);
int bb_group_sync(bb_group *g);

void bb_set_device_count(int count);
int bb_set_chol_version(int version);
void bb_set_trace_budget(long long bytes);
int bb_set_tuning(int key, int value);
void bb_debug_interrupt_after(int polls);
int bb_last_call_info(int *devices, int *trace_capacity, int *interrupted);
void bb_debug_fail_member(int member, int sweep);

void bb_set_device_count_C(const int *count);
void bb_get_device_count_C(int *count);
void bb_plan_devices_C(const int *n, const int *p, const int *ortho, const int *nvisible,
                       int *devices);
void bb_set_device_C(const int *device, int *status);
void bb_set_verbose_C(const int *verbose);
void bb_use_r_rng_C(const int *enable);
void bb_set_seed_C(const double *seed);
void bb_set_rng_state_C(const double *seed, const double *stream);
void bb_get_rng_state_C(double *seed, double *stream);
void bb_set_trace_budget_C(const double *bytes);
void bb_last_call_info_C(int *devices, int *trace_capacity, int *interrupted);

int bb_engine_method(const bb_engine *e);
int bb_engine_get_omega(bb_engine *e, double *omega);
int bb_engine_gram_mode(const bb_engine *e);

int bb_engine_enable_timing(bb_engine *e, int enable);
int bb_engine_set_timed_phase(bb_engine *e, int phase);
int bb_engine_set_timing_stride(bb_engine *e, int stride);
int bb_engine_kernel_times(bb_engine *e, double *gram_ms_avg, double *sweep_ms_avg,
                           int *samples);
int bb_engine_reset_timing(bb_engine *e);
int bb_engine_phase_times(bb_engine *e, double *ms, int cap, int *samples);
int bb_phase_count(void);
const char *bb_phase_name(int i);

int bb_engine_nid_bound(bb_engine *e, double *lambda_x, int *kmax);
int bb_engine_timed_brackets(bb_engine *e, int *count);
int bb_engine_nid_stats(bb_engine *e, unsigned long long *cheb_sweeps,
                        unsigned long long *products, unsigned long long *chol_sweeps,
                        double *eps, int *mode);

int bb_engine_launch_counts(bb_engine *e, unsigned long long *lambda_xu,
                            unsigned long long *lambda_alone);

int bb_kernel_instance(const char *phase, char *buf, int len);

int bb_engine_nid_mixed(bb_engine *e, unsigned long long *mixed_sweeps,
                        unsigned long long *products32, double *eta, int *k2, int *holds_x32);

int bb_engine_nid_beta32(bb_engine *e, unsigned long long *beta32_sweeps, int *b32);

int bb_engine_error_flags(bb_engine *e, uint32_t *flags);


int bb_retstable_batch(double *x, const double *alpha, const double *V0, const double *h,
                       int num, uint64_t seed, uint64_t stream, uint64_t t, int group);

int bb_sample_lambda(double *lambda, const double *beta, int p, double alpha, double tau,
                     uint64_t seed, uint64_t stream, uint64_t t, uint64_t j0, int group);

int bb_bench_lambda(const double *beta, int p, double alpha, double tau, int group,
                    int noinline, int reps, double *ms_avg, double *lambda_out);

int bb_bench_chol(int m, int reps, double *ms_factor, double *ms_solve,
                  unsigned long long *trace);

int bb_gram(double *C, const double *Y, const double *w, int n, int k);

int bb_trace_summary(const double *x, int K, int M, int Q, int maxlag, int chunk, double *mean,
                     double *var, double *acov, double *hmean, double *hvar);

int bb_bench_ozaki(int n, int k, int nsplit, int dbg, int reps, double *ms);

int bb_gram_ozaki(double *C, const double *Y, const double *w, int n, int k);

int bb_sparse_gram(double *C, double *xu, const int *colptr, const int *rowidx, const double *val,
                   const double *D, const double *u, int n, int p);
int bb_bench_sparse_gram(const int *colptr, const int *rowidx, const double *val, const double *D,
                         int n, int p, int reps, double *ms_gram, double *ms_rows,
                         long long *pairs);

int bb_chol_solve(double *x, const double *A, const double *b, int m, int nrhs);

int bb_bridge_em(double *beta, const double *y, const double *X, int n, int p, double ratio,
                 double alpha, double lambda_max, double tol, int max_iter, int use_cg);

int bb_bridge_em_batch(double *beta, int *solves, const double *y, const double *X, int n,
                       int p, const double *ratios, const double *lambda_max, int count,
                       double alpha, double tol, int max_iter);
void bb_set_em_scratch_budget(long long bytes);

#ifdef __cplusplus
}
#endif

#endif
```

Measured before the change: 1337 sweeps/s.

## Size second Chebyshev stage from measured restart residual instead of worst-case bound

Adds a residual-aware planning path for the mixed-precision near-identity Chebyshev solve. The restart kernel now accumulates the squared residual norm, and a new single-block kernel compares it with the right-hand-side norm. That ratio sets the second-stage iteration count and decides whether the beta32 shortcut applies, replacing an a-priori bound. If the measured ratio cannot meet tolerance, the code falls back to a redo path that adopts the precomputed fallback plan and reinitialises the iteration. This aims to cut fp64 correction steps at the cost of an extra host-device tag handshake, a small reduction kernel and occasional full redo.

```diff
diff --git a/bayesbridge_amd/__init__.py b/bayesbridge_amd/__init__.py
--- a/bayesbridge_amd/__init__.py
+++ b/bayesbridge_amd/__init__.py
@@ -140,6 +140,7 @@
     L.bb_kernel_instance.argtypes = [c.c_char_p, c.c_char_p, c.c_int]
     L.bb_engine_nid_mixed.argtypes = [c.c_void_p, u64p, u64p, _dp, _ip, _ip]
     L.bb_engine_nid_beta32.argtypes = [c.c_void_p, u64p, _ip]
+    L.bb_engine_nid_resid.argtypes = [c.c_void_p, u64p, u64p, _dp]
     L.bb_group_destroy.argtypes = [c.c_void_p]
     L.bb_group_init_state.argtypes = [c.c_void_p]
     L.bb_group_run.argtypes = [c.c_void_p, c.c_uint64, c.c_int, c.c_int, c.c_int, c.c_int]
@@ -1275,7 +1276,13 @@
         library().bb_engine_nid_bound(self._h, ctypes.byref(lam), ctypes.byref(kmax))
         return dict(cheb_sweeps=a.value, products=b.value, chol_sweeps=c.value, eps=eps.value,
                     mode=mode.value, lambda_x=lam.value, kmax=kmax.value,
-                    beta32_sweeps=self._beta32()[0])
+                    beta32_sweeps=self._beta32()[0], redo_sweeps=self._resid()[1])
+
+    def _resid(self):
+        a, b, r = ctypes.c_ulonglong(), ctypes.c_ulonglong(), ctypes.c_double()
+        _check(library().bb_engine_nid_resid(self._h, ctypes.byref(a), ctypes.byref(b),
+                                             ctypes.byref(r)), "bb_engine_nid_resid")
+        return a.value, b.value, r.value
 
     def _beta32(self):
         a, f = ctypes.c_ulonglong(), ctypes.c_int()
@@ -1290,8 +1297,10 @@
                                              ctypes.byref(eta), ctypes.byref(k2),
                                              ctypes.byref(hx)), "bb_engine_nid_mixed")
         n32, last32 = self._beta32()
+        nres, nredo, ratio = self._resid()
         return dict(mixed_sweeps=a.value, products32=b.value, eta=eta.value, k2=k2.value,
-                    holds_x32=bool(hx.value), beta32_sweeps=n32, beta32=last32)
+                    holds_x32=bool(hx.value), beta32_sweeps=n32, beta32=last32,
+                    resid_sweeps=nres, redo_sweeps=nredo, resid_ratio=ratio)
 
     def launch_counts(self):
         a, b = ctypes.c_ulonglong(), ctypes.c_ulonglong()
diff --git a/bayesbridge_amd/csrc/bb_engine.cpp b/bayesbridge_amd/csrc/bb_engine.cpp
--- a/bayesbridge_amd/csrc/bb_engine.cpp
+++ b/bayesbridge_amd/csrc/bb_engine.cpp
@@ -79,6 +79,7 @@
 int g_nid_poll = 1;
 int g_nid_fold = 1;
 int g_nid_b32 = 1;
+int g_nid_resid = 1;
 int g_chains_packed = 0;
 int g_chains_wide = 0;
 int g_fused_alpha = 0;
@@ -140,6 +141,10 @@
     int nid_k2 = 0;
     double *gb = nullptr, *ch_c = nullptr, *ch_xu = nullptr;
     bool nid_b32 = false;
+    double *nid_sq = nullptr;
+    int nid_sqn = 0;
+    bool nid_resid = false;
+    unsigned long long nid_kseq = 0;
     double nid_cost[3] = {0.0, 0.0, 0.0};
     int ea_parts = 1;
     int nid_kmax = 0;
@@ -226,9 +231,16 @@
         return X32 != nullptr && g_nid_mixed && !sharded() && !group_member && dense();
     }
     bool b32_ok() const { return gb != nullptr && g_nid_b32 && mixed_ok() && nid_sync(); }
+    bool resid_ok() const {
+        return nid_sq != nullptr && g_nid_resid && g_nid_poll && mixed_ok() && nid_sync() &&
+               (g_nid_resid >= 2 || nid_cost[1] > 4.0 * nid_cost[2]);
+    }
     int allow_mask() const {
         return (mixed_ok() ? kAllowMixed : 0) |
-               (b32_ok() ? kAllowBeta32 | (g_nid_b32 == 2 ? kBeta32AnyCost : 0) : 0);
+               (b32_ok() ? kAllowBeta32 | (g_nid_b32 == 2 ? kBeta32AnyCost : 0) : 0) |
+               (resid_ok() ? kAllowResid | (g_nid_resid >= 2 ? kResidAnyCost : 0) |
+                                 (std::max(g_nid_resid - 2, 0) << kResidPhiShift)
+                           : 0);
     }
     double *bank() const { return b32_ok() ? gb : nullptr; }
     Beta32Vecs b32_vecs() const {
@@ -330,9 +342,11 @@
         int mode, k2;
         if (g_nid_poll) {
             const unsigned long long tag = wait_tag(nid_dseq);
-            mode = (int)((tag >> 8) & 0xff);
+            mode = (int)((tag >> 8) & 0x7f);
+            nid_resid = ((tag >> 15) & 1) != 0;
             k2 = (int)(tag & 0xff);
         } else {
+            nid_resid = false;
             wait_event(nid_sev);
             mode = (int)((volatile double *)eps_host)[kNidRing + 1];
             k2 = (int)((volatile double *)eps_host)[kNidRing + 2];
@@ -344,12 +358,12 @@
         nid_last = mode;
         return mode;
     }
-    unsigned long long wait_tag(unsigned long long seq) {
-        const unsigned long long *tp = (const unsigned long long *)(eps_host + kNidRing + 3);
-        const unsigned long long want = seq & 0xffffffffffffull;
+    unsigned long long wait_tag(unsigned long long seq, int slot = 3, int shift = 16) {
+        const unsigned long long *tp = (const unsigned long long *)(eps_host + kNidRing + slot);
+        const unsigned long long want = seq & (~0ull >> shift);
         for (long spin = 0;; ++spin) {
             const unsigned long long v = __atomic_load_n(tp, __ATOMIC_ACQUIRE);
-            if ((v >> 16) == want) return v;
+            if ((v >> shift) == want) return v;
             if ((spin & 1023) != 1023) {
                 __builtin_ia32_pause();
                 continue;
@@ -359,7 +373,7 @@
             const hipError_t q = hipStreamQuery(stream);
             if (q == hipSuccess) {
                 const unsigned long long w = __atomic_load_n(tp, __ATOMIC_ACQUIRE);
-                if ((w >> 16) == want) return w;
+                if ((w >> shift) == want) return w;
                 throw HipError("near-identity decision tag not written by the drained stream");
             }
             if (q != hipErrorNotReady) HIPCHECK(q);
@@ -398,9 +412,11 @@
         else
             launch_cheb_init(stream, nid_xu, xu_fused ? xu_fused : ea_parts, n, n_pad, y, sc,
                              cfg.seed, cfg.stream, t, nid, w, ch_r, ch_d,
-                             mixed_ok() ? ch_b : nullptr, b32_ok() ? ch_xu : nullptr);
+                             mixed_ok() ? ch_b : nullptr, b32_ok() ? ch_xu : nullptr,
+                             resid_ok() ? nid_sq : nullptr);
     }
     void nidx_mixed_tail(int k2) {
+        if (nid_resid) return nidx_resid_tail();
         const Beta32Vecs bv = b32_vecs();
         mark(PH_EAPPLY);
         launch_eapply(stream, X, n_pad, n_pad, p_loc, D, w, nid, 0, ea_part, X32, 2, bank());
@@ -413,6 +429,43 @@
             launch_cheb_step(stream, ea_part, ea_parts, n_pad, sc, nid, j, w, ch_r, ch_d, 2,
                              &bv);
         }
+    }
+    void nidx_resid_tail() {
+        const Beta32Vecs bv = b32_vecs();
+        const int gb_ = cheb_sq_parts(n_pad, xu_fused ? xu_fused : ea_parts);
+        const int gr_ = cheb_sq_parts(n_pad, ea_parts);
+        mark(PH_EAPPLY);
+        launch_eapply(stream, X, n_pad, n_pad, p_loc, D, w, nid, 0, ea_part, X32, 2, bank());
+        mark(PH_NID);
+        launch_cheb_restart(stream, ea_part, ea_parts, n_pad, sc, nid, ch_b, w, ch_r, ch_d, &bv,
+                            nid_sq + nid_sqn);
+        launch_nid_k2(stream, nid_sq, gb_, nid_sq + nid_sqn, gr_, std::min(g_nid_kmax, nid_kmax),
+                      sc, nid, &bv, w, n_pad,
+                      (unsigned long long *)(eps_dev + kNidRing + 4), ++nid_kseq);
+        auto correction = [&](int j) {
+            mark(PH_EAPPLY);
+            launch_eapply(stream, X, n_pad, n_pad, p_loc, D, ch_d, nid, j, ea_part, X32, 3);
+            mark(PH_NID);
+            launch_cheb_step(stream, ea_part, ea_parts, n_pad, sc, nid, j, w, ch_r, ch_d, 2,
+                             &bv);
+        };
+        correction(1);
+        const unsigned long long tag = wait_tag(nid_kseq, 4, 24);
+        const int mode = (int)((tag >> 8) & 0xff), k2 = (int)(tag & 0x7f);
+        nid_b32 = b32_ok() && (tag & 128) != 0;
+        nid_k2 = k2;
+        nid_last = mode;
+        nid_resid = false;
+        if (((tag >> 16) & 1) == 0) {
+            for (int j = 2; j < k2; ++j) correction(j);
+            return;
+        }
+        launch_nid_redo(stream, nid, ch_b, n_pad, w, ch_r, ch_d);
+        for (int j = 1; j < mode; ++j) {
+            nidx_eapply(j);
+            nidx_step(j);
+        }
+        if (k2 > 0) nidx_mixed_tail(k2);
     }
     void nidx_eapply(int j) {
         mark(PH_EAPPLY);
@@ -992,6 +1045,13 @@
     HIPCHECK(hipMemcpyAsync(&e->nid->lambda_x, &lam, sizeof(double), hipMemcpyHostToDevice, s));
     HIPCHECK(hipMemcpyAsync(&e->nid->c64, e->nid_cost, sizeof(e->nid_cost), hipMemcpyHostToDevice,
                             s));
+    std::vector<double> hcn(e->p_loc);
+    HIPCHECK(hipMemcpyAsync(hcn.data(), e->cn, hcn.size() * sizeof(double), hipMemcpyDeviceToHost,
+                            s));
+    HIPCHECK(hipStreamSynchronize(s));
+    double scn = 0.0;
+    for (double v : hcn) scn += v;
+    HIPCHECK(hipMemcpyAsync(&e->nid->sum_cn, &scn, sizeof(double), hipMemcpyHostToDevice, s));
     HIPCHECK(hipStreamSynchronize(s));
     e->lambda_x = lam;
     (void)hipFree(ones);
@@ -1130,11 +1190,12 @@
             e->nid_wg = dalloc<double>(
                 (size_t)std::max(nid_sum_groups(c.p_local), 1024) * (kNidTS + 1), o);
             e->nid_sum = dalloc<double>(n_pad, o);
-            const int nh = bb_engine::kNidRing + 4;
+            const int nh = bb_engine::kNidRing + 5;
             HIPCHECK(hipHostMalloc((void **)&e->eps_host, nh * sizeof(double),
                                    hipHostMallocMapped | hipHostMallocCoherent));
             for (int q = 0; q < nh; ++q) e->eps_host[q] = -1.0;
             *(unsigned long long *)(e->eps_host + bb_engine::kNidRing + 3) = 0ull;
+            *(unsigned long long *)(e->eps_host + bb_engine::kNidRing + 4) = 0ull;
             HIPCHECK(hipHostGetDevicePointer((void **)&e->eps_dev, e->eps_host, 0));
             e->nid_kmax = e->nid_kmax_model();
             if (e->dense() && c.world == 1 && g_nid_mixed && e->nid_kmax > 0) {
@@ -1156,6 +1217,10 @@
                     } else {
                         o.push_back(x32);
                         e->X32 = (float *)x32;
+                        e->nid_sqn = (n_pad + 7) / 8;
+                        e->nid_sq = dalloc<double>(2 * (size_t)e->nid_sqn, o);
+                        HIPCHECK(hipMemsetAsync(e->nid_sq, 0, 2 * sizeof(double) * e->nid_sqn,
+                                                e->stream));
                         if (beta_xb_supported(n_pad)) {
                             e->gb = dalloc<double>(p_pad, o);
                             e->ch_c = dalloc<double>(n_pad, o);
@@ -1917,6 +1982,20 @@
     });
 }
 
+int bb_engine_nid_resid(bb_engine *e, unsigned long long *resid_sweeps,
+                        unsigned long long *redo_sweeps, double *ratio) {
+    return guarded([&] {
+        NidState h{};
+        if (e->nid) {
+            HIPCHECK(hipMemcpyAsync(&h, e->nid, sizeof(h), hipMemcpyDeviceToHost, e->stream));
+            HIPCHECK(hipStreamSynchronize(e->stream));
+        }
+        if (resid_sweeps) *resid_sweeps = h.n_resid;
+        if (redo_sweeps) *redo_sweeps = h.n_redo;
+        if (ratio) *ratio = h.ratio;
+    });
+}
+
 int bb_engine_nid_bound(bb_engine *e, double *lambda_x, int *kmax) {
     if (lambda_x) *lambda_x = e->lambda_x;
     if (kmax) *kmax = e->nid ? std::min(g_nid_kmax, e->nid_kmax) : -1;
@@ -3091,7 +3170,7 @@
                  {12, &g_rs_xcd, 1},    {13, &g_lam_wave, 1},  {15, &g_lam_lend, 1},
                  {17, &g_nid_fold, 2},  {20, &g_bsolve_ll, 1}, {21, &g_chains_packed, 1},
                  {24, &g_nid_b32, 2},   {25, &g_chains_wide, 1}, {26, &g_fused_alpha, 1},
-                 {27, &g_fused_tri_alpha, 1}};
+                 {27, &g_fused_tri_alpha, 1}, {29, &g_nid_resid, 8}};
     for (const auto &k : kKeys)
         if (k.key == key) {
             const int old = *k.var;
diff --git a/bayesbridge_amd/csrc/bb_kernels.h b/bayesbridge_amd/csrc/bb_kernels.h
--- a/bayesbridge_amd/csrc/bb_kernels.h
+++ b/bayesbridge_amd/csrc/bb_kernels.h
@@ -44,6 +44,9 @@
     double c64, c32, cstep;
     int b32;
     unsigned long long n_beta32;
+    int resid, fb_mode, fb_k2, fb_b32;
+    double theta2, delta2, sigma12, e2, fb_eta, sum_cn, ratio;
+    unsigned long long n_resid, n_redo;
 };
 constexpr double kNidTol = 1.3877787807814457e-17;
 constexpr double kBeta32Tol = 1.4901161193847656e-08;
@@ -94,6 +97,7 @@
 bool eapply_supported(int n_pad);
 constexpr int kNidTS = 32;
 constexpr int kAllowMixed = 1, kAllowBeta32 = 2, kBeta32AnyCost = 4;
+constexpr int kAllowResid = 8, kResidAnyCost = 16, kResidPhiShift = 8;
 int nid_sum_groups(int p_loc);
 void launch_nid_sums(hipStream_t s, const double *D, const double *cn, int p_loc,
                      const DevScalars *sc, NidState *nid, int k_launched, int allow, int decide,
@@ -122,7 +126,7 @@
 void launch_cheb_init(hipStream_t s, const double *xu_part, int nparts, int n, int n_pad,
                       const double *y, const DevScalars *sc, uint64_t k0, uint64_t k1,
                       uint64_t t, const NidState *nid, double *x, double *r, double *d,
-                      double *b = nullptr, double *xu = nullptr);
+                      double *b = nullptr, double *xu = nullptr, double *sqb = nullptr);
 struct Beta32Vecs {
     double *c = nullptr;
     const double *b = nullptr, *xu = nullptr;
@@ -133,7 +137,14 @@
                       double *d, int phase = 1, const Beta32Vecs *bv = nullptr);
 void launch_cheb_restart(hipStream_t s, const double *part, int nparts, int n_pad,
                          const DevScalars *sc, const NidState *nid, const double *b, double *x,
-                         double *r, double *d, const Beta32Vecs *bv = nullptr);
+                         double *r, double *d, const Beta32Vecs *bv = nullptr,
+                         double *sqr = nullptr);
+int cheb_sq_parts(int n_pad, int nparts);
+void launch_nid_k2(hipStream_t s, const double *sqb, int Gb, const double *sqr, int Gr, int kcap,
+                   const DevScalars *sc, NidState *nid, const Beta32Vecs *bv, const double *w,
+                   int n_pad, unsigned long long *tag, unsigned long long seq);
+void launch_nid_redo(hipStream_t s, NidState *nid, const double *b, int n_pad, double *x,
+                     double *r, double *d);
 void launch_eapply(hipStream_t s, const double *X, int ldx, int n_pad, int p_loc,
                    const double *D, const double *v, const NidState *nid, int j, double *part,
                    const float *X32 = nullptr, int kind = 0, double *gb = nullptr);
diff --git a/bayesbridge_amd/csrc/bb_nid.hip b/bayesbridge_amd/csrc/bb_nid.hip
--- a/bayesbridge_amd/csrc/bb_nid.hip
+++ b/bayesbridge_amd/csrc/bb_nid.hip
@@ -81,6 +81,60 @@
         K1 = bk1;
         K2 = bk2;
         err1_out = be;
+    }
+}
+
+__device__ void nid_plan_resid(double eta, double e2, double eps1, int kcap, double limit,
+                               const NidState *nid, bool any_cost, double bsave, int &K1,
+                               int &K2) {
+    const int lane = threadIdx.x & 63;
+    K1 = K2 = 0;
+    if (!(e2 < 1e300) || !(eps1 > 0.0) || kcap < 1) return;
+    const ChebConst c1 = cheb_const(eps1), c2 = cheb_const(e2);
+    const int kmax = kcap < 64 ? kcap : 64;
+    const double a1 = acosh(c1.sigma1), a2 = acosh(c2.sigma1);
+    const bool in = lane + 1 <= kmax;
+    const double t1 = in ? sqrt(1.0 + eps1) / cosh((lane + 1) * a1) * (1.0 + 1e-12) : HUGE_VAL;
+    const double t2 = in ? sqrt(1.0 + e2) / cosh((lane + 1) * a2) * (1.0 + 1e-12) : HUGE_VAL;
+    const double step32 = nid->c32 + nid->cstep, step64 = nid->c64 + nid->cstep;
+    const double cap = (kcap - 1) * step64;
+    const int k1 = lane + 1;
+    const double rho = eta + t1 * (1.0 + eta);
+    const double need = kNidTol / rho;
+    int lo = 1, hi = kmax + 1;
+#pragma unroll
+    for (int it = 0; it < 7; ++it) {
+        const int mid = (lo + hi) >> 1;
+        const double tm = __shfl(t2, (mid < kmax ? mid : kmax) - 1, 64);
+        if (lo < hi) {
+            if (eta + tm * (1.0 + eta) <= need)
+                hi = mid;
+            else
+                lo = mid + 1;
+        }
+    }
+    const int k2 = lo <= kmax ? lo : 0;
+    double cost = (k1 <= kmax && rho < 1.0 && k2)
+                      ? (k1 - 1) * step32 + step64 + (k2 - 1) * step32
+                      : HUGE_VAL;
+    if (!(cost < cap * (1.0 - 1e-9))) cost = HUGE_VAL;
+    if (rho * (1.0 + 1e-6) <= kBeta32Tol) cost -= bsave;
+    if (!any_cost && !(cost <= limit)) cost = HUGE_VAL;
+    double bc = cost;
+    int bk1 = k1, bk2 = k2;
+#pragma unroll
+    for (int o = 32; o > 0; o >>= 1) {
+        const double oc = __shfl_xor(bc, o, 64);
+        const int ok1 = __shfl_xor(bk1, o, 64), ok2 = __shfl_xor(bk2, o, 64);
+        if (oc < bc || (oc == bc && ok1 < bk1)) {
+            bc = oc;
+            bk1 = ok1;
+            bk2 = ok2;
+        }
+    }
+    if (bc < HUGE_VAL) {
+        K1 = bk1;
+        K2 = bk2;
     }
 }
 
@@ -132,7 +186,6 @@
             eta = 0.0;
         }
     }
-    if ((threadIdx.x & 63) != 0) return;
     int b32 = 0;
     if (b32_pays && mode > 0) {
         double bound = HUGE_VAL;
@@ -142,17 +195,62 @@
             bound = cheb_bound_at(eps, mode) + cheb_bound_at(eps, mode - 1);
         b32 = bound * (1.0 + 1e-6) <= kBeta32Tol;
     }
+    int resid = 0;
+    const int fb_mode = mode, fb_k2 = k2, fb_b32 = b32;
+    const double fb_eta = eta;
+    double ecb2 = ecb;
+    if (allow && (allow_mixed & kAllowMixed) && (allow_mixed & kAllowResid) &&
+        g_dev_nid_force_k == 0 && mode > 0 && (K == 0 || K > 2)) {
+        const double tr = round_up_12(red[kNidTS] / sc->sig2 * (1.0 + 1e-6));
+        const double etam = (2.0 * kU32 * sqrt(tr * eps) + kU32 * kU32 * tr) * (1.0 + 1e-6);
+        const double e2 = eps + etam;
+        const double phi = ldexp(8.0, -4 * (allow_mixed >> kResidPhiShift));
+        double eps1 = e2;
+        if (lam > 0.0 && lam < HUGE_VAL && nid->sum_cn > 0.0)
+            eps1 = fmin(e2, phi * tr * lam / nid->sum_cn);
+        const double step32 = nid->c32 + nid->cstep, step64 = nid->c64 + nid->cstep;
+        const double today = (k2 ? (mode - 1) * step32 + step64 + (k2 - 1) * step32
+                                 : (mode - 1) * step64) -
+                             (b32 ? bsave : 0.0);
+        int k1r, k2r;
+        nid_plan_resid(etam, e2, eps1, k_launched, today * (k2 ? 1.0 + 1e-9 : 1.0 - 1e-9), nid,
+                       (allow_mixed & kResidAnyCost) != 0, bsave, k1r, k2r);
+        if (k2r > 0) {
+            resid = 1;
+            mode = k1r;
+            k2 = k2r;
+            b32 = b32_pays;
+            eta = etam;
+            ecb = eps1;
+            ecb2 = e2;
+        }
+    }
+    if ((threadIdx.x & 63) != 0) return;
     nid->eps = eps;
     nid->mode = mode;
     nid->k2 = k2;
     nid->b32 = b32;
-    nid->n_beta32 += (unsigned long long)b32;
+    if (!resid) nid->n_beta32 += (unsigned long long)b32;
     nid->eta = eta;
-    const ChebConst c = cheb_const(ecb);
+    const ChebConst c = cheb_const(ecb), cc = cheb_const(ecb2);
     nid->theta = c.theta;
     nid->delta = c.delta;
     nid->sigma1 = c.sigma1;
-    if (mode && k2) {
+    nid->theta2 = cc.theta;
+    nid->delta2 = cc.delta;
+    nid->sigma12 = cc.sigma1;
+    nid->e2 = ecb2;
+    nid->resid = resid;
+    nid->fb_mode = fb_mode;
+    nid->fb_k2 = fb_k2;
+    nid->fb_b32 = fb_b32;
+    nid->fb_eta = fb_eta;
+    if (resid) {
+        nid->n_cheb += 1;
+        nid->n_mixed += 1;
+        nid->n_products += 1ull;
+        nid->n_products32 += (unsigned long long)(mode - 1);
+    } else if (mode && k2) {
         nid->n_cheb += 1;
         nid->n_mixed += 1;
         nid->n_products += 1ull;
@@ -168,7 +266,7 @@
     if (k2_host) *k2_host = (double)(k2 + 128 * b32);
     if (tag_seq && mode_host)
         __hip_atomic_store((unsigned long long *)(mode_host + 2),
-                           (tag_seq << 16) | ((unsigned long long)mode << 8) |
+                           (tag_seq << 16) | ((unsigned long long)(mode | (resid << 7)) << 8) |
                                (unsigned)(k2 | (b32 << 7)),
                            __ATOMIC_RELAXED, __HIP_MEMORY_SCOPE_SYSTEM);
 }
@@ -334,20 +432,30 @@
 static int rowsum_rw(int nparts) { return nparts >= 128 ? 8 : 64; }
 
 template <int RW>
+__device__ __forceinline__ void rows_sq_part(double v, double *__restrict__ out) {
+    double s = v * v;
+#pragma unroll
+    for (int o = RW / 2; o > 0; o >>= 1) s += __shfl_xor(s, o, RW);
+    if (threadIdx.x == 0) out[blockIdx.x] = s;
+}
+
+template <int RW>
 __global__ __launch_bounds__(kRsThreads) void k_cheb_init(
     const double *__restrict__ xu_part, int nparts, int n, int n_pad,
     const double *__restrict__ y, const DevScalars *sc, Key key, uint64_t t, const NidState *nid,
-    double *x, double *r, double *d, double *b, double *xu_out, int xcd) {
+    double *x, double *r, double *d, double *b, double *xu_out, int xcd, double *sqb) {
     if (nid->mode == 0) return;
     const int i = rs_block(xcd) * RW + (int)threadIdx.x;
     const double xu = part_rowsum_rw<RW>(xu_part, nparts, n_pad, rs_block(xcd) * RW);
-    if ((int)threadIdx.x >= RW || i >= n_pad) return;
+    if ((int)threadIdx.x >= RW) return;
     double rhs = 0.0;
     if (i < n) {
         const double sig = sqrt(sc->sig2);
         const double delta = normal_at(key, t, KIND_DELTA, (uint64_t)i);
         rhs = y[i] / sig - (xu / sig + delta);
     }
+    if (sqb) rows_sq_part<RW>(rhs, sqb);
+    if (i >= n_pad) return;
     const double d0 = rhs / nid->theta;
     r[i] = rhs;
     d[i] = d0;
@@ -373,9 +481,10 @@
     const double dv = d[i];
     const double qv = dv + e / sc->sig2;
     const double rv = r[i] - qv;
-    const double s1 = nid->sigma1;
+    const double s1 = phase == 2 ? nid->sigma12 : nid->sigma1;
+    const double dl = phase == 2 ? nid->delta2 : nid->delta;
     const double rho0 = cheb_rho(s1, j - 1), rho1 = 1.0 / (2.0 * s1 - rho0);
-    const double dn = rho1 * rho0 * dv + (2.0 * rho1 / nid->delta) * rv;
+    const double dn = rho1 * rho0 * dv + (2.0 * rho1 / dl) * rv;
     r[i] = rv;
     d[i] = dn;
     const double xn = x[i] + dn;
@@ -391,21 +500,119 @@
 __global__ __launch_bounds__(kRsThreads) void k_cheb_restart(
     const double *__restrict__ part, int nparts, int n_pad, const DevScalars *sc,
     const NidState *nid, const double *__restrict__ b, double *x, double *r, double *d, int xcd,
-    Beta32Vecs bv) {
+    Beta32Vecs bv, double *sqr) {
     if (nid->k2 == 0 || nid->mode == 0) return;
     const int i = rs_block(xcd) * RW + (int)threadIdx.x;
     const double e = part_rowsum_rw<RW>(part, nparts, n_pad, rs_block(xcd) * RW);
-    if ((int)threadIdx.x >= RW || i >= n_pad) return;
-    const double xv = x[i];
-    const double rv = b[i] - (xv + e / sc->sig2);
-    const double dv = rv / nid->theta;
+    if ((int)threadIdx.x >= RW) return;
+    const bool in = i < n_pad;
+    const double xv = in ? x[i] : 0.0;
+    const double rv = in ? b[i] - (xv + e / sc->sig2) : 0.0;
+    if (sqr) rows_sq_part<RW>(rv, sqr);
+    if (!in) return;
+    const double dv = rv / nid->theta2;
     r[i] = rv;
     d[i] = dv;
     x[i] = xv + dv;
     if (bv.c) {
         bv.c[i] = dv;
-        if (nid->k2 == 1 && nid->b32) beta32_xb(bv, sc, i, xv + dv);
-    }
+        if (nid->k2 == 1 && nid->b32 && !nid->resid) beta32_xb(bv, sc, i, xv + dv);
+    }
+}
+
+constexpr int kK2Threads = 1024;
+__global__ __launch_bounds__(kK2Threads) void k_nid_k2(
+    const double *__restrict__ sqb, int Gb, const double *__restrict__ sqr, int Gr, int kcap,
+    const DevScalars *sc, NidState *nid, Beta32Vecs bv, const double *__restrict__ w, int n_pad,
+    unsigned long long *tag, unsigned long long seq) {
+    __shared__ int sh[3];
+    __shared__ double shr;
+    if (!nid->resid || nid->mode == 0 || nid->k2 == 0) return;
+    const int lane = threadIdx.x & 63;
+    if (threadIdx.x < 64) {
+        const double eps = nid->eps, eta = nid->eta, e2 = nid->e2;
+        const int wanted = nid->b32;
+        double bb = 0.0, rr = 0.0;
+        for (int g = lane; g < Gb; g += 64) bb += sqb[g];
+        for (int g = lane; g < Gr; g += 64) rr += sqr[g];
+        bb = wave_sum_all(bb);
+        rr = wave_sum_all(rr);
+        double ratio = rr == 0.0 ? 0.0 : sqrt(rr) * (1.0 + eps) * (1.0 + 1e-6) / sqrt(bb);
+        const int kmax = kcap < 64 ? kcap : 64;
+        const ChebConst c = cheb_const(e2);
+        const double tk = lane + 1 <= kmax ? sqrt(1.0 + e2) / cosh((lane + 1) * acosh(c.sigma1)) *
+                                                 (1.0 + 1e-12)
+                                           : HUGE_VAL;
+        const double err2 = eta + tk * (1.0 + eta);
+        const bool ok = ratio < 1.0 && lane + 1 <= kmax && err2 * ratio <= kNidTol;
+        const unsigned long long m = __ballot(ok);
+        const int K2 = m ? __ffsll((long long)m) : 0;
+        const double e2k = __shfl(err2, K2 ? K2 - 1 : 0, 64);
+        const int b32 = K2 && wanted && (1.0 + e2k) * ratio * (1.0 + 1e-6) <= kBeta32Tol;
+        if (lane == 0) {
+            sh[0] = K2;
+            sh[1] = b32;
+            shr = ratio;
+        }
+    }
+    __syncthreads();
+    const int K2 = sh[0], b32 = sh[1];
+    if (K2 == 1 && b32 && bv.c)
+        for (int i = threadIdx.x; i < n_pad; i += kK2Threads) beta32_xb(bv, sc, i, w[i]);
+    if (threadIdx.x != 0) return;
+    const int mode = nid->mode;
+    nid->ratio = shr;
+    unsigned long long word;
+    if (K2) {
+        nid->k2 = K2;
+        nid->b32 = b32;
+        nid->n_beta32 += (unsigned long long)b32;
+        nid->n_products32 += (unsigned long long)(K2 - 1);
+        nid->n_resid += 1;
+        word = ((unsigned long long)mode << 8) | (unsigned)(K2 | (b32 << 7));
+    } else {
+        nid->mode = 0;
+        nid->k2 = 0;
+        nid->b32 = 0;
+        nid->n_redo += 1;
+        word = (1ull << 16) | ((unsigned long long)nid->fb_mode << 8) |
+               (unsigned)(nid->fb_k2 | (nid->fb_b32 << 7));
+    }
+    __hip_atomic_store(tag, (seq << 24) | word, __ATOMIC_RELAXED, __HIP_MEMORY_SCOPE_SYSTEM);
+}
+
+__global__ __launch_bounds__(64) void k_nid_adopt(NidState *nid) {
+    if (threadIdx.x != 0 || nid->resid == 0) return;
+    const int mode = nid->fb_mode, k2 = nid->fb_k2;
+    nid->mode = mode;
+    nid->k2 = k2;
+    nid->b32 = nid->fb_b32;
+    nid->n_beta32 += (unsigned long long)nid->fb_b32;
+    nid->eta = nid->fb_eta;
+    const ChebConst c = cheb_const(k2 ? nid->e2 : nid->eps);
+    nid->theta = nid->theta2 = c.theta;
+    nid->delta = nid->delta2 = c.delta;
+    nid->sigma1 = nid->sigma12 = c.sigma1;
+    nid->resid = 0;
+    if (k2) {
+        nid->n_products += 1ull;
+        nid->n_products32 += (unsigned long long)(mode - 1 + k2 - 1);
+    } else {
+        nid->n_mixed -= 1;
+        nid->n_products += (unsigned long long)(mode - 1);
+    }
+}
+
+__global__ __launch_bounds__(256) void k_cheb_reinit(const NidState *nid,
+                                                     const double *__restrict__ b, int n_pad,
+                                                     double *x, double *r, double *d) {
+    const int i = blockIdx.x * 256 + threadIdx.x;
+    if (nid->mode == 0 || i >= n_pad) return;
+    const double rhs = b[i];
+    const double d0 = rhs / nid->theta;
+    r[i] = rhs;
+    d[i] = d0;
+    x[i] = d0;
 }
 
 __global__ __launch_bounds__(64 * kRedWaves) void k_part_sum(const double *__restrict__ part,
@@ -679,15 +886,15 @@
 void launch_cheb_init(hipStream_t s, const double *xu_part, int nparts, int n, int n_pad,
                       const double *y, const DevScalars *sc, uint64_t k0, uint64_t k1,
                       uint64_t t, const NidState *nid, double *x, double *r, double *d,
-                      double *b, double *xu) {
+                      double *b, double *xu, double *sqb) {
     if (rowsum_rw(nparts) == 8)
         k_cheb_init<8><<<(n_pad + 7) / 8, kRsThreads, 0, s>>>(xu_part, nparts, n, n_pad, y, sc,
                                                               Key{k0, k1}, t, nid, x, r, d, b,
-                                                              xu, g_rs_xcd);
+                                                              xu, g_rs_xcd, sqb);
     else
         k_cheb_init<64><<<(n_pad + 63) / 64, kRsThreads, 0, s>>>(xu_part, nparts, n, n_pad, y,
                                                                  sc, Key{k0, k1}, t, nid, x, r, d,
-                                                                 b, xu, g_rs_xcd);
+                                                                 b, xu, g_rs_xcd, sqb);
 }
 
 void launch_cheb_step(hipStream_t s, const double *part, int nparts, int n_pad,
@@ -704,14 +911,32 @@
 
 void launch_cheb_restart(hipStream_t s, const double *part, int nparts, int n_pad,
                          const DevScalars *sc, const NidState *nid, const double *b, double *x,
-                         double *r, double *d, const Beta32Vecs *bv) {
+                         double *r, double *d, const Beta32Vecs *bv, double *sqr) {
     const Beta32Vecs v = bv ? *bv : Beta32Vecs{};
     if (rowsum_rw(nparts) == 8)
         k_cheb_restart<8><<<(n_pad + 7) / 8, kRsThreads, 0, s>>>(part, nparts, n_pad, sc, nid, b,
-                                                                 x, r, d, g_rs_xcd, v);
+                                                                 x, r, d, g_rs_xcd, v, sqr);
     else
         k_cheb_restart<64><<<(n_pad + 63) / 64, kRsThreads, 0, s>>>(part, nparts, n_pad, sc, nid,
-                                                                    b, x, r, d, g_rs_xcd, v);
+                                                                    b, x, r, d, g_rs_xcd, v, sqr);
+}
+
+int cheb_sq_parts(int n_pad, int nparts) {
+    const int rw = rowsum_rw(nparts);
+    return (n_pad + rw - 1) / rw;
+}
+
+void launch_nid_k2(hipStream_t s, const double *sqb, int Gb, const double *sqr, int Gr, int kcap,
+                   const DevScalars *sc, NidState *nid, const Beta32Vecs *bv, const double *w,
+                   int n_pad, unsigned long long *tag, unsigned long long seq) {
+    k_nid_k2<<<1, kK2Threads, 0, s>>>(sqb, Gb, sqr, Gr, kcap, sc, nid, bv ? *bv : Beta32Vecs{}, w,
+                                      n_pad, tag, seq);
+}
+
+void launch_nid_redo(hipStream_t s, NidState *nid, const double *b, int n_pad, double *x,
+                     double *r, double *d) {
+    k_nid_adopt<<<1, 64, 0, s>>>(nid);
+    k_cheb_reinit<<<(n_pad + 255) / 256, 256, 0, s>>>(nid, b, n_pad, x, r, d);
 }
 
 void launch_eapply(hipStream_t s, const double *X, int ldx, int n_pad, int p_loc,
diff --git a/include/bayesbridge.h b/include/bayesbridge.h
--- a/include/bayesbridge.h
+++ b/include/bayesbridge.h
@@ -281,6 +281,9 @@
 
 int bb_engine_nid_beta32(bb_engine *e, unsigned long long *beta32_sweeps, int *b32);
 
+int bb_engine_nid_resid(bb_engine *e, unsigned long long *resid_sweeps,
+                        unsigned long long *redo_sweeps, double *ratio);
+
 int bb_engine_error_flags(bb_engine *e, uint32_t *flags);
 
 
```

Result: faster. 1399 sweeps/s, median of 6 (+4.6%).
